# phylo42/IPK

Hardware: AMD Instinct MI355X
Metric: scored phylo-k-mers/sec (higher is better)
Workload: dtype f32

## Files before the change

### ipk_amd/csrc/ipkgpu.hip

```cpp
#include <cstring>
#include <hip/hip_runtime.h>
#include <rocprim/rocprim.hpp>

#include <algorithm>
#include <cmath>
#include <cstdarg>
#include <cstdio>
#include <cstring>
#include <new>
#include <string>
#include <type_traits>
#include <unordered_map>
#include <memory>
#include <vector>

#include "../../include/ipkgpu.h"
#include "dcla_device.hpp"
#include "kernels_score.hpp"
#include "kernels_quad.hpp"
#include "kernels_compact.hpp"
#include "kernels_keymajor.hpp"
#include "kernels_reduce_pipe.hpp"
#include "kernels_filter.hpp"
#include "kernels_dbfile.hpp"
#include "kernels_spill.hpp"
#include "spill_format.hpp"
#include <sys/stat.h>
#include <chrono>

using namespace ipkgpu;


namespace {

struct DevBuf {
    void* p = nullptr;
    size_t cap = 0;
    template <class T> T* as() const { return reinterpret_cast<T*>(p); }
};

struct EventPool {
    std::vector<hipEvent_t> free_ev;
    hipEvent_t get()
    {
        if (!free_ev.empty()) { hipEvent_t e = free_ev.back(); free_ev.pop_back(); return e; }
        hipEvent_t e = nullptr;
        return hipEventCreate(&e) == hipSuccess ? e : nullptr;
    }
    void put(hipEvent_t e) { if (free_ev.size() < 64) free_ev.push_back(e); else (void)hipEventDestroy(e); }
};
struct Stopwatch {
    hipStream_t stream;
    EventPool* pool;
    std::vector<hipEvent_t> ev;
    Stopwatch(hipStream_t s, EventPool* p) : stream(s), pool(p) {}
    ~Stopwatch() { for (hipEvent_t e : ev) pool->put(e); }
    int mark()
    {
        hipEvent_t e = pool->get();
        if (!e) return -1;
        (void)hipEventRecord(e, stream);
        ev.push_back(e);
        return (int)ev.size() - 1;
    }
    double ms(int a, int b) const
    {
        float t = 0;
        if (a < 0 || b < 0 || hipEventElapsedTime(&t, ev[a], ev[b]) != hipSuccess) return 0;
        return t;
    }
};

}

struct ipkgpu_comm;
struct ipkgpu_ctx;
static void ipkgpu_comm_release(ipkgpu_ctx* ctx);
struct ipkgpu_ctx {
    int device = 0;
    ipkgpu_comm* comm = nullptr;
    hipStream_t stream = nullptr;
    std::string err;
    int64_t workspace_bytes = 0;
    int64_t opt_variant = 0;
    int64_t opt_flags = 0;
    int64_t opt_kmc_pass = 0;
    int64_t opt_prefix_mats = 0;
    int64_t opt_wg_chunks2 = 0;
    int64_t opt_rounds = 0;
    int64_t opt_pool_limit = 0;
    int64_t opt_pool_chunks = 0;
    DevBuf table, best, ovfq, counts, offsets, goff, idx, branch, scan_sums, scan_boff, tmp_a, tmp_b, tmp_c;
    DevBuf pool, desc, gbcnt, gboff, gbcur, clist, gm, tile_next;
    DevBuf ptrs;
    DevBuf sp_bits, sp_pops, sp_rank, sp_c16;
    void* h_spill[2] = {nullptr, nullptr}; hipEvent_t ev_spill[2] = {nullptr, nullptr}; size_t h_spill_cap = 0;
    size_t held = 0, held_peak = 0;
    int64_t budget = 0;
    size_t refused_need = 0;
    DevBuf mask;
    bool mask_valid = false;
    uint64_t mask_words = 0;
    bool table_compressed = false;
    DevBuf rank, vaddr, ucnt, qpack, xstart, pcounts;
    DevBuf seq, pvals, pvaddr, mrank, cursnap;
    DevBuf cvals, coff, croom;
    bool comp_own_vals = false;
    std::vector<uint32_t> h_branch;
    uint32_t comp_nb = 0, comp_stride = 0, comp_tbl = 0;
    double pairs_per_window = 0;
    double acc_main_ms = 0, acc_reduce_ms = 0;
    double acc_count_ms = 0, acc_write_ms = 0, acc_km_ms = 0;
    const char* main_kernel = "";
    std::vector<std::pair<void*, size_t>> free_blocks;
    std::unordered_map<void*, size_t> live_blocks;
    size_t cached_bytes = 0, cache_limit = 0;
    void* small = nullptr;
    void* h_up = nullptr; size_t h_up_cap = 0; hipEvent_t up_done = nullptr; bool up_pending = false;
    unsigned long long emitted_host = 0; bool emitted_fetched = false;
    uint32_t* h_rb = nullptr;
    EventPool events;
    bool spec_skip_wait = false;
    uint64_t pool_want_min = 0;
    struct Pending {
        bool active = false;
        std::unique_ptr<Stopwatch> sw; int ev_a = -1, ev_b = -1, ev_c = -1, ev_d = -1;
        uint64_t cap = 0, max_chunks = 0, windows = 0; uint32_t gb = 0; bool pool_ovf_ok = false, use_quad = false;
    } pend;
    uint64_t last_entries = 0; uint32_t last_gb = 0;
    double t_write_total = 0, t_write_device = 0, t_write_file = 0;
    int num_cu = 256;
};

struct ipkgpu_result {
    ipkgpu_ctx* ctx = nullptr;
    std::vector<uint32_t> group_ids;
    std::vector<uint64_t> offsets;
    uint64_t emitted = 0;
    uint32_t* d_keys = nullptr;
    float* d_scores = nullptr;
    uint32_t* d_positions = nullptr;
    size_t cap = 0;
    std::vector<uint32_t> h_keys;
    std::vector<float> h_scores;
    std::vector<uint32_t> h_positions;
    bool h_keys_ok = false, h_scores_ok = false, h_positions_ok = false;
    double t_total = 0, t_prefix = 0, t_score = 0, t_compact = 0, t_main = 0, t_reduce = 0;
    int score_launches = 0;
};

struct ipkgpu_parts {
    ipkgpu_ctx* ctx = nullptr;
    uint32_t n_owners = 1;
    uint64_t slots = 0;
    uint32_t* d_counts = nullptr;
    uint2* d_entries = nullptr;
    uint32_t* d_positions = nullptr;
    std::vector<uint64_t> owner_off;
    uint64_t emitted = 0;
    uint32_t* pre_keys = nullptr; uint64_t* pre_key_off = nullptr; uint64_t pre_n_keys = 0; double t_keys = 0;
    uint32_t sigma = 0, k = 0;
    uint32_t lead = 0;
    uint64_t key_base = 0;
    double t_total = 0, t_prefix = 0, t_score = 0, t_compact = 0, t_main = 0, t_reduce = 0, t_count = 0, t_write = 0, t_km = 0;
    int score_launches = 0;
};

struct ipkgpu_db {
    ipkgpu_ctx* ctx = nullptr;
    uint64_t n_keys = 0, n_entries = 0;
    uint32_t* d_keys = nullptr;
    uint64_t* d_key_off = nullptr;
    uint2* d_entries = nullptr;
    uint32_t* d_positions = nullptr;
    std::vector<uint32_t> h_positions;
    bool h_pos_ok = false;
    std::vector<uint32_t> h_keys;
    std::vector<uint64_t> h_key_off;
    std::vector<uint32_t> h_entries;
    bool h_ok = false;
    double t_merge = 0;
    double* d_fv64 = nullptr;
    float* d_fv32 = nullptr;
    uint32_t* d_order = nullptr;
    std::vector<double> h_fv64;
    std::vector<float> h_fv32;
    std::vector<uint32_t> h_order;
    bool h_filter_ok = false;
    double t_filter = 0;
};

static std::string g_create_err;
constexpr size_t RB_BYTES = 4096, RB_OWNER_OFF = 8 , RB_OWNERS_MAX = 500;

template <class T = uint32_t> static T* small_at(const ipkgpu_ctx* ctx, uint32_t off) { return reinterpret_cast<T*>(static_cast<char*>(ctx->small) + off); }

static int fail(ipkgpu_ctx* ctx, int code, const char* fmt, ...)
{
    char buf[512];
    va_list ap;
    va_start(ap, fmt);
    vsnprintf(buf, sizeof buf, fmt, ap);
    va_end(ap);
    if (ctx) ctx->err = buf; else g_create_err = buf;
    return code;
}

#define HIP_TRY(ctx, expr)                                                                      \
    do {                                                                                        \
        hipError_t e_ = (expr);                                                                 \
// ... 49 lines not shown


static int upload_stage(ipkgpu_ctx* ctx, size_t bytes, void** out)
{
    if (ctx->up_pending) { HIP_TRY(ctx, hipEventSynchronize(ctx->up_done)); ctx->up_pending = false; }
    if (!ctx->up_done) HIP_TRY(ctx, hipEventCreateWithFlags(&ctx->up_done, hipEventDisableTiming));
    if (bytes > ctx->h_up_cap) {
        if (ctx->h_up) { (void)hipHostFree(ctx->h_up); ctx->h_up = nullptr; ctx->h_up_cap = 0; }
        const size_t cap = std::max<size_t>(bytes + bytes / 2, 1 << 16);
        HIP_TRY(ctx, hipHostMalloc(&ctx->h_up, cap, hipHostMallocDefault));
        ctx->h_up_cap = cap;
    }
    *out = ctx->h_up;
    return IPKGPU_OK;
}
static int upload_staged(ipkgpu_ctx* ctx)
{
    HIP_TRY(ctx, hipEventRecord(ctx->up_done, ctx->stream));
    ctx->up_pending = true;
    return IPKGPU_OK;
}

static hipError_t ctx_alloc(ipkgpu_ctx* ctx, void** out, size_t bytes)
{
    bytes = std::max<size_t>((bytes + 255) & ~(size_t)255, 256);
    size_t best = (size_t)-1;
    for (size_t i = 0; i < ctx->free_blocks.size(); ++i) {
        const size_t cap = ctx->free_blocks[i].second;
        if (cap >= bytes && cap <= bytes + bytes / 2 + (1 << 20) && (best == (size_t)-1 || cap < ctx->free_blocks[best].second)) best = i;
    }
    if (best != (size_t)-1) {
        *out = ctx->free_blocks[best].first;
        ctx->live_blocks[*out] = ctx->free_blocks[best].second;
        ctx->cached_bytes -= ctx->free_blocks[best].second;
        ctx->free_blocks.erase(ctx->free_blocks.begin() + best);
        return hipSuccess;
    }
    hipError_t e = dev_malloc(ctx, out, bytes);
    if (e != hipSuccess && !ctx->free_blocks.empty()) {
        drop_cache(ctx);
        (void)hipGetLastError();
        e = dev_malloc(ctx, out, bytes);
    }
    if (e == hipSuccess) ctx->live_blocks[*out] = bytes;
    return e;
}
static void ctx_release(ipkgpu_ctx* ctx, void* p)
{
    if (!p) return;
    auto it = ctx->live_blocks.find(p);
    if (it == ctx->live_blocks.end()) { (void)hipFree(p); return; }
    const size_t cap = it->second;
    ctx->live_blocks.erase(it);
    if (ctx->cached_bytes + cap <= ctx->cache_limit) { ctx->free_blocks.push_back({p, cap}); ctx->cached_bytes += cap; }
    else (void)dev_free(ctx, p, cap);
}

static constexpr uint64_t WAVE_PER_ITEM_SPAN = 1ull << 24;

static hipError_t ctx_alloc_atleast(ipkgpu_ctx* ctx, void** out, size_t min_bytes, size_t want_bytes, size_t* got)
{
    min_bytes = std::max<size_t>((min_bytes + 255) & ~(size_t)255, 256);
    want_bytes = std::max(want_bytes, min_bytes);
    size_t best = (size_t)-1;
    for (size_t i = 0; i < ctx->free_blocks.size(); ++i) {
        const size_t cap = ctx->free_blocks[i].second;
        if (cap >= min_bytes && cap <= want_bytes + want_bytes / 2 + (1 << 20) && (best == (size_t)-1 || cap < ctx->free_blocks[best].second)) best = i;
    }
    if (best != (size_t)-1) {
        *out = ctx->free_blocks[best].first;
        *got = ctx->free_blocks[best].second;
        ctx->live_blocks[*out] = *got;
        ctx->cached_bytes -= *got;
        ctx->free_blocks.erase(ctx->free_blocks.begin() + best);
        return hipSuccess;
    }
    const hipError_t e = ctx_alloc(ctx, out, want_bytes);
    if (e == hipSuccess) *got = ctx->live_blocks[*out];
    return e;
}

static std::vector<DevBuf*> all_workspaces(ipkgpu_ctx* ctx)
{
    return {&ctx->table, &ctx->best, &ctx->ovfq, &ctx->counts, &ctx->offsets, &ctx->goff, &ctx->idx,
            &ctx->branch, &ctx->scan_sums, &ctx->scan_boff, &ctx->tmp_a, &ctx->tmp_b, &ctx->tmp_c,
            &ctx->pool, &ctx->desc, &ctx->gbcnt, &ctx->gboff, &ctx->gbcur, &ctx->clist, &ctx->gm, &ctx->tile_next, &ctx->mask,
            &ctx->rank, &ctx->vaddr, &ctx->ucnt, &ctx->qpack, &ctx->xstart, &ctx->pcounts, &ctx->ptrs,
            &ctx->cvals, &ctx->coff, &ctx->croom, &ctx->seq, &ctx->pvals, &ctx->pvaddr, &ctx->mrank, &ctx->cursnap,
            &ctx->sp_bits, &ctx->sp_pops, &ctx->sp_rank, &ctx->sp_c16};
}

extern "C" {

uint32_t ipkgpu_bits_per_symbol(uint32_t sigma) { return sigma == 4 ? 2u : sigma == 20 ? 5u : 0u; }
uint32_t ipkgpu_max_k(uint32_t sigma) { return sigma == 4 ? 14u : sigma == 20 ? 6u : 0u; }
uint32_t ipkgpu_max_k_keyrange(uint32_t sigma) { return sigma == 4 ? 16u : ipkgpu_max_k(sigma); }
size_t ipkgpu_kmer_batch(uint32_t key, size_t n_ranges) { return n_ranges ? key % n_ranges : 0; }

float ipkgpu_log_threshold(float omega, uint32_t sigma, uint32_t k)
{
    return log10f(powf(omega / (float)sigma, (float)k));
}

const char* ipkgpu_last_error(const ipkgpu_ctx* ctx) { return ctx ? ctx->err.c_str() : g_create_err.c_str(); }

int ipkgpu_create(int device_id, ipkgpu_ctx** out)
{
    if (!out) return fail(nullptr, IPKGPU_ERR_INVALID, "ipkgpu_create: null out pointer");
    *out = nullptr;
    int n = 0;
    hipError_t e = hipGetDeviceCount(&n);
    if (e != hipSuccess || n <= 0)
        return fail(nullptr, IPKGPU_ERR_NODEVICE, "no HIP device available (%s); this engine has no CPU fallback",
                    e != hipSuccess ? hipGetErrorString(e) : "device count 0");
    if (device_id < 0 || device_id >= n)
        return fail(nullptr, IPKGPU_ERR_INVALID, "device %d out of range (0..%d)", device_id, n - 1);
    ipkgpu_ctx* ctx = new (std::nothrow) ipkgpu_ctx();
    if (!ctx) return fail(nullptr, IPKGPU_ERR_NOMEM, "out of host memory");
    ctx->device = device_id;
    if ((e = hipSetDevice(device_id)) != hipSuccess ||
        (e = hipStreamCreateWithFlags(&ctx->stream, hipStreamNonBlocking)) != hipSuccess) {
        delete ctx;
        return fail(nullptr, IPKGPU_ERR_HIP, "device setup failed: %s", hipGetErrorString(e));
    }
    hipDeviceProp_t prop;
    if (hipGetDeviceProperties(&prop, device_id) == hipSuccess) ctx->num_cu = prop.multiProcessorCount;
    size_t free_b = 0, total_b = 0;
    if (hipMemGetInfo(&free_b, &total_b) == hipSuccess) { ctx->workspace_bytes = (int64_t)(free_b / 2); ctx->cache_limit = free_b / 4; }
    else ctx->workspace_bytes = (int64_t)8 << 30;
    if ((e = hipMalloc(&ctx->small, SMALL_BYTES)) != hipSuccess) {
        (void)hipStreamDestroy(ctx->stream);
        delete ctx;
        return fail(nullptr, IPKGPU_ERR_NOMEM, "hipMalloc failed: %s", hipGetErrorString(e));
    }
    if ((e = hipHostMalloc((void**)&ctx->h_rb, RB_BYTES, hipHostMallocDefault)) != hipSuccess) {
        (void)hipFree(ctx->small);
        (void)hipStreamDestroy(ctx->stream);
        delete ctx;
        return fail(nullptr, IPKGPU_ERR_NOMEM, "hipHostMalloc failed: %s", hipGetErrorString(e));
    }
    memset(ctx->h_rb, 0, RB_BYTES);
    *out = ctx;
    return IPKGPU_OK;
}

void ipkgpu_destroy(ipkgpu_ctx* ctx)
{
    if (!ctx) return;
    (void)hipSetDevice(ctx->device);
    (void)hipStreamSynchronize(ctx->stream);
    for (DevBuf* b : all_workspaces(ctx)) if (b->p) (void)hipFree(b->p);
    for (auto& b : ctx->free_blocks) (void)hipFree(b.first);
    ipkgpu_comm_release(ctx);
    if (ctx->small) (void)hipFree(ctx->small);
    if (ctx->h_up) (void)hipHostFree(ctx->h_up);
    for (int i = 0; i < 2; ++i) { if (ctx->h_spill[i]) (void)hipHostFree(ctx->h_spill[i]); if (ctx->ev_spill[i]) (void)hipEventDestroy(ctx->ev_spill[i]); }
    ctx->pend.sw.reset();
    for (hipEvent_t e : ctx->events.free_ev) (void)hipEventDestroy(e);
    ctx->events.free_ev.clear();
    if (ctx->h_rb) (void)hipHostFree(ctx->h_rb);
    if (ctx->up_done) (void)hipEventDestroy(ctx->up_done);
    (void)hipStreamDestroy(ctx->stream);
    delete ctx;
}

int ipkgpu_set_option(ipkgpu_ctx* ctx, const char* name, int64_t value)
{
// ... 55 lines not shown
    if (SIGMA == 4) return K <= 10 ? IPK_QCAP : IPK_QCAP12;
    return IPK_AACAP;
}

template <int SIGMA, int K, bool POS = false>
int launch_score(ipkgpu_ctx* ctx, const ScoreParams& p)
{
    constexpr int CAP = fast_cap<SIGMA, K>();
    constexpr size_t lds = TileGeo<SIGMA, K, TW>::HEAD_BYTES + (size_t)NW * wave_scratch_entries<SIGMA, K, CAP>() * 8;
    static_assert(lds <= 160 * 1024, "fast-path LDS budget");
    auto kern = score_tiles_kernel<SIGMA, K, CAP, TW, NW, POS>;
    if (lds > 64 * 1024)
        HIP_TRY(ctx, hipFuncSetAttribute(reinterpret_cast<const void*>(kern), hipFuncAttributeMaxDynamicSharedMemorySize, (int)lds));
    const uint64_t blocks = (uint64_t)p.n_batch_mats * p.tiles_per_mat;
    if (blocks > 0x7fffffffull) return fail(ctx, IPKGPU_ERR_INVALID, "batch too large for one launch");
    hipLaunchKernelGGL(kern, dim3((uint32_t)blocks), dim3(NW * 64), lds, ctx->stream, p);
    HIP_TRY(ctx, hipGetLastError());
    return IPKGPU_OK;
}

template <int SIGMA, int K, bool POS = false>
int launch_overflow(ipkgpu_ctx* ctx, const ScoreParams& p)
{
    if constexpr (Geo<SIGMA, K, 1 << 30>::DIRECT || ipow(SIGMA, K - K / 2) <= (uint32_t)fast_cap<SIGMA, K>()) {
        (void)ctx; (void)p;
        return IPKGPU_OK;
    } else {
        constexpr size_t lds = TileGeo<SIGMA, K, 1>::HEAD_BYTES + (size_t)wave_scratch_entries<SIGMA, K, big_capf<SIGMA, K>()>() * 8;
        static_assert(lds <= 160 * 1024, "big-list LDS budget");
        auto kern = score_overflow_kernel<SIGMA, K, POS>;
        if (lds > 64 * 1024)
            HIP_TRY(ctx, hipFuncSetAttribute(reinterpret_cast<const void*>(kern), hipFuncAttributeMaxDynamicSharedMemorySize, (int)lds));
        const uint32_t per_cu = (uint32_t)std::max<size_t>(1, std::min<size_t>(32 / OVF_NW, (160 * 1024) / (lds + 64)));
        hipLaunchKernelGGL(kern, dim3(ctx->num_cu * per_cu), dim3(OVF_NW * 64), lds, ctx->stream, p);
        HIP_TRY(ctx, hipGetLastError());
        return IPKGPU_OK;
    }
}

template <int SIGMA, int K, bool POS>
int launch_both(ipkgpu_ctx* ctx, const ScoreParams& p)
{
    RC_TRY((launch_score<SIGMA, K, POS>(ctx, p)));
    return launch_overflow<SIGMA, K, POS>(ctx, p);
}


template <int SIGMA, int K> constexpr uint32_t stream_tbl()
{
    constexpr uint64_t T = ipow(SIGMA, K);
    if (Geo<SIGMA, K, 1 << 30>::DIRECT) return 0;
    if (SIGMA == 4 && K >= 13) return 0;
    if (SIGMA == 4) return T <= 16384 ? (uint32_t)T : (K <= 10 ? 16384u : 32768u);
    if (K <= 3) return (uint32_t)T;
    if (K <= 5) return 32000u;
    return 0;
}

template <int SIGMA, int K> constexpr int stream_nw() { return NW; }
template <int SIGMA, int K> constexpr int stream_tw() { return TW; }

template <int SIGMA, int K>
int launch_stream_pass1(ipkgpu_ctx* ctx, const StreamParams& sp, uint32_t n_wg)
{
    constexpr uint32_t TBL = stream_tbl<SIGMA, K>();
    if constexpr (TBL == 0) { (void)sp; (void)n_wg; return fail(ctx, IPKGPU_ERR_INVALID, "stream variant unsupported for this sigma/k"); }
    else {
        constexpr int CAP = fast_cap<SIGMA, K>();
        constexpr uint32_t T = ipow(SIGMA, K);
        constexpr uint32_t NB = (T + TBL - 1) / TBL;
        constexpr int SNW = stream_nw<SIGMA, K>(), STW = stream_tw<SIGMA, K>();
        constexpr size_t lds = TileGeo<SIGMA, K, STW>::HEAD_BYTES + (size_t)SNW * stream_wave_scratch<SIGMA, K, CAP>() * 8 + (size_t)SNW * 2 * NB * SUB * 4;
        static_assert(lds <= 160 * 1024, "stream pass-1 LDS budget");
        auto kern = score_stream_kernel<SIGMA, K, CAP, STW, SNW, TBL>;
        if (lds > 64 * 1024)
            HIP_TRY(ctx, hipFuncSetAttribute(reinterpret_cast<const void*>(kern), hipFuncAttributeMaxDynamicSharedMemorySize, (int)lds));
        hipLaunchKernelGGL(kern, dim3(n_wg), dim3(SNW * 64), lds, ctx->stream, sp);
        HIP_TRY(ctx, hipGetLastError());
        return IPKGPU_OK;
    }
}

template <int SIGMA, int K>
int launch_stream_overflow(ipkgpu_ctx* ctx, const StreamParams& sp)
{
    constexpr uint32_t TBL = stream_tbl<SIGMA, K>();
    if constexpr (TBL == 0 || ipow(SIGMA, K - K / 2) <= (uint32_t)fast_cap<SIGMA, K>()) {
        (void)ctx; (void)sp;
        return IPKGPU_OK;
    } else {
        constexpr uint32_t NB = (uint32_t)((ipow(SIGMA, K) + TBL - 1) / TBL);
        constexpr size_t lds = TileGeo<SIGMA, K, 1>::HEAD_BYTES + (size_t)wave_scratch_entries<SIGMA, K, big_capf<SIGMA, K>()>() * 8 +
                               (size_t)OVF_NW * 2 * NB * SUB * 4;
        static_assert(lds + 64 <= 160 * 1024, "big-list (stream) LDS budget");
        auto kern = score_overflow_stream_kernel<SIGMA, K, TBL>;
        if (lds > 64 * 1024)
            HIP_TRY(ctx, hipFuncSetAttribute(reinterpret_cast<const void*>(kern), hipFuncAttributeMaxDynamicSharedMemorySize, (int)lds));
        const uint32_t per_cu = (uint32_t)std::max<size_t>(1, std::min<size_t>(32 / OVF_NW, (160 * 1024) / (lds + 64)));
        hipLaunchKernelGGL(kern, dim3(ctx->num_cu * per_cu), dim3(OVF_NW * 64), lds, ctx->stream, sp);
        HIP_TRY(ctx, hipGetLastError());
        return IPKGPU_OK;
    }
}

#ifndef IPK_RPIPE_DEFAULT
#define IPK_RPIPE_DEFAULT 1
#endif
#ifndef IPK_RPIPE_D
#define IPK_RPIPE_D 2
#endif
template <int SIGMA, int K>
int launch_stream_pass2(ipkgpu_ctx* ctx, uint32_t n_gb, uint64_t T, uint32_t* table, bool compress)
{
    constexpr uint32_t TBL = stream_tbl<SIGMA, K>();
    if constexpr (TBL == 0) { (void)n_gb; (void)T; (void)table; (void)compress; return fail(ctx, IPKGPU_ERR_INVALID, "stream variant unsupported"); }
    else {
        constexpr uint32_t NB = (uint32_t)((ipow(SIGMA, K) + TBL - 1) / TBL);
        constexpr int NT = TBL <= 16384 ? 512 : 1024;
        const size_t lds = compress ? (size_t)comp_padded_slots<TBL, NT>() * 4 + (NT / 64 + 1) * 4 : (size_t)TBL * 4;
        auto launch = [&](auto kern) -> int {
            if (lds > 64 * 1024)
                HIP_TRY(ctx, hipFuncSetAttribute(reinterpret_cast<const void*>(kern), hipFuncAttributeMaxDynamicSharedMemorySize, (int)lds));
            hipLaunchKernelGGL(kern, dim3(n_gb), dim3(NT), lds, ctx->stream, ctx->pool.as<uint2>(),
                               ctx->gboff.as<uint64_t>(), ctx->clist.as<uint2>(), NB, T, table, ctx->mask.as<uint32_t>(), ctx->mask_words,
                               ctx->cvals.as<uint2>(), ctx->coff.as<uint64_t>(), ctx->rank.as<uint32_t>(), ctx->vaddr.as<uint64_t>(), ctx->ucnt.as<uint32_t>());
            HIP_TRY(ctx, hipGetLastError());
            return IPKGPU_OK;
        };
        if constexpr (TBL * 4 > 80 * 1024) {
            if (compress && ((IPK_RPIPE_DEFAULT != 0) != ((ctx->opt_flags & 2048) != 0))) {
                constexpr int PD = IPK_RPIPE_D;
                auto kern = reduce_buckets_pipe_kernel<TBL, NT, PD>;
                HIP_TRY(ctx, hipFuncSetAttribute(reinterpret_cast<const void*>(kern), hipFuncAttributeMaxDynamicSharedMemorySize, (int)lds));
                hipLaunchKernelGGL(kern, dim3(std::min<uint32_t>(n_gb, (uint32_t)ctx->num_cu)), dim3(NT), lds, ctx->stream, ctx->pool.as<uint2>(),
                                   ctx->gboff.as<uint64_t>(), ctx->clist.as<uint2>(), n_gb, NB, T, ctx->mask.as<uint32_t>(), ctx->mask_words,
                                   ctx->cvals.as<uint2>(), ctx->coff.as<uint64_t>(), ctx->rank.as<uint32_t>(), ctx->vaddr.as<uint64_t>(), ctx->ucnt.as<uint32_t>());
                HIP_TRY(ctx, hipGetLastError());
                return IPKGPU_OK;
            }
        }
        return compress ? launch(reduce_buckets_kernel<TBL, NT, true>) : launch(reduce_buckets_kernel<TBL, NT, false>);
    }
}

template <int SIGMA, int K> size_t stream_lds() {
    constexpr uint32_t TBL = stream_tbl<SIGMA, K>();
    if constexpr (TBL == 0) return 0;
    else {
        constexpr int CAP = fast_cap<SIGMA, K>();
        constexpr uint32_t NB = (uint32_t)((ipow(SIGMA, K) + TBL - 1) / TBL);
        return TileGeo<SIGMA, K, stream_tw<SIGMA, K>()>::HEAD_BYTES + (size_t)stream_nw<SIGMA, K>() * stream_wave_scratch<SIGMA, K, CAP>() * 8 +
               (size_t)stream_nw<SIGMA, K>() * 2 * NB * SUB * 4;
    }
}
template <int SIGMA, int K> uint32_t stream_nb() {
    constexpr uint32_t TBL = stream_tbl<SIGMA, K>();
    if constexpr (TBL == 0) return 0; else return (uint32_t)((ipow(SIGMA, K) + TBL - 1) / TBL);
}

template <int SIGMA, int K> constexpr bool quad_ok() { return QuadGeo<SIGMA, K>::OK && stream_tbl<SIGMA, K>() != 0; }
#ifndef IPK_QNW
#define IPK_QNW 4
#endif
#ifndef IPK_QTW
#define IPK_QTW 40
#endif
template <int SIGMA, int K> constexpr int quad_nw() { return K <= 10 ? IPK_QNW : IPK_QNW12; }
template <int SIGMA, int K> constexpr int quad_tw() { return K <= 10 ? IPK_QTW : IPK_QTW12; }
#ifndef IPK_QROWLANE12
#define IPK_QROWLANE12 1
#endif
#ifndef IPK_QROWLANE
#define IPK_QROWLANE 0
#endif
template <int SIGMA, int K> constexpr bool quad_rowlane() { return K <= 10 ? IPK_QROWLANE != 0 : IPK_QROWLANE12 != 0; }
#ifndef IPK_QONEWIN12
#define IPK_QONEWIN12 1
#endif
template <int SIGMA, int K> constexpr bool quad_onewin() { return K >= 11 && IPK_QONEWIN12 != 0 && quad_rowlane<SIGMA, K>(); }
template <int SIGMA, int K> size_t quad_lds()
{
    if constexpr (!quad_ok<SIGMA, K>()) return 0;
    else {
        constexpr int CAP = fast_cap<SIGMA, K>();
        constexpr uint32_t TBL = stream_tbl<SIGMA, K>();
        constexpr uint32_t NB = (uint32_t)((ipow(SIGMA, K) + TBL - 1) / TBL);
        return QuadTile<SIGMA, K, quad_tw<SIGMA, K>()>::HEAD_BYTES + (size_t)quad_nw<SIGMA, K>() * quad_wave_entries<SIGMA, K, CAP, quad_onewin<SIGMA, K>()>() * 8 +
               (size_t)quad_nw<SIGMA, K>() * NB * 8;
    }
}
template <int SIGMA, int K, bool COUNT_ONLY = false>
int launch_quad_pass1(ipkgpu_ctx* ctx, const StreamParams& sp, uint32_t n_wg)
{
    if constexpr (!quad_ok<SIGMA, K>()) { (void)sp; (void)n_wg; return fail(ctx, IPKGPU_ERR_INVALID, "quad kernel unsupported for this sigma/k"); }
    else {
        constexpr int CAP = fast_cap<SIGMA, K>();
        constexpr uint32_t TBL = stream_tbl<SIGMA, K>();
        constexpr int QNW = quad_nw<SIGMA, K>(), QTW = quad_tw<SIGMA, K>();
        const size_t lds = quad_lds<SIGMA, K>();
        auto kern = score_quad_kernel<SIGMA, K, CAP, QTW, QNW, TBL, COUNT_ONLY, quad_rowlane<SIGMA, K>(), quad_onewin<SIGMA, K>()>;
        if (lds > 64 * 1024)
            HIP_TRY(ctx, hipFuncSetAttribute(reinterpret_cast<const void*>(kern), hipFuncAttributeMaxDynamicSharedMemorySize, (int)lds));
        hipLaunchKernelGGL(kern, dim3(n_wg), dim3(QNW * 64), lds, ctx->stream, sp);
        HIP_TRY(ctx, hipGetLastError());
        return IPKGPU_OK;
    }
}

#ifndef IPK_XPNW
#define IPK_XPNW 11
#endif
#ifndef IPK_XPTW
#define IPK_XPTW 128
#endif
constexpr int XP_TW = IPK_XPTW;
template <int SIGMA, int K> constexpr int xp_nw() { return SIGMA == 20 ? IPK_XPNW : 11; }
template <int SIGMA, int K> constexpr uint32_t xp_tbl()
{
    if (SIGMA == 20 && K == 6) return 16000u;
    if (SIGMA == 4 && K >= 13) return 32768u;
    return stream_tbl<SIGMA, K>();
}
template <int SIGMA, int K, int KK = K> uint32_t xp_nb() {
    constexpr uint32_t TBL = xp_tbl<SIGMA, K>();
    if constexpr (TBL == 0) return 0; else return (uint32_t)((ipow(SIGMA, KK) + TBL - 1) / TBL);
}
template <int SIGMA, int K, int KK = K> size_t xp_lds() {
    constexpr uint32_t TBL = xp_tbl<SIGMA, K>();
    if constexpr (TBL == 0) return 0;
    else {
        constexpr int CAP = fast_cap<SIGMA, K>();
        constexpr uint32_t NB = (uint32_t)((ipow(SIGMA, KK) + TBL - 1) / TBL);
        return TileGeo<SIGMA, K, XP_TW>::HEAD_BYTES + (size_t)xp_nw<SIGMA, K>() * stream_wave_scratch<SIGMA, K, CAP>() * 8 + (size_t)NB * 4;
    }
}
template <int SIGMA, int K, bool WRITE, int KK = K, bool POS = false>
int launch_xp(ipkgpu_ctx* ctx, const XpParams& xp, uint32_t n_wg)
{
    constexpr uint32_t TBL = xp_tbl<SIGMA, K>();
    if constexpr (TBL == 0) { (void)xp; (void)n_wg; return fail(ctx, IPKGPU_ERR_INVALID, "exact-partition variant unsupported for this sigma/k"); }
    else {
        constexpr int CAP = fast_cap<SIGMA, K>();
        constexpr uint32_t NB = (uint32_t)((ipow(SIGMA, KK) + TBL - 1) / TBL);
        constexpr size_t lds = TileGeo<SIGMA, K, XP_TW>::HEAD_BYTES + (size_t)xp_nw<SIGMA, K>() * stream_wave_scratch<SIGMA, K, CAP>() * 8 + (size_t)NB * 4;
        static_assert(lds <= 160 * 1024, "exact-partition LDS budget");
        static_assert((TileGeo<SIGMA, K, XP_TW>::HEAD_BYTES + (size_t)xp_nw<SIGMA, K>() * stream_wave_scratch<SIGMA, K, CAP>() * 8) % 8 == 0, "cursor alignment");
        auto kern = score_xp_kernel<SIGMA, K, CAP, XP_TW, xp_nw<SIGMA, K>(), TBL, WRITE, KK, POS>;
        if (lds > 64 * 1024)
            HIP_TRY(ctx, hipFuncSetAttribute(reinterpret_cast<const void*>(kern), hipFuncAttributeMaxDynamicSharedMemorySize, (int)lds));
        hipLaunchKernelGGL(kern, dim3(n_wg), dim3(xp_nw<SIGMA, K>() * 64), lds, ctx->stream, xp);
        HIP_TRY(ctx, hipGetLastError());
        return IPKGPU_OK;
    }
}
template <int SIGMA, int K, bool WRITE, int KK = K, bool POS = false>
int launch_xp_overflow(ipkgpu_ctx* ctx, const XpParams& xp)
{
    constexpr uint32_t TBL = xp_tbl<SIGMA, K>();
    if constexpr (TBL == 0 || ipow(SIGMA, K - K / 2) <= (uint32_t)fast_cap<SIGMA, K>()) {
        (void)ctx; (void)xp;
        return IPKGPU_OK;
    } else {
// ... 9 lines not shown
    }
}
template <int SIGMA, int K, bool COMPRESS, int KK = K>
int launch_xp_reduce(ipkgpu_ctx* ctx, uint32_t n_gb, uint32_t S, uint64_t T, const uint64_t* off, uint32_t* table)
{
    constexpr uint32_t TBL = xp_tbl<SIGMA, K>();
    if constexpr (TBL == 0) { (void)n_gb; (void)S; (void)T; (void)off; (void)table; return fail(ctx, IPKGPU_ERR_INVALID, "exact-partition variant unsupported"); }
    else {
        constexpr uint32_t NB = (uint32_t)((ipow(SIGMA, KK) + TBL - 1) / TBL);
        static_assert(!COMPRESS || NB == 1 || TBL % 64 == 0, "a 64-slot block must not straddle two buckets");
        constexpr int NT = TBL <= 16384 ? 512 : 1024;
        constexpr size_t lds = COMPRESS ? (size_t)comp_padded_slots<TBL, NT>() * 4 + (NT / 64 + 1) * 4 : (size_t)TBL * 4;
        auto kern = reduce_ranges_kernel<TBL, NT, COMPRESS>;
        if (lds > 64 * 1024)
            HIP_TRY(ctx, hipFuncSetAttribute(reinterpret_cast<const void*>(kern), hipFuncAttributeMaxDynamicSharedMemorySize, (int)lds));
        hipLaunchKernelGGL(kern, dim3(n_gb), dim3(NT), lds, ctx->stream, ctx->pool.as<uint2>(), off, S, NB, T, table,
                           ctx->mask.as<uint32_t>(), ctx->mask_words, ctx->rank.as<uint32_t>(), ctx->vaddr.as<uint64_t>(), ctx->ucnt.as<uint32_t>());
        HIP_TRY(ctx, hipGetLastError());
        return IPKGPU_OK;
    }
}
template <int SIGMA, int K>
int launch_xp_reduce_pos(ipkgpu_ctx* ctx, uint32_t n_gb, uint32_t S, uint64_t T, const uint64_t* off, uint32_t nwin)
{
    constexpr uint32_t TBL = xp_tbl<SIGMA, K>();
    if constexpr (TBL == 0) { (void)n_gb; (void)S; (void)T; (void)off; (void)nwin; return fail(ctx, IPKGPU_ERR_INVALID, "exact-partition variant unsupported"); }
    else {
        constexpr uint32_t NB = (uint32_t)((ipow(SIGMA, K) + TBL - 1) / TBL);
        static_assert(NB == 1 || TBL % 64 == 0, "a 64-slot block must not straddle two buckets");
        constexpr int NT = pos_sub_slots<TBL>() <= 4096 ? 256 : 1024;
        constexpr size_t lds = (size_t)pos_sub_blocks<TBL>() * 64 * 8 + (pos_sub_blocks<TBL>() + 1) * 4;
        static_assert(lds <= 160 * 1024, "positions reduce LDS budget");
        auto kern = reduce_ranges_pos_kernel<TBL, NT>;
        if (lds > 64 * 1024)
            HIP_TRY(ctx, hipFuncSetAttribute(reinterpret_cast<const void*>(kern), hipFuncAttributeMaxDynamicSharedMemorySize, (int)lds));
        hipLaunchKernelGGL(kern, dim3(n_gb), dim3(NT), lds, ctx->stream, ctx->pool.as<uint2>(), ctx->seq.as<uint32_t>(), off, S, NB, T, nwin,
                           ctx->mask_words, ctx->pvals.as<uint32_t>(), ctx->pvaddr.as<uint64_t>());
        HIP_TRY(ctx, hipGetLastError());
        return IPKGPU_OK;
    }
}
template <int V> using int_c = std::integral_constant<int, V>;

template <int SIGMA, int K, int KMAX, class F> int with_k(ipkgpu_ctx* ctx, uint32_t k, F& f)
{
    if (k == (uint32_t)K) return f(int_c<SIGMA>{}, int_c<K>{});
    if constexpr (K < KMAX) return with_k<SIGMA, K + 1, KMAX>(ctx, k, f);
    else return fail(ctx, IPKGPU_ERR_INVALID, "unsupported sigma/k (%u/%u)", (uint32_t)SIGMA, k);
}
template <class F> int with_sigma_k(ipkgpu_ctx* ctx, uint32_t sigma, uint32_t k, F&& f)
{
    if (sigma == 4) return with_k<4, 2, 14>(ctx, k, f);
    if (sigma == 20) return with_k<20, 2, 6>(ctx, k, f);
    return fail(ctx, IPKGPU_ERR_INVALID, "unsupported sigma/k (%u/%u)", sigma, k);
}

bool keyrange_supported(uint32_t sigma, uint32_t k, uint32_t lead)
{
    return sigma == 4 && lead >= 1 && k > lead && k - lead >= 13 && k - lead <= 14 && k <= 16;
}
template <class F> int with_xp_shape(ipkgpu_ctx* ctx, uint32_t sigma, uint32_t k, uint32_t lead, F&& f)
{
    if (!lead) return with_sigma_k(ctx, sigma, k, [&](auto S_, auto K_) { return f(S_, K_, K_); });
    if (sigma == 4) {
        switch (k * 8 + lead) {
            case 14 * 8 + 1: return f(int_c<4>{}, int_c<14>{}, int_c<13>{});
            case 15 * 8 + 1: return f(int_c<4>{}, int_c<15>{}, int_c<14>{});
            case 15 * 8 + 2: return f(int_c<4>{}, int_c<15>{}, int_c<13>{});
            case 16 * 8 + 2: return f(int_c<4>{}, int_c<16>{}, int_c<14>{});
            case 16 * 8 + 3: return f(int_c<4>{}, int_c<16>{}, int_c<13>{});
        }
    }
    return fail(ctx, IPKGPU_ERR_INVALID, "unsupported key range");
}

struct Geometry {
    uint32_t fast_cap = 0;
    uint32_t stream_nb = 0, stream_tbl = 0;
    uint32_t stream_nw = NW, stream_tw = TW;
    size_t stream_lds = 0;
    bool quad = false;
    uint32_t quad_nw = NW, quad_tw = TW;
    size_t quad_lds = 0;
    uint32_t xp_nb = 0, xp_tbl = 0;
    size_t xp_lds = 0;
};

int fill_geometry(ipkgpu_ctx* ctx, uint32_t sigma, uint32_t k, uint32_t lead, Geometry& g)
{
    if (!lead)
        RC_TRY(with_sigma_k(ctx, sigma, k, [&](auto S_, auto K_) {
            g.fast_cap = fast_cap<S_, K_>();
            g.stream_nb = stream_nb<S_, K_>(); g.stream_tbl = stream_tbl<S_, K_>();
            g.stream_nw = stream_nw<S_, K_>(); g.stream_tw = stream_tw<S_, K_>(); g.stream_lds = stream_lds<S_, K_>();
            g.quad = quad_ok<S_, K_>();
            g.quad_nw = quad_nw<S_, K_>(); g.quad_tw = quad_tw<S_, K_>(); g.quad_lds = quad_lds<S_, K_>();
            return IPKGPU_OK;
        }));
    return with_xp_shape(ctx, sigma, k, lead, [&](auto S_, auto K_, auto KK_) {
        g.xp_nb = xp_nb<S_, K_, KK_>(); g.xp_tbl = xp_tbl<S_, K_>(); g.xp_lds = xp_lds<S_, K_, KK_>();
        return IPKGPU_OK;
    });
}

#ifndef IPK_KMC_RUNS_DEFAULT
#define IPK_KMC_RUNS_DEFAULT 1
#endif
#ifndef IPK_KMC_PASS
#define IPK_KMC_PASS 256
#endif
#define KM_LAUNCH(KERN, CAPV, ...)                                                                                        \
    do {                                                                                                                  \
        if (P == 1) hipLaunchKernelGGL((KERN<true, CAPV>), dim3((uint32_t)(per_xcd * 8)), dim3(256), 0, ctx->stream, __VA_ARGS__); \
        else hipLaunchKernelGGL((KERN<false, CAPV>), dim3((uint32_t)(per_xcd * 8)), dim3(256), 0, ctx->stream, __VA_ARGS__);     \
    } while (0)

CompTable comp_table(const ipkgpu_ctx* ctx)
{
    CompTable ct;
    ct.mask = ctx->mask.as<uint32_t>(); ct.rank = ctx->rank.as<uint32_t>(); ct.vaddr = ctx->vaddr.as<uint64_t>();
    ct.pool = ctx->comp_own_vals ? ctx->cvals.as<uint2>() : ctx->pool.as<uint2>();
    ct.off = ctx->comp_own_vals ? ctx->coff.as<uint64_t>() : ctx->gboff.as<uint64_t>(); ct.mask_words = ctx->mask_words;
    ct.NB = ctx->comp_nb; ct.stride = ctx->comp_stride; ct.TBL = ctx->comp_tbl;
    return ct;
}

}

namespace {

constexpr int IPKGPU_RETRY_SMALLER = 100;
constexpr int IPKGPU_RETRY_AGAIN = 101;
#ifndef IPK_OVF_POOL_RATIO
#define IPK_OVF_POOL_RATIO 500
#endif

enum class PassKind { tiles, stream, quad, xp };
struct Pass {
    PassKind kind = PassKind::tiles;
    bool positions = false;
    bool compress = false;
    bool seq = false;
    double slot_bytes() const { return positions ? 8.0 : kind == PassKind::xp && compress ? 0.3125 : 4.0; }
};

Pass choose_pass(int64_t variant, uint32_t sigma, uint32_t lead, bool positions, bool km_positions, const Geometry& g)
{
    Pass ps;
    ps.positions = positions;
    if (positions) return ps;
    if (km_positions) { ps.kind = PassKind::xp; ps.compress = true; ps.seq = true; return ps; }
    const int64_t v = variant;
    if (g.xp_nb != 0 && (v == 3 || v == 4 || (v == 0 && g.stream_nb == 0) || lead != 0)) {
        ps.kind = PassKind::xp;
        ps.compress = v != 3;
    } else if (g.stream_nb != 0 && g.stream_nb <= 2048 && (v == 0 || v == 2 || v == 5 || v == 6 || v == 7)) {
        ps.kind = v != 2 && g.quad ? PassKind::quad : PassKind::stream;
        ps.compress = v == 6 || (v == 0 && g.stream_tbl == 32768u && sigma == 4);
    }
    return ps;
}

struct Plan {
    uint32_t n_mats = 0, sites = 0, sigma = 0, k = 0;
    float eps = 0;
    std::vector<uint32_t> group_ids;
    std::vector<uint32_t> slot_of;
    uint32_t n_groups = 0, nwin = 0, tiles_per_mat = 0, chunks_per_group = 0;
    uint64_t table_size = 0, gpb = 1;
    uint32_t lead = 0, lead_c = 0;
    Geometry geo;
    Pass pass;
    const uint32_t* mat_rank = nullptr;
};

int make_plan(ipkgpu_ctx* ctx, const void* logp, uint32_t n_mats, uint32_t sites, uint32_t sigma,
              const uint32_t* mat_group, uint32_t k, float log_eps, Plan& pl, uint32_t lead = 0, uint32_t lead_c = 0,
              bool positions = false, bool km_positions = false)
{
    if (!logp || !mat_group) return fail(ctx, IPKGPU_ERR_INVALID, "null input pointer");
    if (sigma != 4 && sigma != 20) return fail(ctx, IPKGPU_ERR_INVALID, "unsupported alphabet size %u (4 or 20)", sigma);
    if (lead == 0 && (k < 2 || k > ipkgpu_max_k(sigma)))
        return fail(ctx, IPKGPU_ERR_INVALID, "k=%u out of range [2, %u] for sigma=%u", k, ipkgpu_max_k(sigma), sigma);
    if (lead != 0 && !keyrange_supported(sigma, k, lead))
        return fail(ctx, IPKGPU_ERR_INVALID, "no key-range pass of k=%u with %u leading symbols for sigma=%u", k, lead, sigma);
    pl.lead = lead; pl.lead_c = lead_c;
    if (n_mats == 0) return fail(ctx, IPKGPU_ERR_INVALID, "no matrices");
    if (sites < k) return fail(ctx, IPKGPU_ERR_INVALID, "alignment has %u sites, fewer than k=%u", sites, k);
    pl.n_mats = n_mats; pl.sites = sites; pl.sigma = sigma; pl.k = k; pl.eps = log_eps;
    RC_TRY(fill_geometry(ctx, sigma, k, lead, pl.geo));
    if (km_positions && (lead != 0 || pl.geo.xp_nb == 0))
        return fail(ctx, IPKGPU_ERR_INVALID, "no positioned database for sigma=%u k=%u: the call takes the exact partition, which needs more than 64 keys "
                                             "and no key-range pass", sigma, k);
    pl.pass = choose_pass(ctx->opt_variant, sigma, lead, positions, km_positions, pl.geo);
    pl.slot_of.resize(n_mats);
    std::unordered_map<uint32_t, uint32_t> index;
    index.reserve(n_mats);
    for (uint32_t i = 0; i < n_mats; ++i) {
        auto it = index.find(mat_group[i]);
        if (it == index.end()) {
            it = index.emplace(mat_group[i], (uint32_t)pl.group_ids.size()).first;
            pl.group_ids.push_back(mat_group[i]);
        }
        pl.slot_of[i] = it->second;
    }
    pl.n_groups = (uint32_t)pl.group_ids.size();
    pl.table_size = ipow(sigma, (int)(k - lead));
    pl.chunks_per_group = (uint32_t)((pl.table_size + CHUNK - 1) / CHUNK);
    pl.nwin = sites - k + 1;
    {
        const double ppw = ctx->pairs_per_window > 0 ? ctx->pairs_per_window : 256.0;
        const double pool_per_group = (double)n_mats / (double)pl.n_groups * (double)pl.nwin * ppw * (pl.pass.seq ? 16.0 : 8.0) * 1.25;
        const double per_group = (double)pl.table_size * pl.pass.slot_bytes() + pool_per_group;
        pl.gpb = std::max<uint64_t>(1, (uint64_t)((double)ctx->workspace_bytes / per_group));
    }
    pl.gpb = std::min<uint64_t>(pl.gpb, pl.n_groups);
    while (pl.gpb > 1 && pl.gpb * pl.chunks_per_group > 0x7fffffffull) pl.gpb /= 2;
    pl.tiles_per_mat = (pl.nwin + TW - 1) / TW;
// ... 81 lines not shown
        const size_t free_b = mem_free_bytes(ctx);
        const bool over_limit = ctx->opt_pool_limit > 0 && total * 8 > (uint64_t)ctx->opt_pool_limit;
        const uint64_t side = seq ? total * 8 + 512 : 0;
        const uint64_t side_have = seq ? ctx->seq.cap + ctx->pvals.cap : 0;
        if (over_limit || (total * 8 > ctx->pool.cap && total * 8 > free_b + ctx->pool.cap) ||
            (side > side_have && total * 8 + side > free_b + ctx->pool.cap + side_have)) {
            if (gb > 1) return IPKGPU_RETRY_SMALLER;
            return fail(ctx, IPKGPU_ERR_NOMEM, "the pair pool of ONE branch group (%llu pairs) does not fit device memory", (unsigned long long)total);
        }
    }
    RC_TRY(ensure(ctx, ctx->pool, std::max<uint64_t>(total, 1) * 8 + 256));
    {
        const uint64_t n_start = (uint64_t)gb * S * XNB;
        RC_TRY(ensure(ctx, ctx->xstart, n_start * 4));
        hipLaunchKernelGGL(xp_unit_starts_kernel, dim3((uint32_t)((n_start + 255) / 256)), dim3(256), 0, ctx->stream,
                           ctx->gboff.as<uint64_t>(), XNB, S, stride, n_start, ctx->xstart.as<uint32_t>(), small_at(ctx, SMALL_XP_TOO_BIG));
        HIP_TRY(ctx, hipGetLastError());
        xp.start = ctx->xstart.as<uint32_t>();
    }
    sp.pool = ctx->pool.as<uint2>();
    if (seq) {
        RC_TRY(ensure(ctx, ctx->seq, std::max<uint64_t>(total, 1) * 4 + 256));
        RC_TRY(ensure(ctx, ctx->pvals, std::max<uint64_t>(total, 1) * 4 + 256));
        xp.seq = ctx->seq.as<uint32_t>(); xp.mat_rank = pl.mat_rank;
    }
    const int ev_c = sw.mark();
    RC_TRY(xp_kernel(true));
    const int ev_d0 = sw.mark();
    RC_TRY(xp_overflow(true));
    const int ev_d = sw.mark();
    if (compress) {
        RC_TRY(ensure(ctx, ctx->rank, (size_t)gb * (ctx->mask_words / 2) * 4));
        RC_TRY(ensure(ctx, ctx->vaddr, (size_t)gb * (ctx->mask_words / 2) * 8));
        RC_TRY(ensure(ctx, ctx->ucnt, n_gb * 4));
    } else {
        RC_TRY(ensure(ctx, ctx->table, (size_t)gb * pl.table_size * 4));
    }
    uint32_t* const table = compress ? nullptr : ctx->table.as<uint32_t>();
    if (seq) {
        RC_TRY(ensure(ctx, ctx->pvaddr, (size_t)gb * (ctx->mask_words / 2) * 8));
        RC_TRY(with_sigma_k(ctx, pl.sigma, pl.k, [&](auto S_, auto K_) {
            return launch_xp_reduce_pos<S_, K_>(ctx, (uint32_t)n_gb, stride, pl.table_size, ctx->gboff.as<uint64_t>(), pl.nwin);
        }));
    }
    RC_TRY(with_xp_shape(ctx, pl.sigma, pl.k, pl.lead, [&](auto S_, auto K_, auto KK_) {
        const uint64_t* off = ctx->gboff.as<uint64_t>();
        return compress ? launch_xp_reduce<S_, K_, true, KK_>(ctx, (uint32_t)n_gb, stride, pl.table_size, off, table)
                        : launch_xp_reduce<S_, K_, false, KK_>(ctx, (uint32_t)n_gb, stride, pl.table_size, off, table);
    }));
    const int ev_e = sw.mark();
    uint32_t too_big = 0;
    HIP_TRY(ctx, hipMemcpyAsync(&too_big, small_at(ctx, SMALL_XP_TOO_BIG), 4, hipMemcpyDeviceToHost, ctx->stream));
    HIP_TRY(ctx, hipStreamSynchronize(ctx->stream));
    if (too_big) return fail(ctx, IPKGPU_ERR_INVALID, "a branch group scores 2^32 phylo-k-mers or more in one batch (exact-partition variant: 32-bit offsets inside a group)");
    ctx->mask_valid = true;
    ctx->table_compressed = compress;
    ctx->comp_nb = XNB; ctx->comp_stride = stride; ctx->comp_tbl = pl.geo.xp_tbl;
    ctx->acc_main_ms += sw.ms(ev_a, ev_a2) + sw.ms(ev_c, ev_d0);
    ctx->acc_count_ms += sw.ms(ev_a, ev_a2); ctx->acc_write_ms += sw.ms(ev_c, ev_d0);
    ctx->acc_reduce_ms += sw.ms(ev_d, ev_e);
    ctx->main_kernel = "score_xp_kernel";
    return IPKGPU_OK;
}

int stream_batch_check(ipkgpu_ctx* ctx)
{
    ipkgpu_ctx::Pending& pd = ctx->pend;
    if (!pd.active) return IPKGPU_OK;
    pd.active = false;
    std::unique_ptr<Stopwatch> sw(pd.sw.release());
    const uint32_t n_ovf = ctx->h_rb[SMALL_OVF_COUNT / 4], pool_exhausted = ctx->h_rb[SMALL_POOL_OVF / 4];
    if (pool_exhausted) {
        if (pd.cap >= pd.max_chunks) {
            ctx->pool_want_min = 0;
            if (pd.gb > 1) return IPKGPU_RETRY_SMALLER;
            return fail(ctx, IPKGPU_ERR_NOMEM, "the pair pool of ONE branch group is exhausted at the device-memory limit");
        }
        ctx->pool_want_min = pd.cap * 2;
        return IPKGPU_RETRY_AGAIN;
    }
    ctx->pool_want_min = 0;
    memcpy(&ctx->emitted_host, ctx->h_rb + SMALL_EMITTED / 4, 8);
    ctx->emitted_fetched = true;
    ctx->spec_skip_wait = !(n_ovf > 0 && (uint64_t)n_ovf * IPK_OVF_POOL_RATIO >= pd.windows && pd.pool_ovf_ok);
    if (sw) { ctx->acc_main_ms += sw->ms(pd.ev_a, pd.ev_b); ctx->acc_reduce_ms += sw->ms(pd.ev_c, pd.ev_d); }
    return IPKGPU_OK;
}

int arm_capped(ipkgpu_ctx* ctx, uint32_t sigma, uint32_t k, ScoreParams& p)
{
    const bool capped_lists = sigma == 4 && k >= 13;
    p.big_ovf = capped_lists ? small_at(ctx, SMALL_BIG_OVF) : nullptr;
    if (capped_lists) HIP_TRY(ctx, hipMemsetAsync(p.big_ovf, 0, 4, ctx->stream));
    return IPKGPU_OK;
}

int check_capped(ipkgpu_ctx* ctx, uint32_t k, const ScoreParams& p)
{
    if (!p.big_ovf) return IPKGPU_OK;
    uint32_t hit = 0;
    HIP_TRY(ctx, hipMemcpyAsync(&hit, p.big_ovf, 4, hipMemcpyDeviceToHost, ctx->stream));
    HIP_TRY(ctx, hipStreamSynchronize(ctx->stream));
    if (hit) return fail(ctx, IPKGPU_ERR_INVALID, "a window's half list exceeds %d entries: beyond the capacity of this engine at k = %u "
                                                  "(the lists of k >= 13 are capped; lower omega's reach or k)", BIG_CAP_ENTRIES, k);
    return IPKGPU_OK;
}

int score_batch_impl(ipkgpu_ctx* ctx, const Plan& pl, const float* logp_dev, uint32_t g0, uint32_t gb, bool defer)
{
    const uint32_t n_mats = pl.n_mats;
    uint32_t nb = 0;
    for (uint32_t i = 0; i < n_mats; ++i) nb += (pl.slot_of[i] >= g0 && pl.slot_of[i] < g0 + gb);
    const size_t gm_words = (size_t)gb + 1 + nb;
    void* stage = nullptr;
    RC_TRY(upload_stage(ctx, ((size_t)n_mats * 2 + gm_words) * 4, &stage));
    uint32_t* mat_list_h = reinterpret_cast<uint32_t*>(stage);
    uint32_t* mat_slot_h = mat_list_h + n_mats;
    uint32_t* gm = mat_slot_h + n_mats;
    nb = 0;
    for (uint32_t i = 0; i < n_mats; ++i) {
        mat_slot_h[i] = 0;
        if (pl.slot_of[i] >= g0 && pl.slot_of[i] < g0 + gb) { mat_list_h[nb++] = i; mat_slot_h[i] = pl.slot_of[i] - g0; }
    }
    for (uint32_t i = nb; i < n_mats; ++i) mat_list_h[i] = 0;
    for (size_t i = 0; i < gm_words; ++i) gm[i] = 0;
    for (uint32_t i = 0; i < n_mats; ++i)
        if (pl.slot_of[i] >= g0 && pl.slot_of[i] < g0 + gb) gm[pl.slot_of[i] - g0 + 1]++;
    for (uint32_t g = 0; g < gb; ++g) gm[g + 1] += gm[g];
    {
        std::vector<uint32_t> cur(gm, gm + gb);
        for (uint32_t i = 0; i < n_mats; ++i)
            if (pl.slot_of[i] >= g0 && pl.slot_of[i] < g0 + gb) gm[(size_t)gb + 1 + cur[pl.slot_of[i] - g0]++] = i;
    }
    RC_TRY(ensure(ctx, ctx->idx, (size_t)n_mats * 8));
    RC_TRY(ensure(ctx, ctx->ovfq, (size_t)nb * pl.nwin * 8));
    RC_TRY(ensure(ctx, ctx->gm, gm_words * 4));
    HIP_TRY(ctx, hipMemcpyAsync(ctx->idx.p, mat_list_h, (size_t)n_mats * 8, hipMemcpyHostToDevice, ctx->stream));
    HIP_TRY(ctx, hipMemcpyAsync(ctx->gm.p, gm, gm_words * 4, hipMemcpyHostToDevice, ctx->stream));
    RC_TRY(upload_staged(ctx));

    const Pass& ps = pl.pass;
    ScoreParams p;
    p.logp = logp_dev;
    p.best = ctx->best.as<float>();
    p.mat_list = ctx->idx.as<uint32_t>();
    p.mat_slot = ctx->idx.as<uint32_t>() + n_mats;
    p.n_batch_mats = nb; p.sites = pl.sites; p.nwin = pl.nwin; p.tiles_per_mat = pl.tiles_per_mat;
    p.eps = pl.eps;
    p.table = ctx->table.p;
    p.mat_rank = pl.mat_rank;
    p.table_size = pl.table_size;
    p.emitted = small_at<unsigned long long>(ctx, SMALL_EMITTED);
    p.ovf_queue = ctx->ovfq.as<unsigned long long>();
    p.ovf_count = small_at(ctx, SMALL_OVF_COUNT);
    p.flags = (uint32_t)(!ps.positions && ctx->opt_variant == 99 ? 1 : 0);
    p.mask = nullptr; p.mask_words = 0;
    RC_TRY(arm_capped(ctx, pl.sigma, pl.k, p));
    ctx->mask_valid = false;
    ctx->table_compressed = false;
    ctx->comp_own_vals = false;
    const bool use_stream = ps.kind == PassKind::stream || ps.kind == PassKind::quad;
    const bool use_quad = ps.kind == PassKind::quad;
    if (!use_stream) {
        HIP_TRY(ctx, hipMemsetAsync(p.emitted, 0, 8, ctx->stream));
        HIP_TRY(ctx, hipMemsetAsync(p.ovf_count, 0, 4, ctx->stream));
    }
    if (ps.kind == PassKind::tiles) {
        const size_t table_bytes = (size_t)gb * pl.table_size * (ps.positions ? 8 : 4);
        RC_TRY(ensure(ctx, ctx->table, table_bytes));
        p.table = ctx->table.p;
        HIP_TRY(ctx, hipMemsetAsync(ctx->table.p, 0, table_bytes, ctx->stream));
        Stopwatch sw(ctx->stream, &ctx->events);
        const int a = sw.mark();
        RC_TRY(with_sigma_k(ctx, pl.sigma, pl.k, [&](auto S_, auto K_) {
            if (ps.positions) return launch_both<S_, K_, true>(ctx, p);
            if constexpr (S_ == 4 && K_ > 12) return fail(ctx, IPKGPU_ERR_INVALID, "unsupported sigma/k (%u/%u)", pl.sigma, pl.k);
            else return launch_both<S_, K_, false>(ctx, p);
        }));
        const int b = sw.mark();
        HIP_TRY(ctx, hipStreamSynchronize(ctx->stream));
        ctx->acc_main_ms += sw.ms(a, b);
        ctx->main_kernel = "score_tiles_kernel";
        return check_capped(ctx, pl.k, p);
    }

    ctx->mask_words = 2 * ((pl.table_size + 63) / 64);
    RC_TRY(ensure(ctx, ctx->mask, (size_t)gb * ctx->mask_words * 4));
    p.mask = ctx->mask.as<uint32_t>(); p.mask_words = ctx->mask_words;
    if (ps.kind == PassKind::xp) {
        if (!ps.compress) {
            RC_TRY(ensure(ctx, ctx->table, (size_t)gb * pl.table_size * 4));
            p.table = ctx->table.p;
        }
        const int rc = score_batch_xp(ctx, pl, logp_dev, gb, p);
        return rc ? rc : check_capped(ctx, pl.k, p);
    }

    const bool pool_ovf_ok = gb < (1u << 22) && n_mats < (1u << 21) && pl.nwin < (1u << 21);
    bool s_compress = pool_ovf_ok && ps.compress;
    const uint32_t NBK = pl.geo.stream_nb, TBL = pl.geo.stream_tbl;
    const uint32_t SNW = use_quad ? pl.geo.quad_nw : pl.geo.stream_nw;
    const uint32_t STW = use_quad ? pl.geo.quad_tw : pl.geo.stream_tw;
    const uint32_t s_tiles_per_mat = (pl.nwin + STW - 1) / STW;
    auto pass1 = [&](const StreamParams& sp, uint32_t n_wg, bool count_only) {
        return with_sigma_k(ctx, pl.sigma, pl.k, [&](auto S_, auto K_) {
            if (!use_quad) return launch_stream_pass1<S_, K_>(ctx, sp, n_wg);
            return count_only ? launch_quad_pass1<S_, K_, true>(ctx, sp, n_wg) : launch_quad_pass1<S_, K_, false>(ctx, sp, n_wg);
        });
    };

    const uint64_t windows = (uint64_t)nb * pl.nwin;
    if (ctx->pairs_per_window <= 0) {
        const uint32_t n_s = std::min<uint32_t>(gb, std::max<uint32_t>(2, gb / 64));
        const uint32_t stride_g = gb / n_s;
        std::vector<uint32_t> sgm((size_t)n_s + 1, 0), slist;
        for (uint32_t j = 0; j < n_s; ++j) {
            const uint32_t g = j * stride_g;
            for (uint32_t m = gm[g]; m < gm[g + 1]; ++m) slist.push_back(gm[(size_t)gb + 1 + m]);
            sgm[j + 1] = (uint32_t)slist.size();
        }
        std::vector<uint32_t> both(sgm);
        both.insert(both.end(), slist.begin(), slist.end());
        RC_TRY(ensure(ctx, ctx->tmp_a, both.size() * 4));
        HIP_TRY(ctx, hipMemcpyAsync(ctx->tmp_a.p, both.data(), both.size() * 4, hipMemcpyHostToDevice, ctx->stream));
        HIP_TRY(ctx, hipMemsetAsync(p.emitted, 0, 8, ctx->stream));
        HIP_TRY(ctx, hipMemsetAsync(p.ovf_count, 0, 4, ctx->stream));
        StreamParams ss;
        ss.logp = logp_dev; ss.best = ctx->best.as<float>();
        ss.gm_off = ctx->tmp_a.as<uint32_t>(); ss.gm_list = ctx->tmp_a.as<uint32_t>() + n_s + 1;
        ss.sites = pl.sites; ss.nwin = pl.nwin; ss.tiles_per_mat = s_tiles_per_mat;
        ss.S = (uint32_t)std::max<uint64_t>(1, std::min<uint64_t>(s_tiles_per_mat, (uint64_t)ctx->num_cu * 4 / n_s));
        ss.eps = pl.eps;
        ss.pool = nullptr; ss.pool_cap = 0; ss.pool_next = nullptr; ss.desc = nullptr; ss.pool_ovf = nullptr; ss.pre_chunks = 0;
        ss.emitted = p.emitted; ss.ovf_queue = p.ovf_queue; ss.ovf_count = p.ovf_count; ss.mat_slot = p.mat_slot;
        ss.flags = 2u;
        RC_TRY(pass1(ss, n_s * ss.S, true));
        unsigned long long se = 0; uint32_t so = 0;
        HIP_TRY(ctx, hipMemcpyAsync(&se, p.emitted, 8, hipMemcpyDeviceToHost, ctx->stream));
        HIP_TRY(ctx, hipMemcpyAsync(&so, p.ovf_count, 4, hipMemcpyDeviceToHost, ctx->stream));
        HIP_TRY(ctx, hipStreamSynchronize(ctx->stream));
        const uint64_t s_windows = (uint64_t)slist.size() * pl.nwin;
        const double cap_pairs = 0.25 * (double)pl.geo.fast_cap * (double)pl.geo.fast_cap;
        if (s_windows) ctx->pairs_per_window = std::max(1.0, ((double)se + (double)so * cap_pairs) / (double)s_windows * 1.15);
    }
    const double ppw_est = ctx->pairs_per_window > 0 ? ctx->pairs_per_window : 256.0;
    if (!s_compress && pool_ovf_ok && ctx->opt_variant == 0 && pl.table_size >= (1u << 16) &&
        (double)windows * ppw_est < 0.5 * (double)gb * (double)pl.table_size)
        s_compress = true;
    if (!s_compress) {
        RC_TRY(ensure(ctx, ctx->table, (size_t)gb * pl.table_size * 4));
        p.table = ctx->table.p;
    }
    const size_t lds_bytes = use_quad ? pl.geo.quad_lds : pl.geo.stream_lds;
    const uint64_t wg_per_cu = std::max<uint64_t>(1, std::min<uint64_t>(32 / SNW, (160 * 1024) / std::max<size_t>(lds_bytes, 1)));
    const uint64_t slots = (uint64_t)ctx->num_cu * wg_per_cu;
    const uint32_t CH = chunk_pairs_rt(TBL);
    const uint64_t expected_chunks = (uint64_t)((double)windows * ppw_est / CH);
#ifndef IPK_WG_CHUNKS2
#define IPK_WG_CHUNKS2 2
#endif
    const uint64_t wg_chunks2 = ctx->opt_wg_chunks2 > 0 ? (uint64_t)ctx->opt_wg_chunks2 : (uint64_t)IPK_WG_CHUNKS2;
    const uint64_t max_wg = std::max<uint64_t>(slots, expected_chunks * 2 / wg_chunks2 / ((uint64_t)SNW * NBK * SUB));
#ifndef IPK_ROUNDS
#define IPK_ROUNDS 8
#endif
    const uint64_t rounds = std::max<uint64_t>(1, std::min<uint64_t>(ctx->opt_rounds > 0 ? (uint64_t)ctx->opt_rounds : (uint64_t)IPK_ROUNDS, max_wg / slots));
    uint64_t S64 = std::max<uint64_t>(1, (slots * rounds) / gb);
    uint32_t S = (uint32_t)std::max<uint64_t>(1, std::min<uint64_t>(S64, s_tiles_per_mat));
    const uint32_t n_wg = gb * S;
    const uint64_t n_waves = (uint64_t)n_wg * SNW;
    const uint64_t n_gb = (uint64_t)gb * NBK;

    const size_t free_b = mem_free_bytes(ctx);
    uint64_t max_chunks = std::min<uint64_t>(0xFFFFFFF0ull, (uint64_t)(free_b + ctx->pool.cap + ctx->desc.cap) * 9 / 10 / (CH * 8 + 8));
    if (ctx->opt_pool_limit > 0) max_chunks = std::min<uint64_t>(max_chunks, (uint64_t)ctx->opt_pool_limit / (CH * 8 + 8));
    const double ppw = ctx->pairs_per_window > 0 ? ctx->pairs_per_window : 256.0;
    const uint64_t ovf_waves = (uint64_t)ctx->num_cu * 4 * OVF_NW;
    const uint64_t slack = 2 * (n_waves + ovf_waves) * NBK * SUB + (n_waves + ovf_waves) * ALLOC_BATCH + 1024;
    uint64_t want = (uint64_t)((double)windows * ppw * 1.25 / CH) + slack;
    {
        const uint64_t have = std::min<uint64_t>(std::max<uint64_t>(ctx->pool.cap / (CH * 8), 1) - 1, ctx->desc.cap / 8);
        const uint64_t need = (uint64_t)((double)windows * ppw * 1.1 / CH) + (n_waves + ovf_waves) * (NBK * SUB + ALLOC_BATCH) + 1024;
        if (have >= need) want = have;
    }
    want = std::max<uint64_t>(want, ctx->pool_want_min);
    for (int attempt = 0; attempt < 6; ++attempt) {
        uint64_t cap = std::min<uint64_t>(want, max_chunks);
        const bool forced = attempt == 0 && ctx->opt_pool_chunks > 0 && ctx->pool_want_min == 0;
        if (forced) cap = (uint64_t)ctx->opt_pool_chunks;
        else if (cap < n_waves * NBK * SUB) {
            if (gb > 1) return IPKGPU_RETRY_SMALLER;
            return fail(ctx, IPKGPU_ERR_NOMEM, "the pair pool of ONE branch group does not fit device memory");
        }
        RC_TRY(ensure(ctx, ctx->pool, (cap + 1) * CH * 8));
        RC_TRY(ensure(ctx, ctx->desc, cap * 8));
        if (!forced) cap = std::min<uint64_t>(ctx->pool.cap / (CH * 8) - 1, ctx->desc.cap / 8);
        RC_TRY(ensure(ctx, ctx->gbcnt, 2 * n_gb * 4));
        uint32_t* const d_gbcur = ctx->gbcnt.as<uint32_t>() + n_gb;
        RC_TRY(ensure(ctx, ctx->gboff, (n_gb + 1) * 8));
        uint32_t* d_pool_next = small_at(ctx, SMALL_POOL_NEXT);
        uint32_t* d_pool_ovf = small_at(ctx, SMALL_POOL_OVF);
        const bool pre_ok = use_quad && n_waves * NBK + 1024 <= cap && !(ctx->opt_flags & 32);
        const uint32_t pre_chunks = pre_ok ? (uint32_t)(n_waves * NBK) : 0u;
        uint32_t* d_tile_next = nullptr;
        if (use_quad && !(ctx->opt_flags & 128) && ((uint64_t)nb * s_tiles_per_mat >= 4ull * gb * S || (ctx->opt_flags & 256))) {
            RC_TRY(ensure(ctx, ctx->tile_next, (size_t)gb * 4));
            d_tile_next = ctx->tile_next.as<uint32_t>();
        }
        hipLaunchKernelGGL(small_reset_kernel, dim3((std::max<uint32_t>(gb, SMALL_XP_TOO_BIG / 4) + 255) / 256), dim3(256), 0, ctx->stream,
                           reinterpret_cast<uint32_t*>(ctx->small), pre_chunks, d_tile_next, gb, S);
        HIP_TRY(ctx, hipGetLastError());
        HIP_TRY(ctx, hipMemsetAsync(ctx->desc.p, 0, cap * 8, ctx->stream));

        StreamParams sp;
        sp.logp = logp_dev; sp.best = ctx->best.as<float>();
        sp.gm_off = ctx->gm.as<uint32_t>(); sp.gm_list = ctx->gm.as<uint32_t>() + gb + 1;
        sp.sites = pl.sites; sp.nwin = pl.nwin; sp.tiles_per_mat = s_tiles_per_mat; sp.S = S;
        sp.eps = pl.eps;
        sp.pool = ctx->pool.as<uint2>(); sp.pool_cap = (uint32_t)cap; sp.pool_next = d_pool_next;
        sp.desc = ctx->desc.as<unsigned long long>(); sp.pool_ovf = d_pool_ovf;
        sp.emitted = p.emitted; sp.ovf_queue = p.ovf_queue; sp.ovf_count = p.ovf_count; sp.mat_slot = p.mat_slot;
        sp.flags = (uint32_t)(ctx->opt_flags);
        sp.pre_chunks = pre_chunks;
        sp.tile_next = d_tile_next;
        std::unique_ptr<Stopwatch> sw_own(new Stopwatch(ctx->stream, &ctx->events));
        Stopwatch& sw = *sw_own;
        const int ev_a = sw.mark();
        RC_TRY(pass1(sp, n_wg, false));
        const int ev_b = sw.mark();
        const bool spec = ctx->spec_skip_wait && !s_compress && !(ctx->opt_flags & 64);
        uint32_t n_ovf = 0;
        uint32_t h[2] = {0, 0};
        if (!spec) {
            HIP_TRY(ctx, hipMemcpyAsync(ctx->h_rb, ctx->small, SMALL_BYTES, hipMemcpyDeviceToHost, ctx->stream));
            HIP_TRY(ctx, hipStreamSynchronize(ctx->stream));
            n_ovf = ctx->h_rb[SMALL_OVF_COUNT / 4]; h[0] = ctx->h_rb[SMALL_POOL_NEXT / 4]; h[1] = ctx->h_rb[SMALL_POOL_OVF / 4];
        }
        const bool ovf_in_pool = n_ovf > 0 && ((uint64_t)n_ovf * IPK_OVF_POOL_RATIO >= windows || s_compress) && pool_ovf_ok;
        if (ovf_in_pool) {
            RC_TRY(ensure(ctx, ctx->tmp_a, (size_t)n_ovf * 8));
            RC_TRY(ensure(ctx, ctx->tmp_b, (size_t)n_ovf * 8));
            hipLaunchKernelGGL(ovf_group_keys_kernel, dim3((n_ovf + 255) / 256), dim3(256), 0, ctx->stream,
                               p.ovf_queue, n_ovf, p.mat_slot, ctx->tmp_a.as<unsigned long long>());
            HIP_TRY(ctx, hipGetLastError());
            size_t tmp_bytes = 0;
            HIP_TRY(ctx, rocprim::radix_sort_keys(nullptr, tmp_bytes, ctx->tmp_a.as<unsigned long long>(), ctx->tmp_b.as<unsigned long long>(),
                                                  (size_t)n_ovf, 0, 64, ctx->stream));
            RC_TRY(ensure(ctx, ctx->tmp_c, tmp_bytes));
            HIP_TRY(ctx, rocprim::radix_sort_keys(ctx->tmp_c.p, tmp_bytes, ctx->tmp_a.as<unsigned long long>(), ctx->tmp_b.as<unsigned long long>(),
                                                  (size_t)n_ovf, 0, 64, ctx->stream));
            StreamParams so = sp;
            so.ovf_queue = ctx->tmp_b.as<unsigned long long>();
            if (use_quad) so.emitted = small_at<unsigned long long>(ctx, SMALL_OVF_EMITTED);
            RC_TRY(with_sigma_k(ctx, pl.sigma, pl.k, [&](auto S_, auto K_) { return launch_stream_overflow<S_, K_>(ctx, so); }));
        }
        if (ovf_in_pool) {
            HIP_TRY(ctx, hipMemcpyAsync(ctx->h_rb, ctx->small, SMALL_BYTES, hipMemcpyDeviceToHost, ctx->stream));
            HIP_TRY(ctx, hipStreamSynchronize(ctx->stream));
            h[0] = ctx->h_rb[SMALL_POOL_NEXT / 4]; h[1] = ctx->h_rb[SMALL_POOL_OVF / 4];
        }
        if (h[1] != 0) {
            if (cap >= max_chunks) {
                if (gb > 1) return IPKGPU_RETRY_SMALLER;
                return fail(ctx, IPKGPU_ERR_NOMEM, "the pair pool of ONE branch group is exhausted at the device-memory limit");
            }
            want = std::max<uint64_t>(cap * 2, want);
            continue;
        }
        const uint32_t n_used = spec ? (uint32_t)cap : (uint32_t)std::min<uint64_t>(h[0], cap);
        const uint32_t* n_used_dev = spec ? d_pool_next : nullptr;
        HIP_TRY(ctx, hipMemsetAsync(ctx->gbcnt.p, 0, 2 * n_gb * 4, ctx->stream));
        RC_TRY(ensure(ctx, ctx->clist, ((uint64_t)n_used + 16) * 8));
        if (s_compress) {
            RC_TRY(ensure(ctx, ctx->croom, 2 * n_gb * 4));
            HIP_TRY(ctx, hipMemsetAsync(ctx->croom.p, 0, n_gb * 4, ctx->stream));
        }
        if (n_used) {
            hipLaunchKernelGGL(chunk_hist_kernel, dim3(std::min<uint32_t>((n_used + 255) / 256, 2048u)), dim3(256), 0, ctx->stream,
                               ctx->desc.as<unsigned long long>(), n_used, ctx->gbcnt.as<uint32_t>(),
                               use_quad ? p.emitted : (unsigned long long*)nullptr, s_compress ? ctx->croom.as<uint32_t>() : (uint32_t*)nullptr,
                               n_used_dev);
            HIP_TRY(ctx, hipGetLastError());
        }
        RC_TRY(scan_u32(ctx, ctx->gbcnt.as<uint32_t>(), n_gb, ctx->gboff.as<uint64_t>()));
        if (s_compress) {
            hipLaunchKernelGGL(comp_slice_room_kernel, dim3((uint32_t)((n_gb + 255) / 256)), dim3(256), 0, ctx->stream,
                               ctx->croom.as<uint32_t>(), (uint32_t)n_gb, NBK, pl.table_size, TBL, ctx->croom.as<uint32_t>() + n_gb);
            HIP_TRY(ctx, hipGetLastError());
            RC_TRY(ensure(ctx, ctx->coff, (n_gb + 1) * 8));
            RC_TRY(scan_u32(ctx, ctx->croom.as<uint32_t>() + n_gb, n_gb, ctx->coff.as<uint64_t>()));
            const uint64_t max_vals = std::min<uint64_t>((uint64_t)n_used * CH, (uint64_t)gb * pl.table_size);
            RC_TRY(ensure(ctx, ctx->cvals, (max_vals / 2 + n_gb + 1) * 8 + 256));
            RC_TRY(ensure(ctx, ctx->rank, (size_t)gb * (ctx->mask_words / 2) * 4));
            RC_TRY(ensure(ctx, ctx->vaddr, (size_t)gb * (ctx->mask_words / 2) * 8));
            RC_TRY(ensure(ctx, ctx->ucnt, n_gb * 4));
        }
        if (n_used) {
            const uint64_t n_grid = spec ? std::min<uint64_t>(n_used, expected_chunks * 2 + n_waves * NBK + 4096) : n_used;
            hipLaunchKernelGGL(chunk_scatter_kernel, dim3((uint32_t)std::min<uint64_t>((n_grid + 255) / 256, 1u << 16)), dim3(256), 0, ctx->stream,
                               ctx->desc.as<unsigned long long>(), n_used, ctx->gboff.as<uint64_t>(), d_gbcur,
                               ctx->clist.as<uint2>(), n_used_dev);
            HIP_TRY(ctx, hipGetLastError());
        }
        const int ev_c = sw.mark();
        RC_TRY(with_sigma_k(ctx, pl.sigma, pl.k, [&](auto S_, auto K_) {
            return launch_stream_pass2<S_, K_>(ctx, (uint32_t)n_gb, pl.table_size, ctx->table.as<uint32_t>(), s_compress);
        }));
        const int ev_d = sw.mark();
        if ((spec || n_ovf > 0) && !ovf_in_pool)
            RC_TRY(with_sigma_k(ctx, pl.sigma, pl.k, [&](auto S_, auto K_) { return launch_overflow<S_, K_, false>(ctx, p); }));
        if (s_compress) {
            ctx->table_compressed = true; ctx->comp_own_vals = true;
            ctx->comp_nb = NBK; ctx->comp_stride = 1; ctx->comp_tbl = TBL;
        }
        ctx->mask_valid = true;
        ctx->main_kernel = use_quad ? "score_quad_kernel" : "score_stream_kernel";
        HIP_TRY(ctx, hipMemcpyAsync(ctx->h_rb, ctx->small, SMALL_BYTES, hipMemcpyDeviceToHost, ctx->stream));
        ipkgpu_ctx::Pending& pd = ctx->pend;
        pd.sw.reset(sw_own.release());
        pd.ev_a = ev_a; pd.ev_b = ev_b; pd.ev_c = ev_c; pd.ev_d = ev_d;
        pd.cap = cap; pd.max_chunks = max_chunks; pd.windows = windows; pd.gb = gb; pd.pool_ovf_ok = pool_ovf_ok; pd.use_quad = use_quad;
        pd.active = true;
        if (defer) return IPKGPU_OK;
        HIP_TRY(ctx, hipStreamSynchronize(ctx->stream));
        const int rcf = stream_batch_check(ctx);
        if (rcf == IPKGPU_RETRY_AGAIN) { want = std::max<uint64_t>(want, ctx->pool_want_min); continue; }
        return rcf;
    }
    return fail(ctx, IPKGPU_ERR_NOMEM, "pair pool could not be sized");
}

int score_batch_finish(ipkgpu_ctx* ctx, const Plan& pl, uint32_t g0, uint32_t gb, uint64_t* emitted_acc)
{
    if (ctx->pend.active) RC_TRY(stream_batch_check(ctx));
    unsigned long long e = ctx->emitted_host;
    if (!ctx->emitted_fetched) {
        HIP_TRY(ctx, hipMemcpyAsync(ctx->h_rb, small_at(ctx, SMALL_EMITTED), 8, hipMemcpyDeviceToHost, ctx->stream));
        HIP_TRY(ctx, hipStreamSynchronize(ctx->stream));
        memcpy(&e, ctx->h_rb, 8);
    }
    *emitted_acc += e;
    if (pl.pass.positions) return IPKGPU_OK;
    uint64_t nb = 0;
    for (uint32_t i = 0; i < pl.n_mats; ++i) nb += (pl.slot_of[i] >= g0 && pl.slot_of[i] < g0 + gb);
    if (nb) ctx->pairs_per_window = (double)e / ((double)nb * pl.nwin);
    return IPKGPU_OK;
}

int score_batch(ipkgpu_ctx* ctx, const Plan& pl, const float* logp_dev, uint32_t g0, uint32_t gb, uint64_t* emitted_acc, bool defer = false)
{
    ctx->emitted_fetched = false;
    ctx->pend.active = false; ctx->pend.sw.reset();
    RC_TRY(score_batch_impl(ctx, pl, logp_dev, g0, gb, defer));
    if (ctx->pend.active) return IPKGPU_OK;
    return score_batch_finish(ctx, pl, g0, gb, emitted_acc);
}

#if defined(__HIP_DEVICE_COMPILE__)
#define IPK_GLOBAL_U32(p) ((ipkgpu::global_u32_ptr)(p))
#else
#define IPK_GLOBAL_U32(p) (p)
#endif
struct ScanU32In {
    const uint32_t* in; uint64_t n;
    __host__ __device__ uint64_t operator()(uint64_t i) const { return i < n ? (uint64_t)IPK_GLOBAL_U32(in)[i] : 0ull; }
};
struct ScanNonzeroIn {
    const uint32_t* in; uint64_t n;
    __host__ __device__ uint64_t operator()(uint64_t i) const { return i < n ? (uint64_t)(IPK_GLOBAL_U32(in)[i] != 0u) : 0ull; }
};
int scan_nonzero_u32(ipkgpu_ctx* ctx, const uint32_t* in, uint64_t n, uint64_t* out)
{
    if (n == 0) { HIP_TRY(ctx, hipMemsetAsync(out, 0, 8, ctx->stream)); return IPKGPU_OK; }
    auto it = rocprim::make_transform_iterator(rocprim::make_counting_iterator<uint64_t>(0), ScanNonzeroIn{in, n});
    size_t bytes = 0;
    HIP_TRY(ctx, rocprim::exclusive_scan(nullptr, bytes, it, out, (uint64_t)0, (size_t)(n + 1), rocprim::plus<uint64_t>(), ctx->stream));
    RC_TRY(ensure(ctx, ctx->scan_sums, bytes));
    HIP_TRY(ctx, rocprim::exclusive_scan(ctx->scan_sums.p, bytes, it, out, (uint64_t)0, (size_t)(n + 1), rocprim::plus<uint64_t>(), ctx->stream));
    return IPKGPU_OK;
}
struct ScanRowsIn {
    const uint32_t* const* rows; uint64_t slots, n;
    __host__ __device__ uint64_t operator()(uint64_t i) const
    {
#if defined(__HIP_DEVICE_COMPILE__)
        typedef const uint32_t* const __attribute__((address_space(1)))* rows_ptr;
        return i < n ? (uint64_t)IPK_GLOBAL_U32(((rows_ptr)rows)[i / slots])[i % slots] : 0ull;
#else
        return i < n ? (uint64_t)rows[i / slots][i % slots] : 0ull;
#endif
    }
};
int scan_rows_u32(ipkgpu_ctx* ctx, const uint32_t* const* rows, uint32_t S, uint64_t slots, uint64_t* out)
{
    const uint64_t n = (uint64_t)S * slots;
    if (n == 0) { HIP_TRY(ctx, hipMemsetAsync(out, 0, 8, ctx->stream)); return IPKGPU_OK; }
    auto it = rocprim::make_transform_iterator(rocprim::make_counting_iterator<uint64_t>(0), ScanRowsIn{rows, slots, n});
    size_t bytes = 0;
    HIP_TRY(ctx, rocprim::exclusive_scan(nullptr, bytes, it, out, (uint64_t)0, (size_t)(n + 1), rocprim::plus<uint64_t>(), ctx->stream));
    RC_TRY(ensure(ctx, ctx->scan_sums, bytes));
    HIP_TRY(ctx, rocprim::exclusive_scan(ctx->scan_sums.p, bytes, it, out, (uint64_t)0, (size_t)(n + 1), rocprim::plus<uint64_t>(), ctx->stream));
    return IPKGPU_OK;
}
int scan_u32(ipkgpu_ctx* ctx, const uint32_t* in, uint64_t n, uint64_t* out)
{
    if (n == 0) { HIP_TRY(ctx, hipMemsetAsync(out, 0, 8, ctx->stream)); return IPKGPU_OK; }
    auto it = rocprim::make_transform_iterator(rocprim::make_counting_iterator<uint64_t>(0), ScanU32In{in, n});
    size_t bytes = 0;
    HIP_TRY(ctx, rocprim::exclusive_scan(nullptr, bytes, it, out, (uint64_t)0, (size_t)(n + 1), rocprim::plus<uint64_t>(), ctx->stream));
    RC_TRY(ensure(ctx, ctx->scan_sums, bytes));
    HIP_TRY(ctx, rocprim::exclusive_scan(ctx->scan_sums.p, bytes, it, out, (uint64_t)0, (size_t)(n + 1), rocprim::plus<uint64_t>(), ctx->stream));
    return IPKGPU_OK;
}

int group_major(ipkgpu_ctx* ctx, const float* logp_dev, uint32_t n_mats, uint32_t sites, uint32_t sigma, const uint32_t* mat_group,
                uint32_t k, float log_eps, bool positions, ipkgpu_result** out)
{
    if (!ctx) return IPKGPU_ERR_INVALID;
    if (!out) return fail(ctx, IPKGPU_ERR_INVALID, "null out pointer");
    *out = nullptr;
    Plan pl;
    RC_TRY(make_plan(ctx, logp_dev, n_mats, sites, sigma, mat_group, k, log_eps, pl, 0, 0, positions));
    HIP_TRY(ctx, hipSetDevice(ctx->device));
    const uint32_t n_groups = pl.n_groups, cpg = pl.chunks_per_group;
    if (positions) {
        if ((uint64_t)n_mats * pl.nwin >= 0xFFFFFFFFull) return fail(ctx, IPKGPU_ERR_INVALID, "too many windows per group for the position code");
        std::vector<uint32_t> rank(n_mats), seen(n_groups, 0);
        for (uint32_t i = 0; i < n_mats; ++i) rank[i] = seen[pl.slot_of[i]]++;
        RC_TRY(ensure(ctx, ctx->branch, (size_t)n_mats * 4));
        HIP_TRY(ctx, hipMemcpy(ctx->branch.p, rank.data(), (size_t)n_mats * 4, hipMemcpyHostToDevice));
        pl.mat_rank = ctx->branch.as<uint32_t>();
    }

    ipkgpu_result* res = new (std::nothrow) ipkgpu_result();
    if (!res) return fail(ctx, IPKGPU_ERR_NOMEM, "out of host memory");
    res->ctx = ctx;
    res->group_ids = pl.group_ids;
    res->offsets.assign((size_t)n_groups + 1, 0);
    struct Guard { ipkgpu_result* r; ~Guard() { if (r) ipkgpu_result_free(r); } } guard{res};
    void** const arrays[3] = {(void**)&res->d_keys, (void**)&res->d_scores, (void**)&res->d_positions};
    const int n_arrays = positions ? 3 : 2;

    RC_TRY(ensure(ctx, ctx->counts, (size_t)(pl.gpb * cpg) * 4));
    RC_TRY(ensure(ctx, ctx->offsets, (size_t)(pl.gpb * cpg + 1) * 8));
    RC_TRY(ensure(ctx, ctx->goff, (size_t)(pl.gpb + 1) * 8));

    ctx->acc_main_ms = ctx->acc_reduce_ms = ctx->acc_count_ms = ctx->acc_write_ms = ctx->acc_km_ms = 0;
    Stopwatch sw(ctx->stream, &ctx->events);
    const int t_begin = sw.mark();
    RC_TRY(run_prefix(ctx, pl, logp_dev));
    const int t_pre = sw.mark();
    std::vector<std::pair<int, int>> ev_score, ev_compact;
    uint64_t total_entries = 0;
    uint32_t gpb_now = (uint32_t)pl.gpb, gb = 0;
    for (uint32_t g0 = 0; g0 < n_groups; g0 += gb) {
        gb = std::min<uint32_t>(gpb_now, n_groups - g0);
        const int s0 = sw.mark();
        const int rcb = score_batch(ctx, pl, logp_dev, g0, gb, &res->emitted);
        if (rcb == IPKGPU_RETRY_SMALLER) { gpb_now = std::max<uint32_t>(1, gb / 2); gb = 0; continue; }
        if (rcb) return rcb;
        const int s1 = sw.mark();
        ev_score.push_back({s0, s1});
        res->score_launches += 1;

        const uint32_t n_chunks = ctx->table_compressed ? gb * ctx->comp_nb : gb * cpg;
        const uint32_t per_group = ctx->table_compressed ? ctx->comp_nb : cpg;
        if (ctx->table_compressed) {
            RC_TRY(ensure(ctx, ctx->offsets, ((size_t)n_chunks + 1) * 8));
            RC_TRY(scan_u32(ctx, ctx->ucnt.as<uint32_t>(), n_chunks, ctx->offsets.as<uint64_t>()));
            if (total_entries)
                hipLaunchKernelGGL(add_base_kernel, dim3((n_chunks + 1 + 255) / 256), dim3(256), 0, ctx->stream,
                                   ctx->offsets.as<uint64_t>(), (uint64_t)n_chunks + 1, total_entries);
        } else {
            if (positions)
                hipLaunchKernelGGL(count_chunks64_kernel, dim3(n_chunks), dim3(256), 0, ctx->stream,
                                   ctx->table.as<unsigned long long>(), pl.table_size, cpg, ctx->counts.as<uint32_t>());
            else if (ctx->mask_valid)
                hipLaunchKernelGGL(count_chunks_mask_kernel, dim3(n_chunks), dim3(256), 0, ctx->stream,
                                   ctx->mask.as<uint32_t>(), ctx->mask_words, cpg, ctx->counts.as<uint32_t>());
            else
                hipLaunchKernelGGL(count_chunks_kernel, dim3(n_chunks), dim3(256), 0, ctx->stream,
                                   ctx->table.as<uint32_t>(), pl.table_size, cpg, ctx->counts.as<uint32_t>());
            hipLaunchKernelGGL(scan_counts_kernel, dim3(1), dim3(1024), 0, ctx->stream,
                               ctx->counts.as<uint32_t>(), (uint64_t)n_chunks, total_entries, ctx->offsets.as<uint64_t>());
        }
        hipLaunchKernelGGL(gather_offsets_kernel, dim3((gb + 1 + 255) / 256), dim3(256), 0, ctx->stream,
                           ctx->offsets.as<uint64_t>(), per_group, gb + 1, ctx->goff.as<uint64_t>());
        HIP_TRY(ctx, hipGetLastError());
        std::vector<uint64_t> goff((size_t)gb + 1);
        HIP_TRY(ctx, hipMemcpyAsync(goff.data(), ctx->goff.p, ((size_t)gb + 1) * 8, hipMemcpyDeviceToHost, ctx->stream));
        HIP_TRY(ctx, hipStreamSynchronize(ctx->stream));
        for (uint32_t g = 0; g <= gb; ++g) res->offsets[g0 + g] = goff[g];
        const uint64_t new_total = goff[gb];
        if (new_total > res->cap) {
            const size_t new_cap = (g0 + gb >= n_groups) ? (size_t)new_total : (size_t)std::max<uint64_t>(new_total, 2 * res->cap);
            void* grown[3] = {nullptr, nullptr, nullptr};
            for (int a = 0; a < n_arrays; ++a) {
                const hipError_t e = ctx_alloc(ctx, &grown[a], std::max<size_t>(new_cap, 1) * 4);
                if (e != hipSuccess) { for (int b = 0; b < a; ++b) ctx_release(ctx, grown[b]); HIP_TRY(ctx, e); }
            }
            if (total_entries) {
                for (int a = 0; a < n_arrays; ++a)
                    (void)hipMemcpyAsync(grown[a], *arrays[a], total_entries * 4, hipMemcpyDeviceToDevice, ctx->stream);
                (void)hipStreamSynchronize(ctx->stream);
            }
            for (int a = 0; a < n_arrays; ++a) { ctx_release(ctx, *arrays[a]); *arrays[a] = grown[a]; }
            res->cap = new_cap;
        }
        auto write = [&](auto S_) {
            if (ctx->table_compressed)
                hipLaunchKernelGGL(write_group_c_kernel<S_>, dim3(n_chunks), dim3(256), 0, ctx->stream, comp_table(ctx),
                                   pl.table_size, (int)k, ctx->offsets.as<uint64_t>(), res->d_keys, res->d_scores);
            else if (positions)
                hipLaunchKernelGGL(write_chunks_pos_kernel<S_>, dim3(n_chunks), dim3(256), 0, ctx->stream, ctx->table.as<unsigned long long>(),
                                   pl.table_size, cpg, (int)k, pl.nwin, ctx->offsets.as<uint64_t>(), res->d_keys, res->d_scores, res->d_positions);
            else
                hipLaunchKernelGGL(write_chunks_kernel<S_>, dim3(n_chunks), dim3(256), 0, ctx->stream, ctx->table.as<uint32_t>(),
                                   pl.table_size, cpg, (int)k, ctx->offsets.as<uint64_t>(), res->d_keys, res->d_scores);
        };
        if (sigma == 4) write(int_c<4>{}); else write(int_c<20>{});
        HIP_TRY(ctx, hipGetLastError());
        ev_compact.push_back({s1, sw.mark()});
        total_entries = new_total;
    }
    const int t_end = sw.mark();
    HIP_TRY(ctx, hipStreamSynchronize(ctx->stream));
    res->t_total = sw.ms(t_begin, t_end);
    res->t_prefix = sw.ms(t_begin, t_pre);
    for (auto& pr : ev_score) res->t_score += sw.ms(pr.first, pr.second);
    res->t_main = ctx->acc_main_ms; res->t_reduce = ctx->acc_reduce_ms;
// ... 175 lines not shown
        const uint64_t keys_bound = std::max<uint64_t>(1, std::min<uint64_t>(slots, n_total));
        HIP_TRY(ctx, ctx_alloc(ctx, (void**)&db->d_keys, keys_bound * 4));
        HIP_TRY(ctx, ctx_alloc(ctx, (void**)&db->d_key_off, (keys_bound + 1) * 8));
        const uint32_t nbk = (uint32_t)((slots + 1 + 255) / 256);
        if (sigma == 4)
            hipLaunchKernelGGL(merge_write_keys_kernel<4>, dim3(nbk), dim3(256), 0, ctx->stream, total_out, ctx->offsets.as<uint64_t>(),
                               ctx->tmp_b.as<uint64_t>(), slots, owner, P, (int)k, db->d_keys, db->d_key_off);
        else
            hipLaunchKernelGGL(merge_write_keys_kernel<20>, dim3(nbk), dim3(256), 0, ctx->stream, total_out, ctx->offsets.as<uint64_t>(),
                               ctx->tmp_b.as<uint64_t>(), slots, owner, P, (int)k, db->d_keys, db->d_key_off);
        HIP_TRY(ctx, hipGetLastError());
        HIP_TRY(ctx, hipStreamSynchronize(ctx->stream));
        const uint64_t n_keys = h_tot[1];
        db->n_keys = n_keys;
    }
    return IPKGPU_OK;
}

int keymajor_impl(ipkgpu_ctx* ctx, const float* logp_dev, uint32_t n_mats, uint32_t sites, uint32_t sigma, const uint32_t* mat_group,
                  uint32_t k, float log_eps, uint32_t n_owners, uint32_t lead, uint32_t lead_c, ipkgpu_parts** out, bool positions = false,
                  bool pos_owners = false)
{
    if (!ctx) return IPKGPU_ERR_INVALID;
    if (!out) return fail(ctx, IPKGPU_ERR_INVALID, "null out pointer");
    *out = nullptr;
    if (n_owners == 0) return fail(ctx, IPKGPU_ERR_INVALID, "n_owners must be >= 1");
    if (positions && !pos_owners && n_owners != 1) return fail(ctx, IPKGPU_ERR_INVALID, "a positioned database is built for one owner (n_owners = %u): the exchange does not carry positions", n_owners);
    if (positions && !pos_owners && n_mats == 0) return fail(ctx, IPKGPU_ERR_INVALID, "no matrices");
    const uint64_t key_base = lead ? (uint64_t)lead_c * ipow(sigma, (int)(k - lead)) : 0;
    if (n_mats == 0) {
        if (lead == 0 && ((sigma != 4 && sigma != 20) || k < 2 || k > ipkgpu_max_k(sigma))) return fail(ctx, IPKGPU_ERR_INVALID, "unsupported sigma/k");
        HIP_TRY(ctx, hipSetDevice(ctx->device));
        ipkgpu_parts* e = new (std::nothrow) ipkgpu_parts();
        if (!e) return fail(ctx, IPKGPU_ERR_NOMEM, "out of host memory");
        e->ctx = ctx; e->n_owners = n_owners; e->slots = (ipow(sigma, (int)(k - lead)) + n_owners - 1) / n_owners;
        e->lead = lead; e->key_base = key_base; e->sigma = sigma; e->k = k;
        e->owner_off.assign((size_t)n_owners + 1, 0);
        struct EGuard { ipkgpu_parts* r; ~EGuard() { if (r) ipkgpu_parts_free(r); } } eg{e};
        HIP_TRY(ctx, ctx_alloc(ctx, (void**)&e->d_counts, (size_t)n_owners * e->slots * 4));
        HIP_TRY(ctx, ctx_alloc(ctx, (void**)&e->d_entries, 8));
        if (positions) {
            Geometry geo;
            RC_TRY(fill_geometry(ctx, sigma, k, 0, geo));
            if (lead != 0 || geo.xp_nb == 0)
                return fail(ctx, IPKGPU_ERR_INVALID, "no positioned database for sigma=%u k=%u: the call takes the exact partition, which needs more than 64 keys "
                                                     "and no key-range pass", sigma, k);
            HIP_TRY(ctx, ctx_alloc(ctx, (void**)&e->d_positions, 4));
        }
        HIP_TRY(ctx, hipMemsetAsync(e->d_counts, 0, (size_t)n_owners * e->slots * 4, ctx->stream));
        HIP_TRY(ctx, hipStreamSynchronize(ctx->stream));
        eg.r = nullptr;
        *out = e;
        return IPKGPU_OK;
    }
    Plan pl;
    RC_TRY(make_plan(ctx, logp_dev, n_mats, sites, sigma, mat_group, k, log_eps, pl, lead, lead_c, false, positions));
    HIP_TRY(ctx, hipSetDevice(ctx->device));
    if (positions) {
        std::vector<uint32_t> rank(n_mats), seen(pl.n_groups, 0);
        for (uint32_t i = 0; i < n_mats; ++i) rank[i] = seen[pl.slot_of[i]]++;
        const uint32_t most = *std::max_element(seen.begin(), seen.end());
        if ((uint64_t)most * pl.nwin >= 0xFFFFFFFFull) return fail(ctx, IPKGPU_ERR_INVALID, "too many windows per group for the position code (%u matrices x %u windows)", most, pl.nwin);
        RC_TRY(ensure(ctx, ctx->mrank, (size_t)n_mats * 4));
        HIP_TRY(ctx, hipMemcpy(ctx->mrank.p, rank.data(), (size_t)n_mats * 4, hipMemcpyHostToDevice));
        pl.mat_rank = ctx->mrank.as<uint32_t>();
    }
    const uint64_t T = pl.table_size;
    const uint32_t P = n_owners;
    const uint64_t slots = (T + P - 1) / P;
    const uint32_t n_groups = pl.n_groups;

    ipkgpu_parts* parts = new (std::nothrow) ipkgpu_parts();
    if (!parts) return fail(ctx, IPKGPU_ERR_NOMEM, "out of host memory");
    parts->ctx = ctx; parts->n_owners = P; parts->slots = slots;
    parts->lead = lead; parts->key_base = key_base; parts->sigma = sigma; parts->k = k;
    parts->owner_off.assign((size_t)P + 1, 0);
    struct Guard { ipkgpu_parts* r; ~Guard() { if (r) ipkgpu_parts_free(r); } } guard{parts};

    RC_TRY(ensure(ctx, ctx->branch, (size_t)n_groups * 4));
    ctx->h_branch = pl.group_ids;
    HIP_TRY(ctx, hipMemcpyAsync(ctx->branch.p, ctx->h_branch.data(), (size_t)n_groups * 4, hipMemcpyHostToDevice, ctx->stream));

    ctx->acc_main_ms = ctx->acc_reduce_ms = ctx->acc_count_ms = ctx->acc_write_ms = ctx->acc_km_ms = 0;
    Stopwatch sw(ctx->stream, &ctx->events);
    const int t_begin = sw.mark();
    RC_TRY(run_prefix(ctx, pl, logp_dev));
    const int t_pre = sw.mark();
    std::vector<std::pair<int, int>> ev_score, ev_compact, ev_km;
    std::pair<int, int> ev_keys{-1, -1};

    struct Batch { uint32_t* counts = nullptr; uint2* entries = nullptr; uint2* pentries = nullptr; std::vector<uint64_t> owner_off; };
    std::vector<Batch> batches;
    auto free_batches = [&]() { for (auto& b : batches) { ctx_release(ctx, b.counts); ctx_release(ctx, b.entries); ctx_release(ctx, b.pentries); } batches.clear(); };
    struct BGuard { decltype(free_batches)& f; ~BGuard() { f(); } } bguard{free_batches};

    const uint64_t n_slots_all = (uint64_t)P * slots;
    uint32_t gpb_now = (uint32_t)pl.gpb, gb = 0;
    for (uint32_t g0 = 0; g0 < n_groups; g0 += gb) {
        gb = std::min<uint32_t>(gpb_now, n_groups - g0);
        const int s0 = sw.mark();
        const int rcb = score_batch(ctx, pl, logp_dev, g0, gb, &parts->emitted, true);
        if (rcb == IPKGPU_RETRY_SMALLER) { gpb_now = std::max<uint32_t>(1, gb / 2); gb = 0; continue; }
        if (rcb) return rcb;
        const int s1 = sw.mark();
        ev_score.push_back({s0, s1});
        parts->score_launches += 1;

        batches.emplace_back();
        Batch& b = batches.back();
        HIP_TRY(ctx, ctx_alloc(ctx, (void**)&b.counts, n_slots_all * 4));
        HIP_TRY(ctx, hipMemsetAsync(b.counts, 0, n_slots_all * 4, ctx->stream));
        const uint32_t kmc_pass = (uint32_t)std::min<int64_t>(256, std::max<int64_t>(4, ctx->opt_kmc_pass > 0 ? ctx->opt_kmc_pass : IPK_KMC_PASS));
        const bool fast_c = ctx->table_compressed && 64ull * (ctx->mask_words / 2) * 8 < (1ull << 32);
        uint32_t* qpack = nullptr;
        if (fast_c) {
            RC_TRY(ensure(ctx, ctx->qpack, n_slots_all * 4));
            if (gb <= kmc_pass) qpack = ctx->qpack.as<uint32_t>();
        }
        if (ctx->mask_valid && (T + 31) / 32 >= (uint64_t)ctx->num_cu * 1024)
            hipLaunchKernelGGL(km_count_mask_kernel, dim3((uint32_t)(((T + 31) / 32 + 255) / 256)), dim3(256), 0, ctx->stream,
                               ctx->mask.as<uint32_t>(), ctx->mask_words, T, gb, P, slots, b.counts, qpack);
        else if (ctx->mask_valid)
            hipLaunchKernelGGL(km_count_mask_key_kernel, dim3((uint32_t)((T + 255) / 256)), dim3(256), 0, ctx->stream,
                               ctx->mask.as<uint32_t>(), ctx->mask_words, T, gb, P, slots, b.counts, qpack);
        else
            hipLaunchKernelGGL(km_count_kernel, dim3((uint32_t)((T + 255) / 256)), dim3(256), 0, ctx->stream,
                               ctx->table.as<uint32_t>(), T, gb, P, slots, b.counts);
        HIP_TRY(ctx, hipGetLastError());
        RC_TRY(ensure(ctx, ctx->offsets, (n_slots_all + 1) * 8));
        RC_TRY(scan_u32(ctx, b.counts, n_slots_all, ctx->offsets.as<uint64_t>()));
        RC_TRY(ensure(ctx, ctx->goff, ((size_t)P + 1) * 8));
        hipLaunchKernelGGL(gather_offsets_kernel, dim3((P + 1 + 255) / 256), dim3(256), 0, ctx->stream,
                           ctx->offsets.as<uint64_t>(), (uint32_t)slots, P + 1, ctx->goff.as<uint64_t>());
        HIP_TRY(ctx, hipGetLastError());
        b.owner_off.resize((size_t)P + 1);
        const bool rb_ok = P <= RB_OWNERS_MAX;
        uint64_t* h_off = rb_ok ? reinterpret_cast<uint64_t*>(ctx->h_rb) + RB_OWNER_OFF : b.owner_off.data();
        HIP_TRY(ctx, hipMemcpyAsync(h_off, ctx->goff.p, ((size_t)P + 1) * 8, hipMemcpyDeviceToHost, ctx->stream));

        const bool pre_keys = P == 1 && g0 == 0 && gb == n_groups && rb_ok && !(ctx->opt_flags & 64) &&
                              (slots <= (1ull << 24) || ctx->last_entries * 8 >= slots * 12 * 4);
        uint32_t* k_keys = nullptr; uint64_t* k_off = nullptr;
        struct KGuard { ipkgpu_ctx* c; uint32_t*& a; uint64_t*& b; ~KGuard() { ctx_release(c, a); ctx_release(c, b); } } kguard{ctx, k_keys, k_off};
        int kt0 = -1, kt1 = -1;
        if (pre_keys) {
            kt0 = sw.mark();
            RC_TRY(ensure(ctx, ctx->tmp_b, (slots + 1) * 8));
            RC_TRY(scan_nonzero_u32(ctx, b.counts, slots, ctx->tmp_b.as<uint64_t>()));
            HIP_TRY(ctx, hipMemcpyAsync(h_off + P + 1, ctx->tmp_b.as<uint64_t>() + slots, 8, hipMemcpyDeviceToHost, ctx->stream));
            HIP_TRY(ctx, ctx_alloc(ctx, (void**)&k_keys, slots * 4));
            HIP_TRY(ctx, ctx_alloc(ctx, (void**)&k_off, (slots + 1) * 8));
            const uint32_t nbk = (uint32_t)((slots + 1 + 255) / 256);
            if (sigma == 4)
                hipLaunchKernelGGL(merge_write_keys_kernel<4>, dim3(nbk), dim3(256), 0, ctx->stream, b.counts, ctx->tmp_b.as<uint64_t>(),
                                   ctx->offsets.as<uint64_t>(), slots, (uint32_t)key_base, 1u, (int)k, k_keys, k_off);
            else
                hipLaunchKernelGGL(merge_write_keys_kernel<20>, dim3(nbk), dim3(256), 0, ctx->stream, b.counts, ctx->tmp_b.as<uint64_t>(),
                                   ctx->offsets.as<uint64_t>(), slots, 0u, 1u, (int)k, k_keys, k_off);
            HIP_TRY(ctx, hipGetLastError());
            kt1 = sw.mark();
        }

        uint2* w_dst = nullptr; bool w_posv = false;
        auto comp_table_w = [&]() { CompTable c = comp_table(ctx); if (w_posv) c.vaddr = ctx->pvaddr.as<uint64_t>(); return c; };
        auto launch_writer = [&](uint64_t cap_e) -> int {
            uint2* const dst_entries = w_dst ? w_dst : b.entries;
// ... 722 lines not shown
            HIP_TRY(ctx, hipEventSynchronize(ev[j & 1]));
            t_dev += since(tw);
            const auto tf = std::chrono::steady_clock::now();
            const uint64_t nb = rec_off[pieces[j].hi] - rec_off[pieces[j].lo];
            if (!out.put(h_stage[j & 1], nb)) return fail(ctx, IPKGPU_ERR_INVALID, "write failed");
            t_file += since(tf);
            total += nb;
        }
    }
    { const auto t0 = std::chrono::steady_clock::now(); const int rc = fclose(out.f); out.f = nullptr; if (rc != 0) return fail(ctx, IPKGPU_ERR_INVALID, "close failed"); t_file += since(t0); }
    ctx->t_write_total = since(t_begin); ctx->t_write_device = t_dev; ctx->t_write_file = t_file;
    if (bytes_written) *bytes_written = total;
    return IPKGPU_OK;
}

}

namespace {

constexpr size_t SPILL_STAGE = (size_t)64 << 20;

int spill_stage(ipkgpu_ctx* ctx, size_t want)
{
    want = std::min(std::max<size_t>(want, 1 << 16), SPILL_STAGE);
    for (int i = 0; i < 2; ++i)
        if (!ctx->ev_spill[i]) HIP_TRY(ctx, hipEventCreateWithFlags(&ctx->ev_spill[i], hipEventDisableTiming));
    if (ctx->h_spill_cap >= want) return IPKGPU_OK;
    for (int i = 0; i < 2; ++i) { if (ctx->h_spill[i]) (void)hipHostFree(ctx->h_spill[i]); ctx->h_spill[i] = nullptr; }
    ctx->h_spill_cap = 0;
    for (int i = 0; i < 2; ++i) HIP_TRY(ctx, hipHostMalloc(&ctx->h_spill[i], want, hipHostMallocDefault));
    ctx->h_spill_cap = want;
    return IPKGPU_OK;
}

struct SpillSeg { uint64_t at, bytes; const void* src; const void* dev; };

std::string spill_block_path(const char* dir, uint32_t piece, uint32_t owner)
{
    char name[64];
    snprintf(name, sizeof name, "/p%u_b%u.blk", piece, owner);
    return std::string(dir) + name;
}

struct SpillFile {
    std::string path; ipkspill::Head head; uint64_t key_base = 0, entry_base = 0;
};

int spill_check_files(ipkgpu_ctx* ctx, uint32_t sigma, uint32_t k, uint32_t owner, uint32_t n_owners, const char* const* paths, uint32_t n_blocks,
                      uint64_t slots, std::vector<SpillFile>& files)
{
    files.resize(n_blocks);
    uint64_t keys = 0, entries = 0;
    for (uint32_t s = 0; s < n_blocks; ++s) {
        if (!paths[s]) return fail(ctx, IPKGPU_ERR_INVALID, "null path of block %u", s);
        SpillFile& f = files[s];
        f.path = paths[s];
        FILE* fh = fopen(paths[s], "rb");
        if (!fh) return fail(ctx, IPKGPU_ERR_INVALID, "cannot open spill block %s", paths[s]);
        struct stat st;
        const bool stat_ok = fstat(fileno(fh), &st) == 0;
        memset(&f.head, 0, sizeof f.head);
        const size_t got = fread(&f.head, 1, sizeof f.head, fh);
        fclose(fh);
        if (!stat_ok) return fail(ctx, IPKGPU_ERR_INVALID, "cannot stat spill block %s", paths[s]);
        const char* what = got < sizeof f.head ? "shorter than a block's head"
                                               : ipkspill::check_head(f.head, (uint64_t)st.st_size, sigma, k, n_owners, owner, slots);
        if (what) return fail(ctx, IPKGPU_ERR_INVALID, "spill block %s: %s", paths[s], what);
        f.key_base = keys; f.entry_base = entries;
        keys += f.head.n_keys; entries += f.head.n_entries;
    }
    return IPKGPU_OK;
}

}

extern "C" {

int ipkgpu_get_option(const ipkgpu_ctx* ctx, const char* name, int64_t* value)
{
    if (!ctx || !name || !value) return IPKGPU_ERR_INVALID;
    if (!strcmp(name, "workspace_bytes")) { *value = ctx->workspace_bytes; return IPKGPU_OK; }
    if (!strcmp(name, "device_budget_bytes")) { *value = ctx->budget; return IPKGPU_OK; }
    if (!strcmp(name, "last_refused_bytes")) { *value = (int64_t)ctx->refused_need; return IPKGPU_OK; }
    return IPKGPU_ERR_INVALID;
}

int ipkgpu_mem_stats(ipkgpu_ctx* ctx, uint64_t* held, uint64_t* held_peak, int reset_peak)
{
    if (!ctx) return IPKGPU_ERR_INVALID;
    if (held) *held = ctx->held;
    if (held_peak) *held_peak = ctx->held_peak;
    if (reset_peak) ctx->held_peak = ctx->held;
    return IPKGPU_OK;
}

int ipkgpu_parts_spill(ipkgpu_ctx* ctx, ipkgpu_parts* parts, const char* dir, uint32_t piece, uint64_t* bytes_written)
{
    if (!ctx) return IPKGPU_ERR_INVALID;
    if (!parts || parts->ctx != ctx || !dir) return fail(ctx, IPKGPU_ERR_INVALID, "bad argument");
    if (parts->d_positions) return fail(ctx, IPKGPU_ERR_INVALID, "positioned parts are not spilled: the on-disk build keeps no positions (as the reference's, db_builder.cpp:469)");
    if (parts->lead != 0) return fail(ctx, IPKGPU_ERR_INVALID, "key-range parts are not spilled: a key-range pass already bounds the device");
    if (!parts->d_counts || !parts->d_entries) return fail(ctx, IPKGPU_ERR_INVALID, "these parts' arrays have moved into a database");
    HIP_TRY(ctx, hipSetDevice(ctx->device));
    const uint32_t B = parts->n_owners;
    const uint64_t slots = parts->slots, W = ipkspill::bit_words(slots), n_words = (uint64_t)B * W;
    if (W > 0xFFFFFFFFull || (n_words + 3) / 4 > 0x7FFFFFFFull) return fail(ctx, IPKGPU_ERR_INVALID, "too many key slots to spill");
    RC_TRY(ensure(ctx, ctx->sp_bits, n_words * 8));
    RC_TRY(ensure(ctx, ctx->sp_pops, n_words * 4));
    RC_TRY(ensure(ctx, ctx->sp_rank, (n_words + 1) * 8));
    RC_TRY(ensure(ctx, ctx->goff, ((size_t)B + 1) * 8));
    uint32_t* d_big = small_at(ctx, SMALL_REC_BIG);
    HIP_TRY(ctx, hipMemsetAsync(d_big, 0, 4, ctx->stream));
    const uint32_t grid = (uint32_t)((n_words + 3) / 4);
    hipLaunchKernelGGL(spill_bits_kernel, dim3(grid), dim3(256), 0, ctx->stream, parts->d_counts, slots, W, n_words,
                       ctx->sp_bits.as<unsigned long long>(), ctx->sp_pops.as<uint32_t>(), d_big);
    HIP_TRY(ctx, hipGetLastError());
    RC_TRY(scan_u32(ctx, ctx->sp_pops.as<uint32_t>(), n_words, ctx->sp_rank.as<uint64_t>()));
    hipLaunchKernelGGL(gather_offsets_kernel, dim3((B + 1 + 255) / 256), dim3(256), 0, ctx->stream, ctx->sp_rank.as<uint64_t>(), (uint32_t)W, B + 1,
                       ctx->goff.as<uint64_t>());
    HIP_TRY(ctx, hipGetLastError());
    std::vector<uint64_t> key_base((size_t)B + 1);
    uint32_t h_big = 0;
    HIP_TRY(ctx, hipMemcpyAsync(key_base.data(), ctx->goff.p, ((size_t)B + 1) * 8, hipMemcpyDeviceToHost, ctx->stream));
    HIP_TRY(ctx, hipMemcpyAsync(&h_big, d_big, 4, hipMemcpyDeviceToHost, ctx->stream));
    HIP_TRY(ctx, hipStreamSynchronize(ctx->stream));
    if (h_big) return fail(ctx, IPKGPU_ERR_INVALID, "a key with more than %u entries in one piece: a spill block's counts are 16-bit (pieces of at most %u groups)",
                           ipkspill::COUNT_MAX, ipkspill::COUNT_MAX);
    RC_TRY(ensure(ctx, ctx->sp_c16, key_base[B] * 2));
    hipLaunchKernelGGL(spill_pack_kernel, dim3(grid), dim3(256), 0, ctx->stream, parts->d_counts, slots, W, n_words, ctx->sp_rank.as<uint64_t>(),
                       ctx->sp_c16.as<uint16_t>());
    HIP_TRY(ctx, hipGetLastError());

    uint64_t largest = 0;
    for (uint32_t o = 0; o < B; ++o)
        largest = std::max(largest, ipkspill::file_bytes(slots, key_base[o + 1] - key_base[o], parts->owner_off[o + 1] - parts->owner_off[o]));
    RC_TRY(spill_stage(ctx, largest));
    const uint64_t cap = ctx->h_spill_cap;
    struct Chunk { uint32_t owner = 0; uint64_t bytes = 0; bool first = false, last = false, pending = false; } chunk[2];
    FILE* fh = nullptr;
    std::string tmp_path, final_path;
    uint64_t total = 0;
    auto abandon = [&]() { if (fh) { fclose(fh); fh = nullptr; } if (!tmp_path.empty()) (void)remove(tmp_path.c_str()); (void)hipStreamSynchronize(ctx->stream); };
    auto write_chunk = [&](int b) -> int {
        Chunk& c = chunk[b];
        if (!c.pending) return IPKGPU_OK;
        c.pending = false;
        HIP_TRY(ctx, hipEventSynchronize(ctx->ev_spill[b]));
        if (c.first) {
            final_path = spill_block_path(dir, piece, c.owner);
            tmp_path = final_path + ".tmp";
            fh = fopen(tmp_path.c_str(), "wb");
            if (!fh) { const std::string p = tmp_path; tmp_path.clear(); return fail(ctx, IPKGPU_ERR_INVALID, "cannot create %s", p.c_str()); }
            setvbuf(fh, nullptr, _IONBF, 0);
        }
        if (fwrite(ctx->h_spill[b], 1, c.bytes, fh) != c.bytes) return fail(ctx, IPKGPU_ERR_INVALID, "write failed: %s", tmp_path.c_str());
        total += c.bytes;
        if (c.last) {
            const int rc = fclose(fh);
            fh = nullptr;
            if (rc != 0) return fail(ctx, IPKGPU_ERR_INVALID, "close failed: %s", tmp_path.c_str());
            if (rename(tmp_path.c_str(), final_path.c_str()) != 0) return fail(ctx, IPKGPU_ERR_INVALID, "cannot rename %s", tmp_path.c_str());
            tmp_path.clear();
        }
        return IPKGPU_OK;
    };
    uint64_t n_chunks = 0;
// ... 130 lines not shown
```

### ipk_amd/csrc/kernels_quad.hpp

```cpp
#pragma once
#include "kernels_score.hpp"

namespace ipkgpu {

struct QuadNode { int J, H, TH, OFF; uint32_t F, CMUL; };
struct QuadStep { int H, A, B; };

template <int SIGMA, int K>
struct QuadGeo {
    using D = HalvesDD<SIGMA, K>;
    static constexpr int HL = D::HL, HR = D::HR, LA = D::LA, LB = D::LB, RA = D::RA, RB = D::RB;
    static constexpr bool OK = SIGMA == 4 && D::OK && LA >= 2 && LA <= 3 && LB >= 2 && LB <= 3 && RA >= 2 && RA <= 3 && RB >= 2 && RB <= 3;
    static constexpr uint32_t FLA = D::FLA, FLB = D::FLB, FRA = D::FRA, FRB = D::FRB;
    static constexpr uint32_t mulR = ipow(SIGMA, K - K / 2);
    static constexpr uint32_t CW = FLA + FLB + FRA + FRB;
    static constexpr int th_n(int h) { return h == 2 ? 3 : 5; }
    static constexpr int TH0 = 2, TH1 = TH0 + th_n(LA), TH2 = TH1 + th_n(LB), TH3 = TH2 + th_n(RA);
    static constexpr int TH_F = TH3 + th_n(RB);
    static constexpr int PADW = 1;
    static constexpr QuadNode node(int n)
    {
        return n == 0 ? QuadNode{0, LA, TH0, 0, FLA, 1u}
             : n == 1 ? QuadNode{LA, LB, TH1, (int)FLA, FLB, mulR}
             : n == 2 ? QuadNode{HL, RA, TH2, (int)(FLA + FLB), FRA, 1u}
// ... 362 lines not shown
            const float eps_l = eps - (bs[K] - bs[Q::HL]);
            const float eps_r = eps - (bs[Q::HL] - bs[0]);
            o[0] = eps_l; o[1] = eps_r;
            quad_node_thresholds<0, Q::LA>(bs, eps_l - (bs[Q::HL] - bs[Q::LA]), o + Q::node(0).TH);
            quad_node_thresholds<Q::LA, Q::LB>(bs, eps_l - (bs[Q::LA] - bs[0]), o + Q::node(1).TH);
            quad_node_thresholds<Q::HL, Q::RA>(bs, eps_r - (bs[K] - bs[Q::HL + Q::RA]), o + Q::node(2).TH);
            quad_node_thresholds<Q::HL + Q::RA, Q::RB>(bs, eps_r - (bs[Q::HL + Q::RA] - bs[Q::HL]), o + Q::node(3).TH);
        }
        __syncthreads();

        const uint32_t npair = (nw + WPW - 1) / WPW;
        const float* thw = thr + __umul24(wave * WPW + half, (uint32_t)Q::TH_F);
        for (uint32_t pr = wave; pr < npair; pr += NW, thw += WPW * NW * Q::TH_F) {
            const uint32_t wq = pr * WPW;
            const uint32_t wl = wq + half;
            const bool wvalid = wl < nw;
            uint32_t counts[3] = {0, 0, 0};
            wave_lds_sync();
            auto run_step = [&](auto S) {
                constexpr int s = decltype(S)::value;
                if constexpr (s < NST) {
                    const bool valid = wvalid && st_on[s];
                    const uint64_t vmask = ballot64(valid);
                    const uint32_t base = wl * 4 + st_j4[s];
                    constexpr int H = ONEWIN ? Q::step1_h(s) : Q::step(s < Q::NSTEPS ? s : 0).H;
                    quad_step<H>(cols, base, valid, vmask, thw + st_th[s], child + st_off[s], l16, slot, lt16, st_code[s], st_cmul[s], counts[s]);
                }
            };
            run_step(std::integral_constant<int, 0>{});
            run_step(std::integral_constant<int, 1>{});
            run_step(std::integral_constant<int, 2>{});
            wave_lds_sync();
            const uint32_t nwp = min(WPW, nw - wq);

#pragma unroll 1
            for (uint32_t gw = 0; gw < nwp; ++gw) {
                const uint32_t w = wq + gw;
                constexpr int so0 = ONEWIN ? Q::step1_of(0) : Q::step_of(0), so1 = ONEWIN ? Q::step1_of(1) : Q::step_of(1);
                constexpr int so2 = ONEWIN ? Q::step1_of(2) : Q::step_of(2), so3 = ONEWIN ? Q::step1_of(3) : Q::step_of(3);
                constexpr int sl0 = ONEWIN ? Q::slot1_of(0) : Q::slot_of(0), sl1 = ONEWIN ? Q::slot1_of(1) : Q::slot_of(1);
                constexpr int sl2 = ONEWIN ? Q::slot1_of(2) : Q::slot_of(2), sl3 = ONEWIN ? Q::slot1_of(3) : Q::slot_of(3);
                const uint32_t wbase = ONEWIN ? 0u : gw * 32u;
                const uint32_t nla = (uint32_t)__builtin_amdgcn_readlane((int)counts[so0], (int)(wbase + sl0 * 16));
                const uint32_t nlb = (uint32_t)__builtin_amdgcn_readlane((int)counts[so1], (int)(wbase + sl1 * 16));
                const uint32_t nra = (uint32_t)__builtin_amdgcn_readlane((int)counts[so2], (int)(wbase + sl2 * 16));
                const uint32_t nrb = (uint32_t)__builtin_amdgcn_readlane((int)counts[so3], (int)(wbase + sl3 * 16));
                if (nla * nlb * nra * nrb == 0) continue;
                const uint2* cw = child + gw * Q::CW;
                const uint2 *la = cw + Q::node(0).OFF, *lb = cw + Q::node(1).OFF, *ra = cw + Q::node(2).OFF, *rb = cw + Q::node(3).OFF;
                const float eps_l = thr[w * Q::TH_F], eps_r = thr[w * Q::TH_F + 1];
                const uint32_t tl = nla * nlb, tr = nra * nrb;
                uint32_t nL, nR;
                constexpr bool SLICE = ROWLANE;
                constexpr uint32_t SAFE_L = CAPL / Q::FLB, SAFE_R = CAPR / Q::FRB;
                static_assert(SAFE_L >= 1 && SAFE_R >= 1, "a slice of one row of the first child must fit the list");
                const bool one_step = tl <= 64 && tr <= 64;
                uint32_t sla = nla, sra = nra, ia = 0, ir = 0;
                bool keep_l = false;
                for (;;) {
                wave_lds_sync();
                if (one_step) {
                    const float rnl = __builtin_amdgcn_rcpf((float)nlb), rnr = __builtin_amdgcn_rcpf((float)nrb);
                    const uint32_t il = div_small(lane_h, rnl), jl = (uint32_t)(__mul24((int)il, -(int)nlb) + (int)lane);
                    const uint32_t ir = div_small(lane_h, rnr), jr = (uint32_t)(__mul24((int)ir, -(int)nrb) + (int)lane);
                    const uint2 a0 = la[il], b0 = lb[jl], a1 = ra[ir], b1 = rb[jr];
                    const float s0 = __uint_as_float(a0.y) + __uint_as_float(b0.y);
                    const float s1 = __uint_as_float(a1.y) + __uint_as_float(b1.y);
                    const bool v0 = lane < tl, v1 = lane < tr, c0 = s0 > eps_l, c1 = s1 > eps_r;
                    const bool p0 = v0 && c0, p1 = v1 && c1;
                    const uint64_t h0 = ballot64(v0) & ballot64(c0), h1 = ballot64(v1) & ballot64(c1);
                    if (p0) lp[mbcnt(h0)] = make_uint2(a0.x * (Q::FLB * mulR) + b0.x, __float_as_uint(s0));
                    if (p1) rp[mbcnt(h1)] = make_uint2(a1.x * Q::FRB + b1.x, __float_as_uint(s1));
                    nL = (uint32_t)__popcll(h0); nR = (uint32_t)__popcll(h1);
                } else {
                    if (!keep_l)
                        nL = (uint32_t)__builtin_amdgcn_readfirstlane((int)join_to_list(la + ia, min(sla, nla - ia), lb, nlb, eps_l, Q::FLB * mulR, lp, CAPL));
                    if constexpr (SLICE) {
                        if (nL == LIST_OVERFLOW) { sla = SAFE_L; continue; }
                    }
                    nR = nL == LIST_OVERFLOW || nL == 0 ? nL : (uint32_t)__builtin_amdgcn_readfirstlane((int)join_to_list(ra + ir, min(sra, nra - ir), rb, nrb, eps_r, Q::FRB, rp, CAPR));
                    if constexpr (SLICE) {
                        if (nR == LIST_OVERFLOW) { sra = SAFE_R; keep_l = true; continue; }
                    } else if (nL == LIST_OVERFLOW || nR == LIST_OVERFLOW) {
                        if (lane == 0) {
                            const uint32_t qi = atomicAdd(p.ovf_count, 1u);
                            p.ovf_queue[qi] = ((unsigned long long)mat << 32) | (unsigned long long)(t0 + w);
                        }
                        __builtin_amdgcn_wave_barrier();
                        break;
                    }
                }
                if (nL != 0 && nR != 0) {
                wave_lds_sync();
                if (p.flags & 4u) emitted += nL + nR;
                else
                if constexpr (ROWLANE) {
                    constexpr uint32_t CB = 64;
                    static_assert(CB <= CH, "row-per-lane join: a run must fit a chunk");
                    for (uint32_t ib = 0; ib < nL; ib += 64) {
                        const uint2 a = lp[ib + lane];
                        const bool rv = ib + lane < nL;
                        const float ay = rv ? __uint_as_float(a.y) : -__builtin_inff();
                        const uint32_t bk = a.x / TBL;
                        for (uint32_t jb = 0; jb < nR; jb += CB) {
                            const uint32_t nc = min(CB, nR - jb);
                            const uint2* rj = rp + jb;
                            uint32_t cnt = 0;
                            if constexpr (count_only) {
                                for (uint32_t j = 0; j < nc; ++j) emitted += (uint32_t)__popcll(ballot64(ay + __uint_as_float(rj[j].y) > eps));
                            } else {
                                auto count8 = [&](auto NC, uint32_t j0, uint32_t& n, float e) {
                                    constexpr uint32_t N = decltype(NC)::value;
                                    float by[N];
#pragma unroll
                                    for (uint32_t u = 0; u < N; ++u) by[u] = __uint_as_float(rj[j0 + u].y);
#pragma unroll
                                    for (uint32_t u = 0; u < N; ++u) {
                                        const float sj = ay + by[u];
                                        asm("v_cmp_lt_f32_e32 vcc, %2, %1\n\tv_addc_co_u32_e32 %0, vcc, 0, %0, vcc" : "+v"(n) : "v"(sj), "s"(e) : "vcc");
                                    }
                                };
                                uint32_t j0 = 0;
                                for (; j0 + 8 <= nc; j0 += 8) count8(std::integral_constant<uint32_t, 8>{}, j0, cnt, eps);
                                if (j0 + 4 <= nc) { count8(std::integral_constant<uint32_t, 4>{}, j0, cnt, eps); j0 += 4; }
                                for (; j0 < nc; ++j0) count8(std::integral_constant<uint32_t, 1>{}, j0, cnt, eps);
                            }
                            if constexpr (!count_only) {
                                const bool has = cnt != 0;
                                if (ballot64(has) == 0) continue;
                                if (p.flags & 16u) { emitted += cnt; continue; }
                                unsigned long long got;
                                asm volatile("" : "=v"(got));
                                if (has) got = atomicAdd(&app.st[bk], (unsigned long long)cnt);
                                uint32_t pre = (uint32_t)got, id = (uint32_t)(got >> 32);
                                for (;;) {
                                    uint64_t X = ballot64(has && pre <= CH && pre + cnt > CH);
                                    if (X == 0) break;
                                    do {
                                        const int ls = __ffsll((long long)X) - 1;
                                        const uint32_t bb = (uint32_t)__builtin_amdgcn_readlane((int)bk, ls);
                                        const uint32_t xv = (uint32_t)__builtin_amdgcn_readlane((int)pre, ls);
                                        const uint32_t xid = (uint32_t)__builtin_amdgcn_readlane((int)id, ls);
                                        const uint32_t nid = app.roll_at(bb, xv);
                                        const bool sel = has && bk == bb && id == xid && pre >= xv;
                                        id = sel ? nid : id;
                                        pre = sel ? pre - xv : pre;
                                        X &= X - 1ull;
                                    } while (X);
                                }
                                unsigned long long run = reinterpret_cast<unsigned long long>(p.pool) + (((unsigned long long)id * CH + pre) << 3);
                                if (p.flags & 2u) continue;
                                auto emit8 = [&](auto NC, uint32_t j0) {
                                    constexpr uint32_t N = decltype(NC)::value;
                                    uint2 b[N];
#pragma unroll
                                    for (uint32_t u = 0; u < N; ++u) b[u] = rj[j0 + u];
#pragma unroll
                                    for (uint32_t u = 0; u < N; ++u)
                                        store_pair_if_gt(run, a.x + b[u].x, ay + __uint_as_float(b[u].y), eps);
                                };
                                uint32_t j0 = 0;
                                for (; j0 + 8 <= nc; j0 += 8) emit8(std::integral_constant<uint32_t, 8>{}, j0);
                                if (j0 + 4 <= nc) { emit8(std::integral_constant<uint32_t, 4>{}, j0); j0 += 4; }
                                for (; j0 < nc; ++j0) emit8(std::integral_constant<uint32_t, 1>{}, j0);
                            }
                        }
                    }
                } else
                for (uint32_t jb = 0; jb < nR; jb += 64) {
                    const uint32_t nRb = min(64u, nR - jb);
// ... 110 lines not shown
```

### ipk_amd/csrc/kernels_score.hpp

```cpp
#pragma once
#include <type_traits>
#include "dcla_device.hpp"

namespace ipkgpu {


template <int SIGMA, int M>
__global__ __launch_bounds__(256) void prefix_max_kernel(const float* __restrict__ logp, uint32_t n_mats, uint32_t sites,
                                                         float* __restrict__ best)
{
    constexpr int CH = 2048 / M;
    constexpr int ROW = CH + 4;
    static_assert(M == 1 || M == 2 || M == 4 || M == 8, "matrices per workgroup");
    __shared__ __align__(16) float cmbuf[2][M][ROW];
    const uint32_t mat0 = blockIdx.x * M;
    const uint32_t mv = min((uint32_t)M, n_mats - mat0);
    const bool chain = threadIdx.x < mv;
    const uint32_t my = mat0 + (chain ? threadIdx.x : 0u);
    float* b = best + (size_t)my * (sites + 1);
    if (chain) b[0] = 0.0f;
    float carry = 0.0f;
    auto maxima = [&](uint32_t c0, float (*cmw)[ROW], uint32_t t0, uint32_t nt) {
        const uint32_t n = min((uint32_t)CH, sites - c0);
        for (uint32_t mm = 0; mm < mv; ++mm) {
// ... 238 lines not shown
        const uint32_t inv_seq = POS ? 0xFFFFFFFFu - (p.mat_rank[mat] * p.nwin + start) : 0u;
        const uint2 *L = scratch, *R = scratch + Geo<SIGMA, K / 2, CAPF>::CAPH;
        if (wave == 0) {
            WinCtx c{cols, best, 0};
            uint32_t nL = 0, nR = 0;
            const bool fits = build_halves<SIGMA, K, CAPF>(c, p.eps, scratch, L, nL, R, nR);
            if (!fits) { nL = 0; nR = 0; if (lane == 0 && p.big_ovf) atomicOr(p.big_ovf, 1u); }
            if (lane == 0) { sh_n[0] = nL; sh_n[1] = nR; }
        }
        __syncthreads();
        const uint32_t nL = sh_n[0], nR = sh_n[1];
        if (nL == 0 || nR == 0) continue;
        uint32_t cnt = 0;
        constexpr uint32_t OVF_ROWS = 4;
        const bool no_put = (p.flags & 1u) != 0 || IPK_OVF_NOPUT;
        for (uint32_t jb = 0; jb < nR; jb += 64) {
            const uint32_t j = jb + lane;
            const bool valid = j < nR;
            uint2 b = make_uint2(0, 0);
            if (valid) b = R[j];
            const float by = __uint_as_float(b.y);
            for (uint32_t i0 = wave; i0 < nL; i0 += OVF_NW * OVF_ROWS) {
                uint2 a[OVF_ROWS];
#pragma unroll
                for (uint32_t u = 0; u < OVF_ROWS; ++u) a[u] = L[min(i0 + u * OVF_NW, nL - 1)];
#pragma unroll
                for (uint32_t u = 0; u < OVF_ROWS; ++u) {
                    const float s = __uint_as_float(a[u].y) + by;
                    const bool pass = valid && (i0 + u * OVF_NW < nL) && (s > p.eps);
                    if (pass && !no_put) {
                        const uint32_t idx = a[u].x * mulR + b.x;
                        if constexpr (POS) PutScorePos{tab64, inv_seq}(idx, __float_as_uint(s));
                        else {
#if IPK_OVF_UNCOND_OR
                            atomicMax(tab + idx, enc_score_bits(__float_as_uint(s)));
                            if (p.mask) atomicOr(p.mask + (size_t)p.mat_slot[mat] * p.mask_words + (idx >> 5), 1u << (idx & 31u));
#elif IPK_OVF_PEEK
                            const uint32_t enc = enc_score_bits(__float_as_uint(s));
                            if (__builtin_nontemporal_load(tab + idx) < enc) {
                                const uint32_t old = atomicMax(tab + idx, enc);
                                if (old == 0u && p.mask)
                                    atomicOr(p.mask + (size_t)p.mat_slot[mat] * p.mask_words + (idx >> 5), 1u << (idx & 31u));
                            }
#else
                            const uint32_t old = atomicMax(tab + idx, enc_score_bits(__float_as_uint(s)));
                            if (old == 0u && p.mask)
                                atomicOr(p.mask + (size_t)p.mat_slot[mat] * p.mask_words + (idx >> 5), 1u << (idx & 31u));
#endif
                        }
                    }
                    cnt += (uint32_t)__popcll(__ballot(pass));
                }
            }
        }
        emitted += cnt;
    }
    if (lane == 0 && emitted) atomicAdd(p.emitted, emitted);
}

#ifndef IPK_CH512_TBL
#define IPK_CH512_TBL 0u
#endif
template <uint32_t TBL> constexpr uint32_t chunk_pairs() { return (TBL == 16384 || TBL == IPK_CH512_TBL) ? 512u : 256u; }
inline uint32_t chunk_pairs_rt(uint32_t tbl) { return (tbl == 16384 || tbl == IPK_CH512_TBL) ? 512u : 256u; }
constexpr uint32_t CHUNK_NONE = 0xFFFFFFFFu;
constexpr uint32_t ALLOC_BATCH = 32;
constexpr uint32_t SUB = 1;

struct StreamParams {
    const float* logp;
    const float* best;
    const uint32_t* gm_off;
    const uint32_t* gm_list;
    uint32_t sites, nwin, tiles_per_mat, S;
    float eps;
    uint2* pool;
    uint32_t pool_cap;
    uint32_t* pool_next;
    unsigned long long* desc;
    uint32_t* pool_ovf;
    unsigned long long* emitted;
    unsigned long long* ovf_queue;
    uint32_t* ovf_count;
    const uint32_t* mat_slot;
    uint32_t flags;
    uint32_t pre_chunks;
    uint32_t* tile_next = nullptr;
    uint32_t* big_ovf = nullptr;
};

__device__ __constant__ uint32_t RCP16[65] = {
    0, 65536, 32768, 21846, 16384, 13108, 10923, 9363, 8192, 7282, 6554, 5958, 5462, 5042, 4682, 4370, 4096,
    3856, 3641, 3450, 3277, 3121, 2979, 2850, 2731, 2622, 2521, 2428, 2341, 2260, 2185, 2115, 2048,
    1986, 1928, 1873, 1821, 1772, 1725, 1681, 1639, 1599, 1561, 1525, 1490, 1457, 1425, 1395, 1366,
    1338, 1311, 1286, 1261, 1237, 1214, 1192, 1171, 1150, 1130, 1111, 1093, 1075, 1058, 1041, 1024};

template <int SIGMA, int K>
struct HalvesDD {
    static constexpr int HL = K / 2, HR = K - K / 2;
    static constexpr int LA = HL / 2, LB = HL - LA, RA = HR / 2, RB = HR - RA;
    static constexpr bool OK = ipow(SIGMA, HL) > 64 && ipow(SIGMA, LB) <= 64 && ipow(SIGMA, RB) <= 64;
    static constexpr uint32_t FLA = ipow(SIGMA, LA), FLB = ipow(SIGMA, LB), FRA = ipow(SIGMA, RA), FRB = ipow(SIGMA, RB);
};
template <int SIGMA, int K, int CAP>
constexpr uint32_t stream_wave_scratch()
{
    using D = HalvesDD<SIGMA, K>;
    if constexpr (D::OK)
        return Geo<SIGMA, D::HL, CAP>::CAPH + Geo<SIGMA, D::HR, CAP>::CAPH + D::FLA + D::FLB + D::FRA + D::FRB;
    else
        return wave_scratch_entries<SIGMA, K, CAP>();
}

template <int SIGMA, int K, int CAP>
__device__ __forceinline__ bool build_halves_dd(const WinCtx& c, float eps, uint2* scratch,
                                                const uint2*& Lp, uint32_t& nL, const uint2*& Rp, uint32_t& nR)
{
    using D = HalvesDD<SIGMA, K>;
    constexpr int HL = D::HL, HR = D::HR, LA = D::LA, LB = D::LB, RA = D::RA, RB = D::RB;
    using GL = Geo<SIGMA, HL, CAP>;
    using GR = Geo<SIGMA, HR, CAP>;
    const uint32_t lane = lane_id();
    const float* bs = c.best + c.w;
    const float eps_l = eps - (bs[K] - bs[HL]);
    const float eps_r = eps - (bs[HL] - bs[0]);
    const float eps_la = eps_l - (bs[HL] - bs[LA]);
    const float eps_lb = eps_l - (bs[LA] - bs[0]);
    const float eps_ra = eps_r - (bs[K] - bs[HL + RA]);
    const float eps_rb = eps_r - (bs[HL + RA] - bs[HL]);
    uint2* lp = scratch;
    uint2* rp = lp + GL::CAPH;
    uint2* la = rp + GR::CAPH;
    uint2* lb = la + D::FLA;
    uint2* ra = lb + D::FLB;
    uint2* rb = ra + D::FRA;
    Lp = lp; Rp = rp; nL = 0; nR = 0;

    float sla = 0.f, slb = 0.f, sra = 0.f, srb = 0.f;
    bool pla = false, plb = false, pra = false, prb = false;
    if (lane < D::FLA) pla = Direct<SIGMA, 0, LA>::eval(c, eps_la, lane, sla);
    if (lane < D::FLB) plb = Direct<SIGMA, LA, LB>::eval(c, eps_lb, lane, slb);
    if (lane < D::FRA) pra = Direct<SIGMA, HL, RA>::eval(c, eps_ra, lane, sra);
    if (lane < D::FRB) prb = Direct<SIGMA, HL + RA, RB>::eval(c, eps_rb, lane, srb);
    const uint64_t mla = __ballot(pla), mlb = __ballot(plb), mra = __ballot(pra), mrb = __ballot(prb);
    if (mla == 0 || mlb == 0 || mra == 0 || mrb == 0) return true;
    if (pla) la[mbcnt(mla)] = make_uint2(lane, __float_as_uint(sla));
    if (plb) lb[mbcnt(mlb)] = make_uint2(lane, __float_as_uint(slb));
    if (pra) ra[mbcnt(mra)] = make_uint2(lane, __float_as_uint(sra));
    if (prb) rb[mbcnt(mrb)] = make_uint2(lane, __float_as_uint(srb));
    const uint32_t nla = (uint32_t)__popcll(mla), nlb = (uint32_t)__popcll(mlb);
    const uint32_t nra = (uint32_t)__popcll(mra), nrb = (uint32_t)__popcll(mrb);
    wave_lds_sync();
    const uint32_t tl = nla * nlb, tr = nra * nrb;
    uint32_t cl, cr;
    if (tl <= 64 && tr <= 64) {
        const uint32_t il = (lane * RCP16[nlb]) >> 16, jl = lane - il * nlb;
        const uint32_t ir = (lane * RCP16[nrb]) >> 16, jr = lane - ir * nrb;
        uint2 a0 = make_uint2(0, 0), b0 = a0, a1 = a0, b1 = a0;
        if (lane < tl) { a0 = la[il]; b0 = lb[jl]; }
        if (lane < tr) { a1 = ra[ir]; b1 = rb[jr]; }
        const float s0 = __uint_as_float(a0.y) + __uint_as_float(b0.y);
        const float s1 = __uint_as_float(a1.y) + __uint_as_float(b1.y);
        const bool p0 = (lane < tl) && (s0 > eps_l);
        const bool p1 = (lane < tr) && (s1 > eps_r);
        const uint64_t m0 = __ballot(p0), m1 = __ballot(p1);
        if (p0) lp[mbcnt(m0)] = make_uint2(a0.x * D::FLB + b0.x, __float_as_uint(s0));
        if (p1) rp[mbcnt(m1)] = make_uint2(a1.x * D::FRB + b1.x, __float_as_uint(s1));
        cl = (uint32_t)__popcll(m0); cr = (uint32_t)__popcll(m1);
    } else {
        cl = join_to_list(la, nla, lb, nlb, eps_l, D::FLB, lp, GL::CAPH);
        if (cl == LIST_OVERFLOW) return false;
        if (cl == 0) return true;
        cr = join_to_list(ra, nra, rb, nrb, eps_r, D::FRB, rp, GR::CAPH);
        if (cr == LIST_OVERFLOW) return false;
    }
    nL = cl; nR = cr;
    wave_lds_sync();
    return true;
}

template <uint32_t TBL, uint32_t NB>
struct Appender {
    static constexpr uint32_t CH = chunk_pairs<TBL>();
    const StreamParams& p;
    uint32_t* cbase;
    uint32_t* cfill;
    uint32_t g;
    uint32_t chunk_next = 0, chunk_end = 0;

    __device__ __forceinline__ uint32_t roll(uint32_t bb)
    {
        const uint32_t lane = lane_id();
        if (chunk_next == chunk_end) {
            uint32_t base = 0;
            if (lane == 0) base = atomicAdd(p.pool_next, ALLOC_BATCH);
            chunk_next = (uint32_t)__builtin_amdgcn_readfirstlane((int)base);
            chunk_end = chunk_next + ALLOC_BATCH;
        }
        uint32_t nid = chunk_next++;
        if (nid >= p.pool_cap) { if (lane == 0) atomicOr(p.pool_ovf, 1u); nid = CHUNK_NONE; }
        wave_lds_sync();
        const uint32_t old_id = cbase[bb];
        wave_lds_sync();
        if (lane == 0) {
            if (old_id != CHUNK_NONE) p.desc[old_id] = ((unsigned long long)(g * NB + bb / SUB) << 32) | (unsigned long long)CH;
            cbase[bb] = nid;
            cfill[bb] = cfill[bb] - CH;
        }
        wave_lds_sync();
        return nid;
    }

    __device__ __forceinline__ void append2(bool pass0, uint32_t idx0, uint32_t sb0, bool pass1, uint32_t idx1, uint32_t sb1)
    {
        const uint32_t sub = lane_id() & (SUB - 1);
        const uint32_t bk0 = pass0 ? (idx0 / TBL) * SUB + sub : 0u, bk1 = pass1 ? (idx1 / TBL) * SUB + sub : 0u;
        uint32_t slot0 = 0, slot1 = 0, cb0 = CHUNK_NONE, cb1 = CHUNK_NONE;
        if (pass0) slot0 = atomicAdd(&cfill[bk0], 1u);
        if (pass1) slot1 = atomicAdd(&cfill[bk1], 1u);
        if (pass0) cb0 = cbase[bk0];
        if (pass1) cb1 = cbase[bk1];
        const bool st = !(p.flags & 1u);
        if (pass0 && slot0 < CH && cb0 != CHUNK_NONE && st) p.pool[(size_t)cb0 * CH + slot0] = make_uint2(idx0, sb0);
        if (pass1 && slot1 < CH && cb1 != CHUNK_NONE && st) p.pool[(size_t)cb1 * CH + slot1] = make_uint2(idx1, sb1);
        const bool o0 = pass0 && slot0 >= CH, o1 = pass1 && slot1 >= CH;
        uint64_t ovf0 = __ballot(o0), ovf1 = __ballot(o1);
        while (ovf0 | ovf1) {
            uint32_t bb;
            if (ovf0) bb = (uint32_t)__builtin_amdgcn_readlane((int)bk0, (int)(__ffsll((long long)ovf0) - 1));
            else      bb = (uint32_t)__builtin_amdgcn_readlane((int)bk1, (int)(__ffsll((long long)ovf1) - 1));
            const bool h0 = o0 && bk0 == bb, h1 = o1 && bk1 == bb;
            const uint64_t m0 = __ballot(h0), m1 = __ballot(h1);
            const uint32_t nid = roll(bb);
            if (h0 && nid != CHUNK_NONE && st) p.pool[(size_t)nid * CH + (slot0 - CH)] = make_uint2(idx0, sb0);
            if (h1 && nid != CHUNK_NONE && st) p.pool[(size_t)nid * CH + (slot1 - CH)] = make_uint2(idx1, sb1);
            ovf0 &= ~m0; ovf1 &= ~m1;
        }
    }
};

template <int SIGMA, int K, int CAP, int TW, int NW, uint32_t TBL>
__global__ __launch_bounds__(NW * 64) __attribute__((amdgpu_num_sgpr(80))) void score_stream_kernel(StreamParams p)
{
    extern __shared__ __align__(16) unsigned char smem[];
    constexpr uint32_t CH = chunk_pairs<TBL>();
    using TG = TileGeo<SIGMA, K, TW>;
    constexpr uint32_t T = ipow(SIGMA, K);
    constexpr uint32_t NB = (T + TBL - 1) / TBL;
    constexpr uint32_t WS = stream_wave_scratch<SIGMA, K, CAP>();
    float* cols = reinterpret_cast<float*>(smem);
    float* best = cols + TG::COLS_F;
    uint2* scratch_all = reinterpret_cast<uint2*>(smem + TG::HEAD_BYTES);
    uint32_t* state_all = reinterpret_cast<uint32_t*>(scratch_all + (size_t)NW * WS);

    const uint32_t lane = lane_id(), wave = threadIdx.x >> 6;
    const uint32_t g = blockIdx.x / p.S, seg = blockIdx.x - g * p.S;
    const uint32_t m0 = p.gm_off[g], nm = p.gm_off[g + 1] - m0;
    const uint32_t total_tiles = nm * p.tiles_per_mat;
    const uint32_t t_lo = (uint32_t)(((uint64_t)total_tiles * seg) / p.S);
    const uint32_t t_hi = (uint32_t)(((uint64_t)total_tiles * (seg + 1)) / p.S);

    uint2* scratch = scratch_all + (size_t)wave * WS;
    uint32_t* cbase = state_all + (size_t)wave * 2 * NB * SUB;
    uint32_t* cfill = cbase + NB * SUB;
    for (uint32_t b = lane; b < NB * SUB; b += 64) { cbase[b] = CHUNK_NONE; cfill[b] = CH; }
    Appender<TBL, NB> app{p, cbase, cfill, g};
    unsigned long long emitted = 0;
    constexpr uint32_t mulR = ipow(SIGMA, K - K / 2);

    for (uint32_t t = t_lo; t < t_hi; ++t) {
        const uint32_t q = t / p.tiles_per_mat, tile = t - q * p.tiles_per_mat;
        const uint32_t mat = p.gm_list[m0 + q];
        const uint32_t t0 = tile * TW;
        const uint32_t nw = min((uint32_t)TW, p.nwin - t0);
        const uint32_t ncol = nw + K - 1;
        __syncthreads();
        {
            const float4* src = reinterpret_cast<const float4*>(p.logp + ((size_t)mat * p.sites + t0) * SIGMA);
            float4* dst = reinterpret_cast<float4*>(cols);
            const uint32_t n4 = ncol * (SIGMA / 4);
            for (uint32_t i = threadIdx.x; i < n4; i += NW * 64) dst[i] = src[i];
            const float* bsrc = p.best + (size_t)mat * (p.sites + 1) + t0;
            for (uint32_t i = threadIdx.x; i <= ncol; i += NW * 64) best[i] = bsrc[i];
        }
        __syncthreads();
        for (uint32_t w = wave; w < nw; w += NW) {
            WinCtx c{cols, best, w};
            const uint2 *L, *R;
            uint32_t nL, nR;
            static_assert(!Geo<SIGMA, K, CAP>::DIRECT, "stream variant needs k with sigma^k > 64");
            bool ok;
            if constexpr (HalvesDD<SIGMA, K>::OK) ok = build_halves_dd<SIGMA, K, CAP>(c, p.eps, scratch, L, nL, R, nR);
            else ok = build_halves<SIGMA, K, CAP>(c, p.eps, scratch, L, nL, R, nR);
            if (!ok) {
                if (lane == 0) {
                    const uint32_t qi = atomicAdd(p.ovf_count, 1u);
                    p.ovf_queue[qi] = ((unsigned long long)mat << 32) | (unsigned long long)(t0 + w);
                }
                continue;
            }
            if (nL == 0 || nR == 0) continue;
            if (p.flags & 4u) { emitted += nL + nR; continue; }
            uint32_t cnt = 0;
            if (nR < 64) {
                const uint32_t total = nL * nR;
                const uint32_t M = RCP16[nR];
                const uint32_t q64 = (64u * M) >> 16, r64 = 64u - q64 * nR;
                uint32_t bi = 0, bj = 0;
                for (uint32_t base = 0; base < total; base += 128) {
                    uint32_t bi1 = bi + q64, bj1 = bj + r64;
                    if (bj1 >= nR) { bj1 -= nR; ++bi1; }
                    const uint32_t ta = bj + lane, tb = bj1 + lane;
                    const uint32_t qa = (ta * M) >> 16, qb = (tb * M) >> 16;
                    const bool va = base + lane < total, vb = base + 64 + lane < total;
                    uint2 a0 = make_uint2(0, 0), b0 = a0, a1 = a0, b1 = a0;
                    if (va) { a0 = L[bi + qa]; b0 = R[ta - qa * nR]; }
                    if (vb) { a1 = L[bi1 + qb]; b1 = R[tb - qb * nR]; }
                    const float s0 = __uint_as_float(a0.y) + __uint_as_float(b0.y);
                    const float s1 = __uint_as_float(a1.y) + __uint_as_float(b1.y);
                    const bool p0 = va && (s0 > p.eps), p1 = vb && (s1 > p.eps);
                    cnt += (uint32_t)__popcll(__ballot(p0)) + (uint32_t)__popcll(__ballot(p1));
                    if (!(p.flags & 2u))
                        app.append2(p0, a0.x * mulR + b0.x, __float_as_uint(s0), p1, a1.x * mulR + b1.x, __float_as_uint(s1));
                    bi = bi1 + q64; bj = bj1 + r64;
                    if (bj >= nR) { bj -= nR; ++bi; }
                }
            } else {
                for (uint32_t i = 0; i < nL; ++i) {
                    const uint2 a = L[i];
                    for (uint32_t jb = 0; jb < nR; jb += 128) {
                        const uint32_t ja = jb + lane, jc = jb + 64 + lane;
                        const bool va = ja < nR, vb = jc < nR;
                        uint2 b0 = make_uint2(0, 0), b1 = b0;
                        if (va) b0 = R[ja];
                        if (vb) b1 = R[jc];
                        const float s0 = __uint_as_float(a.y) + __uint_as_float(b0.y);
                        const float s1 = __uint_as_float(a.y) + __uint_as_float(b1.y);
                        const bool p0 = va && (s0 > p.eps), p1 = vb && (s1 > p.eps);
                        cnt += (uint32_t)__popcll(__ballot(p0)) + (uint32_t)__popcll(__ballot(p1));
                        if (!(p.flags & 2u))
                            app.append2(p0, a.x * mulR + b0.x, __float_as_uint(s0), p1, a.x * mulR + b1.x, __float_as_uint(s1));
                    }
                }
            }
            emitted += cnt;
        }
    }
    wave_lds_sync();
    for (uint32_t b = lane; b < NB * SUB; b += 64) {
        const uint32_t id = cbase[b];
        if (id != CHUNK_NONE) p.desc[id] = ((unsigned long long)(g * NB + b / SUB) << 32) | (unsigned long long)min(cfill[b], CH);
    }
    if (lane == 0 && emitted) atomicAdd(p.emitted, emitted);
}

template <int SIGMA, int K, uint32_t TBL>
__global__ __launch_bounds__(OVF_NW * 64) void score_overflow_stream_kernel(StreamParams p)
{
    extern __shared__ __align__(16) unsigned char smem[];
    constexpr uint32_t CH = chunk_pairs<TBL>();
    constexpr int CAPF = big_capf<SIGMA, K>();
    constexpr uint32_t T = ipow(SIGMA, K);
    constexpr uint32_t NB = (T + TBL - 1) / TBL;
    using TG = TileGeo<SIGMA, K, 1>;
    __shared__ uint32_t sh_n[2];
    float* cols = reinterpret_cast<float*>(smem);
    float* best = cols + TG::COLS_F;
    uint2* scratch = reinterpret_cast<uint2*>(smem + TG::HEAD_BYTES);
    uint32_t* state_all = reinterpret_cast<uint32_t*>(scratch + wave_scratch_entries<SIGMA, K, CAPF>());
    const uint32_t n = *p.ovf_count;
    const uint32_t lane = lane_id(), wave = threadIdx.x >> 6;
    uint32_t* cbase = state_all + (size_t)wave * 2 * NB * SUB;
    uint32_t* cfill = cbase + NB * SUB;
    for (uint32_t b = lane; b < NB * SUB; b += 64) { cbase[b] = CHUNK_NONE; cfill[b] = CH; }
    Appender<TBL, NB> app{p, cbase, cfill, 0u};
    bool have_group = false;
    unsigned long long emitted = 0;
    constexpr uint32_t mulR = ipow(SIGMA, K - K / 2);
    auto close_chunks = [&]() {
        wave_lds_sync();
        for (uint32_t b = lane; b < NB * SUB; b += 64) {
            const uint32_t id = cbase[b];
            if (id != CHUNK_NONE) p.desc[id] = ((unsigned long long)(app.g * NB + b / SUB) << 32) | (unsigned long long)min(cfill[b], CH);
            cbase[b] = CHUNK_NONE; cfill[b] = CH;
        }
        wave_lds_sync();
    };
    const uint32_t per = (n + gridDim.x - 1) / gridDim.x;
    const uint32_t q_lo = min(n, blockIdx.x * per), q_hi = min(n, q_lo + per);
    for (uint32_t q = q_lo; q < q_hi; ++q) {
        const unsigned long long e = p.ovf_queue[q];
        const uint32_t g = (uint32_t)(e >> 42), mat = (uint32_t)(e >> 21) & 0x1FFFFFu, start = (uint32_t)e & 0x1FFFFFu;
        if (have_group && g != app.g) close_chunks();
        app.g = g; have_group = true;
        __syncthreads();
        const float* src = p.logp + ((size_t)mat * p.sites + start) * SIGMA;
        for (uint32_t i = threadIdx.x; i < K * SIGMA; i += OVF_NW * 64) cols[i] = src[i];
        const float* bsrc = p.best + (size_t)mat * (p.sites + 1) + start;
        for (uint32_t i = threadIdx.x; i <= K; i += OVF_NW * 64) best[i] = bsrc[i];
        __syncthreads();
        const uint2 *L = scratch, *R = scratch + Geo<SIGMA, K / 2, CAPF>::CAPH;
        if (wave == 0) {
            WinCtx c{cols, best, 0};
            uint32_t nL = 0, nR = 0;
            const bool fits = build_halves<SIGMA, K, CAPF>(c, p.eps, scratch, L, nL, R, nR);
            if (!fits) { nL = 0; nR = 0; if (lane == 0 && p.big_ovf) atomicOr(p.big_ovf, 1u); }
            if (lane == 0) { sh_n[0] = nL; sh_n[1] = nR; }
        }
        __syncthreads();
        const uint32_t nL = sh_n[0], nR = sh_n[1];
        if (nL == 0 || nR == 0) continue;
        uint32_t cnt = 0;
        for (uint32_t i = wave; i < nL; i += OVF_NW) {
            const uint2 a = L[i];
            for (uint32_t jb = 0; jb < nR; jb += 128) {
                const uint32_t ja = jb + lane, jc = jb + 64 + lane;
                const bool va = ja < nR, vb = jc < nR;
                uint2 b0 = make_uint2(0, 0), b1 = b0;
                if (va) b0 = R[ja];
                if (vb) b1 = R[jc];
                const float s0 = __uint_as_float(a.y) + __uint_as_float(b0.y);
                const float s1 = __uint_as_float(a.y) + __uint_as_float(b1.y);
                const bool p0 = va && (s0 > p.eps), p1 = vb && (s1 > p.eps);
                cnt += (uint32_t)__popcll(__ballot(p0)) + (uint32_t)__popcll(__ballot(p1));
                app.append2(p0, a.x * mulR + b0.x, __float_as_uint(s0), p1, a.x * mulR + b1.x, __float_as_uint(s1));
            }
        }
        emitted += cnt;
    }
    if (have_group) close_chunks();
    if (lane == 0 && emitted) atomicAdd(p.emitted, emitted);
}

__global__ __launch_bounds__(256) void ovf_group_keys_kernel(const unsigned long long* __restrict__ queue, uint32_t n,
                                                             const uint32_t* __restrict__ mat_slot,
                                                             unsigned long long* __restrict__ out)
{
    const uint32_t i = blockIdx.x * 256 + threadIdx.x;
    if (i >= n) return;
    const unsigned long long e = queue[i];
    const uint32_t mat = (uint32_t)(e >> 32), start = (uint32_t)e;
    out[i] = ((unsigned long long)mat_slot[mat] << 42) | ((unsigned long long)mat << 21) | (unsigned long long)start;
}

__global__ __launch_bounds__(256) void chunk_hist_kernel(const unsigned long long* __restrict__ desc, uint32_t n,
                                                         uint32_t* __restrict__ cnt, unsigned long long* __restrict__ pairs,
                                                         uint32_t* __restrict__ gb_pairs ,
                                                         const uint32_t* __restrict__ n_dev = nullptr)
{
    __shared__ unsigned long long wsum[4];
    unsigned long long c = 0;
    if (n_dev) n = min(n, *n_dev);
    for (uint32_t i = blockIdx.x * 256 + threadIdx.x; i < n; i += gridDim.x * 256) {
        const unsigned long long d = desc[i];
        if ((uint32_t)d != 0u) {
            atomicAdd(&cnt[(uint32_t)(d >> 32)], 1u);
            if (gb_pairs) atomicAdd(&gb_pairs[(uint32_t)(d >> 32)], (uint32_t)d);
        }
        c += (uint32_t)d;
    }
    if (pairs) {
        for (int o = 32; o > 0; o >>= 1) c += __shfl_down(c, o, 64);
        if (lane_id() == 0) wsum[threadIdx.x >> 6] = c;
        __syncthreads();
        if (threadIdx.x == 0) {
            const unsigned long long t = wsum[0] + wsum[1] + wsum[2] + wsum[3];
            if (t) atomicAdd(pairs, t);
        }
    }
}
__global__ __launch_bounds__(256) void chunk_scatter_kernel(const unsigned long long* __restrict__ desc, uint32_t n,
                                                            const uint64_t* __restrict__ off, uint32_t* __restrict__ cur,
                                                            uint2* __restrict__ list, const uint32_t* __restrict__ n_dev = nullptr)
{
    if (n_dev) n = min(n, *n_dev);
    for (uint32_t i = blockIdx.x * 256 + threadIdx.x; i < n; i += gridDim.x * 256) {
        const unsigned long long d = desc[i];
        if ((uint32_t)d == 0u) continue;
        const uint32_t gb = (uint32_t)(d >> 32);
        list[off[gb] + atomicAdd(&cur[gb], 1u)] = make_uint2(i, (uint32_t)d);
    }
}

constexpr uint32_t SMALL_EMITTED = 0;
constexpr uint32_t SMALL_OVF_COUNT = 16;
constexpr uint32_t SMALL_POOL_NEXT = 32;
constexpr uint32_t SMALL_POOL_OVF = 36;
constexpr uint32_t SMALL_BIG_OVF = 44;
constexpr uint32_t SMALL_OVF_EMITTED = 48;
constexpr uint32_t SMALL_XP_TOO_BIG = 56;
constexpr uint32_t SMALL_REC_BIG = 60;
constexpr uint32_t SMALL_BYTES = 64;

__global__ void small_reset_kernel(uint32_t* __restrict__ small, uint32_t pre_chunks, uint32_t* __restrict__ tile_next, uint32_t n_groups,
                                   uint32_t first_tile)
{
    const uint32_t i = blockIdx.x * blockDim.x + threadIdx.x;
    if (i < SMALL_XP_TOO_BIG / 4) small[i] = i == SMALL_POOL_NEXT / 4 ? pre_chunks : 0u;
    if (tile_next && i < n_groups) tile_next[i] = first_tile;
}

__device__ __forceinline__ void store_slice_mask(const uint32_t* tab, uint32_t nslots, uint32_t* mask_words, uint32_t nthreads)
{
    const uint32_t lane = lane_id(), wave = threadIdx.x >> 6, nwv = nthreads >> 6;
    const uint32_t nblk = (nslots + 63) / 64;
    const uint32_t bpw = (nblk + nwv - 1) / nwv;
    const uint32_t b_lo = min(nblk, wave * bpw), b_hi = min(nblk, b_lo + bpw);
    for (uint32_t b0 = b_lo; b0 < b_hi; b0 += 64) {
        const uint32_t nb = min(64u, b_hi - b0);
        uint64_t mine = 0;
#pragma unroll 4
        for (uint32_t j = 0; j < nb; ++j) {
            const uint32_t c = (b0 + j) * 64;
            const uint32_t v = (c + lane < nslots) ? tab[c + lane] : 0u;
            const uint64_t m = __ballot(v != 0u);
            if (lane == j) mine = m;
        }
        if (lane < nb) *reinterpret_cast<uint2*>(mask_words + 2 * (b0 + lane)) = make_uint2((uint32_t)mine, (uint32_t)(mine >> 32));
    }
}

__global__ __launch_bounds__(256) void comp_slice_room_kernel(const uint32_t* __restrict__ gb_pairs, uint32_t n_gb, uint32_t NB, uint64_t T,
                                                              uint32_t TBL, uint32_t* __restrict__ room)
{
    const uint32_t i = blockIdx.x * 256 + threadIdx.x;
    if (i >= n_gb) return;
    const uint32_t b = i % NB;
    const uint32_t nslots = (uint32_t)min((uint64_t)TBL, T - (uint64_t)b * TBL);
    room[i] = (min(gb_pairs[i], nslots) + 1u) / 2u;
}

#ifndef IPK_RB_ABL
#define IPK_RB_ABL 0
#endif
#ifndef IPK_COMPACT
#define IPK_COMPACT 0
#endif
template <uint32_t LANE>
__device__ __forceinline__ void writelane_imm(uint32_t& v, uint32_t s)
{
    asm("s_nop 1\n\tv_writelane_b32 %0, %1, %2" : "+v"(v) : "s"(s), "n"(LANE));
}
template <uint32_t LANE>
__device__ __forceinline__ void writelane64_imm(uint32_t& vlo, uint32_t& vhi, uint64_t s)
{
    asm("s_nop 1\n\tv_writelane_b32 %0, %2, %4\n\tv_writelane_b32 %1, %3, %4"
        : "+v"(vlo), "+v"(vhi) : "s"((uint32_t)s), "s"((uint32_t)(s >> 32)), "n"(LANE));
}
template <uint32_t N, class F, uint32_t... I>
__device__ __forceinline__ void static_for_impl(F&& f, std::integer_sequence<uint32_t, I...>) { (f(std::integral_constant<uint32_t, I>{}), ...); }
template <uint32_t N, class F>
__device__ __forceinline__ void static_for(F&& f) { static_for_impl<N>(f, std::make_integer_sequence<uint32_t, N>{}); }

template <uint32_t TBL, int NT> constexpr uint32_t comp_bpw() { return ((TBL + 63) / 64 + NT / 64 - 1) / (NT / 64); }
template <uint32_t TBL, int NT> constexpr uint32_t comp_padded_slots() { return comp_bpw<TBL, NT>() * (NT / 64) * 64; }
template <uint32_t TBL, int NT, bool ZERO = false, bool REREAD = false>
__device__ __forceinline__ void compress_slice(uint32_t* tab, uint32_t nslots, uint32_t* vals, uint32_t* mrow, uint32_t* rrow,
                                               uint64_t* arow, uint32_t* ucnt_gb)
{
    constexpr uint32_t NWV = NT / 64, BPW = comp_bpw<TBL, NT>(), PAD = comp_padded_slots<TBL, NT>();
    static_assert(BPW <= 64, "one lane per block of the wave");
    uint32_t* wtot = tab + PAD;
    const uint32_t lane = lane_id(), wave = (uint32_t)__builtin_amdgcn_readfirstlane((int)(threadIdx.x >> 6));
    const uint32_t nblk = (nslots + 63) / 64;
    uint32_t* wb = tab + wave * (BPW * 64) + lane;
    uint32_t vr[REREAD ? 1 : BPW];
    uint32_t mine = 0;
    if constexpr (REREAD) {
#pragma unroll
        for (uint32_t j = 0; j < BPW; ++j) mine += (uint32_t)__popcll(__ballot(wb[j * 64] != 0u));
    } else {
#pragma unroll
        for (uint32_t j = 0; j < BPW; ++j) vr[j] = wb[j * 64];
#pragma unroll
        for (uint32_t j = 0; j < BPW; ++j) mine += (uint32_t)__popcll(__ballot(vr[j] != 0u));
    }
    if (lane == 0) wtot[wave] = mine;
    __syncthreads();
    uint32_t base = 0, all = 0;
#pragma unroll
    for (uint32_t w = 0; w < NWV; ++w) { const uint32_t t = wtot[w]; if (w < wave) base += t; all += t; }
    base = (uint32_t)__builtin_amdgcn_readfirstlane((int)base);
// ... 709 lines not shown
```

Measured before the change: 131.8 billion.

## Replace sorted overflow queue with per-group pooled big-list kernel launched unconditionally

Overflow windows are now queued into per-group slots with a per-group counter, so no radix sort or host readback is needed. A new pooled big-list kernel is always launched right after pass 1, with gb*ovf_parts blocks that share per-bucket chunk state in LDS through CAS. This removes the host synchronisation and the fallback overflow launch, and lets speculation skip waiting unconditionally. The cost is an always-on extra launch, workgroup-level atomics, and extra pool slack reserved for open chunks.

```diff
diff --git a/ipk_amd/csrc/ipkgpu.hip b/ipk_amd/csrc/ipkgpu.hip
--- a/ipk_amd/csrc/ipkgpu.hip
+++ b/ipk_amd/csrc/ipkgpu.hip
@@ -90,7 +90,7 @@
     int64_t opt_rounds = 0;
     int64_t opt_pool_limit = 0;
     int64_t opt_pool_chunks = 0;
-    DevBuf table, best, ovfq, counts, offsets, goff, idx, branch, scan_sums, scan_boff, tmp_a, tmp_b, tmp_c;
+    DevBuf table, best, ovfq, ovfg, counts, offsets, goff, idx, branch, scan_sums, scan_boff, tmp_a, tmp_b, tmp_c;
     DevBuf pool, desc, gbcnt, gboff, gbcur, clist, gm, tile_next;
     DevBuf ptrs;
     DevBuf sp_bits, sp_pops, sp_rank, sp_c16;
@@ -121,11 +121,12 @@
     uint32_t* h_rb = nullptr;
     EventPool events;
     bool spec_skip_wait = false;
+    uint64_t biglist_windows = 0;
     uint64_t pool_want_min = 0;
     struct Pending {
         bool active = false;
         std::unique_ptr<Stopwatch> sw; int ev_a = -1, ev_b = -1, ev_c = -1, ev_d = -1;
-        uint64_t cap = 0, max_chunks = 0, windows = 0; uint32_t gb = 0; bool pool_ovf_ok = false, use_quad = false;
+        uint64_t cap = 0, max_chunks = 0; uint32_t gb = 0;
     } pend;
     uint64_t last_entries = 0; uint32_t last_gb = 0;
     double t_write_total = 0, t_write_device = 0, t_write_file = 0;
@@ -341,7 +342,7 @@
 
 static std::vector<DevBuf*> all_workspaces(ipkgpu_ctx* ctx)
 {
-    return {&ctx->table, &ctx->best, &ctx->ovfq, &ctx->counts, &ctx->offsets, &ctx->goff, &ctx->idx,
+    return {&ctx->table, &ctx->best, &ctx->ovfq, &ctx->ovfg, &ctx->counts, &ctx->offsets, &ctx->goff, &ctx->idx,
             &ctx->branch, &ctx->scan_sums, &ctx->scan_boff, &ctx->tmp_a, &ctx->tmp_b, &ctx->tmp_c,
             &ctx->pool, &ctx->desc, &ctx->gbcnt, &ctx->gboff, &ctx->gbcur, &ctx->clist, &ctx->gm, &ctx->tile_next, &ctx->mask,
             &ctx->rank, &ctx->vaddr, &ctx->ucnt, &ctx->qpack, &ctx->xstart, &ctx->pcounts, &ctx->ptrs,
@@ -563,22 +564,20 @@
 }
 
 template <int SIGMA, int K>
-int launch_stream_overflow(ipkgpu_ctx* ctx, const StreamParams& sp)
+int launch_biglist_pool(ipkgpu_ctx* ctx, const StreamParams& sp, uint32_t gb)
 {
     constexpr uint32_t TBL = stream_tbl<SIGMA, K>();
     if constexpr (TBL == 0 || ipow(SIGMA, K - K / 2) <= (uint32_t)fast_cap<SIGMA, K>()) {
-        (void)ctx; (void)sp;
+        (void)ctx; (void)sp; (void)gb;
         return IPKGPU_OK;
     } else {
         constexpr uint32_t NB = (uint32_t)((ipow(SIGMA, K) + TBL - 1) / TBL);
-        constexpr size_t lds = TileGeo<SIGMA, K, 1>::HEAD_BYTES + (size_t)wave_scratch_entries<SIGMA, K, big_capf<SIGMA, K>()>() * 8 +
-                               (size_t)OVF_NW * 2 * NB * SUB * 4;
-        static_assert(lds + 64 <= 160 * 1024, "big-list (stream) LDS budget");
-        auto kern = score_overflow_stream_kernel<SIGMA, K, TBL>;
+        constexpr size_t lds = TileGeo<SIGMA, K, 1>::HEAD_BYTES + (size_t)wave_scratch_entries<SIGMA, K, big_capf<SIGMA, K>()>() * 8 + (size_t)NB * 8;
+        static_assert(lds + 64 <= 160 * 1024, "big-list (pooled) LDS budget");
+        auto kern = score_biglist_pool_kernel<SIGMA, K, TBL>;
         if (lds > 64 * 1024)
             HIP_TRY(ctx, hipFuncSetAttribute(reinterpret_cast<const void*>(kern), hipFuncAttributeMaxDynamicSharedMemorySize, (int)lds));
-        const uint32_t per_cu = (uint32_t)std::max<size_t>(1, std::min<size_t>(32 / OVF_NW, (160 * 1024) / (lds + 64)));
-        hipLaunchKernelGGL(kern, dim3(ctx->num_cu * per_cu), dim3(OVF_NW * 64), lds, ctx->stream, sp);
+        hipLaunchKernelGGL(kern, dim3(gb * sp.ovf_parts), dim3(OVF_NW * 64), lds, ctx->stream, sp);
         HIP_TRY(ctx, hipGetLastError());
         return IPKGPU_OK;
     }
@@ -659,6 +658,12 @@
 #define IPK_QONEWIN12 1
 #endif
 template <int SIGMA, int K> constexpr bool quad_onewin() { return K >= 11 && IPK_QONEWIN12 != 0 && quad_rowlane<SIGMA, K>(); }
+template <int SIGMA, int K> constexpr bool stream_biglist(bool use_quad)
+{
+    if (stream_tbl<SIGMA, K>() == 0 || ipow(SIGMA, K - K / 2) <= (uint32_t)fast_cap<SIGMA, K>()) return false;
+    if constexpr (quad_ok<SIGMA, K>()) { if (use_quad && quad_rowlane<SIGMA, K>()) return false; }
+    return true;
+}
 template <int SIGMA, int K> size_t quad_lds()
 {
     if constexpr (!quad_ok<SIGMA, K>()) return 0;
@@ -834,6 +839,7 @@
     bool quad = false;
     uint32_t quad_nw = NW, quad_tw = TW;
     size_t quad_lds = 0;
+    bool stream_biglist = false, quad_biglist = false;
     uint32_t xp_nb = 0, xp_tbl = 0;
     size_t xp_lds = 0;
 };
@@ -847,6 +853,7 @@
             g.stream_nw = stream_nw<S_, K_>(); g.stream_tw = stream_tw<S_, K_>(); g.stream_lds = stream_lds<S_, K_>();
             g.quad = quad_ok<S_, K_>();
             g.quad_nw = quad_nw<S_, K_>(); g.quad_tw = quad_tw<S_, K_>(); g.quad_lds = quad_lds<S_, K_>();
+            g.stream_biglist = stream_biglist<S_, K_>(false); g.quad_biglist = stream_biglist<S_, K_>(true);
             return IPKGPU_OK;
         }));
     return with_xp_shape(ctx, sigma, k, lead, [&](auto S_, auto K_, auto KK_) {
@@ -883,9 +890,6 @@
 
 constexpr int IPKGPU_RETRY_SMALLER = 100;
 constexpr int IPKGPU_RETRY_AGAIN = 101;
-#ifndef IPK_OVF_POOL_RATIO
-#define IPK_OVF_POOL_RATIO 500
-#endif
 
 enum class PassKind { tiles, stream, quad, xp };
 struct Pass {
@@ -1133,7 +1137,8 @@
     ctx->pool_want_min = 0;
     memcpy(&ctx->emitted_host, ctx->h_rb + SMALL_EMITTED / 4, 8);
     ctx->emitted_fetched = true;
-    ctx->spec_skip_wait = !(n_ovf > 0 && (uint64_t)n_ovf * IPK_OVF_POOL_RATIO >= pd.windows && pd.pool_ovf_ok);
+    ctx->biglist_windows += n_ovf;
+    ctx->spec_skip_wait = true;
     if (sw) { ctx->acc_main_ms += sw->ms(pd.ev_a, pd.ev_b); ctx->acc_reduce_ms += sw->ms(pd.ev_c, pd.ev_d); }
     return IPKGPU_OK;
 }
@@ -1247,8 +1252,10 @@
         return rc ? rc : check_capped(ctx, pl.k, p);
     }
 
-    const bool pool_ovf_ok = gb < (1u << 22) && n_mats < (1u << 21) && pl.nwin < (1u << 21);
-    bool s_compress = pool_ovf_ok && ps.compress;
+    bool s_compress = ps.compress;
+    RC_TRY(ensure(ctx, ctx->ovfg, (size_t)gb * 4));
+    const bool biglist = use_quad ? pl.geo.quad_biglist : pl.geo.stream_biglist;
+    const uint32_t ovf_parts = biglist ? (uint32_t)std::max<uint64_t>(1, (uint64_t)ctx->num_cu * 4 / gb) : 0u;
     const uint32_t NBK = pl.geo.stream_nb, TBL = pl.geo.stream_tbl;
     const uint32_t SNW = use_quad ? pl.geo.quad_nw : pl.geo.stream_nw;
     const uint32_t STW = use_quad ? pl.geo.quad_tw : pl.geo.stream_tw;
@@ -1276,6 +1283,7 @@
         HIP_TRY(ctx, hipMemcpyAsync(ctx->tmp_a.p, both.data(), both.size() * 4, hipMemcpyHostToDevice, ctx->stream));
         HIP_TRY(ctx, hipMemsetAsync(p.emitted, 0, 8, ctx->stream));
         HIP_TRY(ctx, hipMemsetAsync(p.ovf_count, 0, 4, ctx->stream));
+        HIP_TRY(ctx, hipMemsetAsync(ctx->ovfg.p, 0, (size_t)n_s * 4, ctx->stream));
         StreamParams ss;
         ss.logp = logp_dev; ss.best = ctx->best.as<float>();
         ss.gm_off = ctx->tmp_a.as<uint32_t>(); ss.gm_list = ctx->tmp_a.as<uint32_t>() + n_s + 1;
@@ -1284,6 +1292,7 @@
         ss.eps = pl.eps;
         ss.pool = nullptr; ss.pool_cap = 0; ss.pool_next = nullptr; ss.desc = nullptr; ss.pool_ovf = nullptr; ss.pre_chunks = 0;
         ss.emitted = p.emitted; ss.ovf_queue = p.ovf_queue; ss.ovf_count = p.ovf_count; ss.mat_slot = p.mat_slot;
+        ss.ovf_gcount = ctx->ovfg.as<uint32_t>();
         ss.flags = 2u;
         RC_TRY(pass1(ss, n_s * ss.S, true));
         unsigned long long se = 0; uint32_t so = 0;
@@ -1295,7 +1304,7 @@
         if (s_windows) ctx->pairs_per_window = std::max(1.0, ((double)se + (double)so * cap_pairs) / (double)s_windows * 1.15);
     }
     const double ppw_est = ctx->pairs_per_window > 0 ? ctx->pairs_per_window : 256.0;
-    if (!s_compress && pool_ovf_ok && ctx->opt_variant == 0 && pl.table_size >= (1u << 16) &&
+    if (!s_compress && ctx->opt_variant == 0 && pl.table_size >= (1u << 16) &&
         (double)windows * ppw_est < 0.5 * (double)gb * (double)pl.table_size)
         s_compress = true;
     if (!s_compress) {
@@ -1326,12 +1335,12 @@
     uint64_t max_chunks = std::min<uint64_t>(0xFFFFFFF0ull, (uint64_t)(free_b + ctx->pool.cap + ctx->desc.cap) * 9 / 10 / (CH * 8 + 8));
     if (ctx->opt_pool_limit > 0) max_chunks = std::min<uint64_t>(max_chunks, (uint64_t)ctx->opt_pool_limit / (CH * 8 + 8));
     const double ppw = ctx->pairs_per_window > 0 ? ctx->pairs_per_window : 256.0;
-    const uint64_t ovf_waves = (uint64_t)ctx->num_cu * 4 * OVF_NW;
-    const uint64_t slack = 2 * (n_waves + ovf_waves) * NBK * SUB + (n_waves + ovf_waves) * ALLOC_BATCH + 1024;
+    const uint64_t ovf_open = (uint64_t)gb * ovf_parts * (NBK + (uint64_t)OVF_NW * BIG_ALLOC_BATCH);
+    const uint64_t slack = 2 * n_waves * NBK * SUB + n_waves * ALLOC_BATCH + ovf_open + 1024;
     uint64_t want = (uint64_t)((double)windows * ppw * 1.25 / CH) + slack;
     {
         const uint64_t have = std::min<uint64_t>(std::max<uint64_t>(ctx->pool.cap / (CH * 8), 1) - 1, ctx->desc.cap / 8);
-        const uint64_t need = (uint64_t)((double)windows * ppw * 1.1 / CH) + (n_waves + ovf_waves) * (NBK * SUB + ALLOC_BATCH) + 1024;
+        const uint64_t need = (uint64_t)((double)windows * ppw * 1.1 / CH) + n_waves * (NBK * SUB + ALLOC_BATCH) + ovf_open + 1024;
         if (have >= need) want = have;
     }
     want = std::max<uint64_t>(want, ctx->pool_want_min);
@@ -1359,7 +1368,7 @@
             d_tile_next = ctx->tile_next.as<uint32_t>();
         }
         hipLaunchKernelGGL(small_reset_kernel, dim3((std::max<uint32_t>(gb, SMALL_XP_TOO_BIG / 4) + 255) / 256), dim3(256), 0, ctx->stream,
-                           reinterpret_cast<uint32_t*>(ctx->small), pre_chunks, d_tile_next, gb, S);
+                           reinterpret_cast<uint32_t*>(ctx->small), pre_chunks, d_tile_next, gb, S, ctx->ovfg.as<uint32_t>());
         HIP_TRY(ctx, hipGetLastError());
         HIP_TRY(ctx, hipMemsetAsync(ctx->desc.p, 0, cap * 8, ctx->stream));
 
@@ -1371,6 +1380,7 @@
         sp.pool = ctx->pool.as<uint2>(); sp.pool_cap = (uint32_t)cap; sp.pool_next = d_pool_next;
         sp.desc = ctx->desc.as<unsigned long long>(); sp.pool_ovf = d_pool_ovf;
         sp.emitted = p.emitted; sp.ovf_queue = p.ovf_queue; sp.ovf_count = p.ovf_count; sp.mat_slot = p.mat_slot;
+        sp.ovf_gcount = ctx->ovfg.as<uint32_t>(); sp.ovf_parts = ovf_parts; sp.big_ovf = p.big_ovf;
         sp.flags = (uint32_t)(ctx->opt_flags);
         sp.pre_chunks = pre_chunks;
         sp.tile_next = d_tile_next;
@@ -1379,33 +1389,14 @@
         const int ev_a = sw.mark();
         RC_TRY(pass1(sp, n_wg, false));
         const int ev_b = sw.mark();
+        if (ovf_parts) {
+            StreamParams so = sp;
+            if (use_quad) so.emitted = small_at<unsigned long long>(ctx, SMALL_OVF_EMITTED);
+            RC_TRY(with_sigma_k(ctx, pl.sigma, pl.k, [&](auto S_, auto K_) { return launch_biglist_pool<S_, K_>(ctx, so, gb); }));
+        }
         const bool spec = ctx->spec_skip_wait && !s_compress && !(ctx->opt_flags & 64);
-        uint32_t n_ovf = 0;
         uint32_t h[2] = {0, 0};
         if (!spec) {
-            HIP_TRY(ctx, hipMemcpyAsync(ctx->h_rb, ctx->small, SMALL_BYTES, hipMemcpyDeviceToHost, ctx->stream));
-            HIP_TRY(ctx, hipStreamSynchronize(ctx->stream));
-            n_ovf = ctx->h_rb[SMALL_OVF_COUNT / 4]; h[0] = ctx->h_rb[SMALL_POOL_NEXT / 4]; h[1] = ctx->h_rb[SMALL_POOL_OVF / 4];
-        }
-        const bool ovf_in_pool = n_ovf > 0 && ((uint64_t)n_ovf * IPK_OVF_POOL_RATIO >= windows || s_compress) && pool_ovf_ok;
-        if (ovf_in_pool) {
-            RC_TRY(ensure(ctx, ctx->tmp_a, (size_t)n_ovf * 8));
-            RC_TRY(ensure(ctx, ctx->tmp_b, (size_t)n_ovf * 8));
-            hipLaunchKernelGGL(ovf_group_keys_kernel, dim3((n_ovf + 255) / 256), dim3(256), 0, ctx->stream,
-                               p.ovf_queue, n_ovf, p.mat_slot, ctx->tmp_a.as<unsigned long long>());
-            HIP_TRY(ctx, hipGetLastError());
-            size_t tmp_bytes = 0;
-            HIP_TRY(ctx, rocprim::radix_sort_keys(nullptr, tmp_bytes, ctx->tmp_a.as<unsigned long long>(), ctx->tmp_b.as<unsigned long long>(),
-                                                  (size_t)n_ovf, 0, 64, ctx->stream));
-            RC_TRY(ensure(ctx, ctx->tmp_c, tmp_bytes));
-            HIP_TRY(ctx, rocprim::radix_sort_keys(ctx->tmp_c.p, tmp_bytes, ctx->tmp_a.as<unsigned long long>(), ctx->tmp_b.as<unsigned long long>(),
-                                                  (size_t)n_ovf, 0, 64, ctx->stream));
-            StreamParams so = sp;
-            so.ovf_queue = ctx->tmp_b.as<unsigned long long>();
-            if (use_quad) so.emitted = small_at<unsigned long long>(ctx, SMALL_OVF_EMITTED);
-            RC_TRY(with_sigma_k(ctx, pl.sigma, pl.k, [&](auto S_, auto K_) { return launch_stream_overflow<S_, K_>(ctx, so); }));
-        }
-        if (ovf_in_pool) {
             HIP_TRY(ctx, hipMemcpyAsync(ctx->h_rb, ctx->small, SMALL_BYTES, hipMemcpyDeviceToHost, ctx->stream));
             HIP_TRY(ctx, hipStreamSynchronize(ctx->stream));
             h[0] = ctx->h_rb[SMALL_POOL_NEXT / 4]; h[1] = ctx->h_rb[SMALL_POOL_OVF / 4];
@@ -1458,8 +1449,6 @@
             return launch_stream_pass2<S_, K_>(ctx, (uint32_t)n_gb, pl.table_size, ctx->table.as<uint32_t>(), s_compress);
         }));
         const int ev_d = sw.mark();
-        if ((spec || n_ovf > 0) && !ovf_in_pool)
-            RC_TRY(with_sigma_k(ctx, pl.sigma, pl.k, [&](auto S_, auto K_) { return launch_overflow<S_, K_, false>(ctx, p); }));
         if (s_compress) {
             ctx->table_compressed = true; ctx->comp_own_vals = true;
             ctx->comp_nb = NBK; ctx->comp_stride = 1; ctx->comp_tbl = TBL;
@@ -1470,7 +1459,7 @@
         ipkgpu_ctx::Pending& pd = ctx->pend;
         pd.sw.reset(sw_own.release());
         pd.ev_a = ev_a; pd.ev_b = ev_b; pd.ev_c = ev_c; pd.ev_d = ev_d;
-        pd.cap = cap; pd.max_chunks = max_chunks; pd.windows = windows; pd.gb = gb; pd.pool_ovf_ok = pool_ovf_ok; pd.use_quad = use_quad;
+        pd.cap = cap; pd.max_chunks = max_chunks; pd.gb = gb;
         pd.active = true;
         if (defer) return IPKGPU_OK;
         HIP_TRY(ctx, hipStreamSynchronize(ctx->stream));
@@ -1597,6 +1586,7 @@
     RC_TRY(ensure(ctx, ctx->goff, (size_t)(pl.gpb + 1) * 8));
 
     ctx->acc_main_ms = ctx->acc_reduce_ms = ctx->acc_count_ms = ctx->acc_write_ms = ctx->acc_km_ms = 0;
+    ctx->biglist_windows = 0;
     Stopwatch sw(ctx->stream, &ctx->events);
     const int t_begin = sw.mark();
     RC_TRY(run_prefix(ctx, pl, logp_dev));
@@ -1938,6 +1928,7 @@
     HIP_TRY(ctx, hipMemcpyAsync(ctx->branch.p, ctx->h_branch.data(), (size_t)n_groups * 4, hipMemcpyHostToDevice, ctx->stream));
 
     ctx->acc_main_ms = ctx->acc_reduce_ms = ctx->acc_count_ms = ctx->acc_write_ms = ctx->acc_km_ms = 0;
+    ctx->biglist_windows = 0;
     Stopwatch sw(ctx->stream, &ctx->events);
     const int t_begin = sw.mark();
     RC_TRY(run_prefix(ctx, pl, logp_dev));
@@ -2826,6 +2817,7 @@
     if (!strcmp(name, "workspace_bytes")) { *value = ctx->workspace_bytes; return IPKGPU_OK; }
     if (!strcmp(name, "device_budget_bytes")) { *value = ctx->budget; return IPKGPU_OK; }
     if (!strcmp(name, "last_refused_bytes")) { *value = (int64_t)ctx->refused_need; return IPKGPU_OK; }
+    if (!strcmp(name, "last_biglist_windows")) { *value = (int64_t)ctx->biglist_windows; return IPKGPU_OK; }
     return IPKGPU_ERR_INVALID;
 }
 
diff --git a/ipk_amd/csrc/kernels_quad.hpp b/ipk_amd/csrc/kernels_quad.hpp
--- a/ipk_amd/csrc/kernels_quad.hpp
+++ b/ipk_amd/csrc/kernels_quad.hpp
@@ -468,10 +468,7 @@
                     if constexpr (SLICE) {
                         if (nR == LIST_OVERFLOW) { sra = SAFE_R; keep_l = true; continue; }
                     } else if (nL == LIST_OVERFLOW || nR == LIST_OVERFLOW) {
-                        if (lane == 0) {
-                            const uint32_t qi = atomicAdd(p.ovf_count, 1u);
-                            p.ovf_queue[qi] = ((unsigned long long)mat << 32) | (unsigned long long)(t0 + w);
-                        }
+                        if (lane == 0) queue_big_window(p, g, m0, mat, t0 + w);
                         __builtin_amdgcn_wave_barrier();
                         break;
                     }
diff --git a/ipk_amd/csrc/kernels_score.hpp b/ipk_amd/csrc/kernels_score.hpp
--- a/ipk_amd/csrc/kernels_score.hpp
+++ b/ipk_amd/csrc/kernels_score.hpp
@@ -344,6 +344,8 @@
     unsigned long long* emitted;
     unsigned long long* ovf_queue;
     uint32_t* ovf_count;
+    uint32_t* ovf_gcount = nullptr;
+    uint32_t ovf_parts = 0;
     const uint32_t* mat_slot;
     uint32_t flags;
     uint32_t pre_chunks;
@@ -441,6 +443,13 @@
     return true;
 }
 
+__device__ __forceinline__ void queue_big_window(const StreamParams& p, uint32_t g, uint32_t m0, uint32_t mat, uint32_t start)
+{
+    const uint32_t qi = atomicAdd(&p.ovf_gcount[g], 1u);
+    p.ovf_queue[(size_t)m0 * p.nwin + qi] = ((unsigned long long)mat << 32) | (unsigned long long)start;
+    atomicAdd(p.ovf_count, 1u);
+}
+
 template <uint32_t TBL, uint32_t NB>
 struct Appender {
     static constexpr uint32_t CH = chunk_pairs<TBL>();
@@ -555,10 +564,7 @@
             if constexpr (HalvesDD<SIGMA, K>::OK) ok = build_halves_dd<SIGMA, K, CAP>(c, p.eps, scratch, L, nL, R, nR);
             else ok = build_halves<SIGMA, K, CAP>(c, p.eps, scratch, L, nL, R, nR);
             if (!ok) {
-                if (lane == 0) {
-                    const uint32_t qi = atomicAdd(p.ovf_count, 1u);
-                    p.ovf_queue[qi] = ((unsigned long long)mat << 32) | (unsigned long long)(t0 + w);
-                }
+                if (lane == 0) queue_big_window(p, g, m0, mat, t0 + w);
                 continue;
             }
             if (nL == 0 || nR == 0) continue;
@@ -616,45 +622,39 @@
     if (lane == 0 && emitted) atomicAdd(p.emitted, emitted);
 }
 
+constexpr uint32_t BIG_ALLOC_BATCH = 8;
+
 template <int SIGMA, int K, uint32_t TBL>
-__global__ __launch_bounds__(OVF_NW * 64) void score_overflow_stream_kernel(StreamParams p)
+__global__ __launch_bounds__(OVF_NW * 64) void score_biglist_pool_kernel(StreamParams p)
 {
     extern __shared__ __align__(16) unsigned char smem[];
     constexpr uint32_t CH = chunk_pairs<TBL>();
     constexpr int CAPF = big_capf<SIGMA, K>();
     constexpr uint32_t T = ipow(SIGMA, K);
     constexpr uint32_t NB = (T + TBL - 1) / TBL;
+    constexpr uint32_t mulR = ipow(SIGMA, K - K / 2);
+    static_assert(TBL % mulR == 0, "a row of the final join must stay inside one bucket");
+    static_assert(CH >= 64, "a step's run must fit a chunk");
+    constexpr uint32_t ROWS_PER_BUCKET = TBL / mulR;
     using TG = TileGeo<SIGMA, K, 1>;
     __shared__ uint32_t sh_n[2];
     float* cols = reinterpret_cast<float*>(smem);
     float* best = cols + TG::COLS_F;
     uint2* scratch = reinterpret_cast<uint2*>(smem + TG::HEAD_BYTES);
-    uint32_t* state_all = reinterpret_cast<uint32_t*>(scratch + wave_scratch_entries<SIGMA, K, CAPF>());
-    const uint32_t n = *p.ovf_count;
+    unsigned long long* st = reinterpret_cast<unsigned long long*>(scratch + wave_scratch_entries<SIGMA, K, CAPF>());
+    const uint32_t g = blockIdx.x / p.ovf_parts, part = blockIdx.x - g * p.ovf_parts;
+    const uint32_t m0 = p.gm_off[g];
+    const uint32_t n = min(p.ovf_gcount[g], (p.gm_off[g + 1] - m0) * p.nwin);
+    if (part >= n) return;
+    const unsigned long long* queue = p.ovf_queue + (size_t)m0 * p.nwin;
     const uint32_t lane = lane_id(), wave = threadIdx.x >> 6;
-    uint32_t* cbase = state_all + (size_t)wave * 2 * NB * SUB;
-    uint32_t* cfill = cbase + NB * SUB;
-    for (uint32_t b = lane; b < NB * SUB; b += 64) { cbase[b] = CHUNK_NONE; cfill[b] = CH; }
-    Appender<TBL, NB> app{p, cbase, cfill, 0u};
-    bool have_group = false;
+    for (uint32_t b = threadIdx.x; b < NB; b += OVF_NW * 64) st[b] = ((unsigned long long)CHUNK_NONE << 32) | (unsigned long long)CH;
+    uint32_t chunk_next = 0, chunk_end = 0;
     unsigned long long emitted = 0;
-    constexpr uint32_t mulR = ipow(SIGMA, K - K / 2);
-    auto close_chunks = [&]() {
-        wave_lds_sync();
-        for (uint32_t b = lane; b < NB * SUB; b += 64) {
-            const uint32_t id = cbase[b];
-            if (id != CHUNK_NONE) p.desc[id] = ((unsigned long long)(app.g * NB + b / SUB) << 32) | (unsigned long long)min(cfill[b], CH);
-            cbase[b] = CHUNK_NONE; cfill[b] = CH;
-        }
-        wave_lds_sync();
-    };
-    const uint32_t per = (n + gridDim.x - 1) / gridDim.x;
-    const uint32_t q_lo = min(n, blockIdx.x * per), q_hi = min(n, q_lo + per);
-    for (uint32_t q = q_lo; q < q_hi; ++q) {
-        const unsigned long long e = p.ovf_queue[q];
-        const uint32_t g = (uint32_t)(e >> 42), mat = (uint32_t)(e >> 21) & 0x1FFFFFu, start = (uint32_t)e & 0x1FFFFFu;
-        if (have_group && g != app.g) close_chunks();
-        app.g = g; have_group = true;
+    const bool st_pool = !(p.flags & 1u);
+    for (uint32_t q = part; q < n; q += p.ovf_parts) {
+        const unsigned long long e = queue[q];
+        const uint32_t mat = (uint32_t)(e >> 32), start = (uint32_t)e;
         __syncthreads();
         const float* src = p.logp + ((size_t)mat * p.sites + start) * SIGMA;
         for (uint32_t i = threadIdx.x; i < K * SIGMA; i += OVF_NW * 64) cols[i] = src[i];
@@ -673,36 +673,67 @@
         const uint32_t nL = sh_n[0], nR = sh_n[1];
         if (nL == 0 || nR == 0) continue;
         uint32_t cnt = 0;
-        for (uint32_t i = wave; i < nL; i += OVF_NW) {
-            const uint2 a = L[i];
-            for (uint32_t jb = 0; jb < nR; jb += 128) {
-                const uint32_t ja = jb + lane, jc = jb + 64 + lane;
-                const bool va = ja < nR, vb = jc < nR;
-                uint2 b0 = make_uint2(0, 0), b1 = b0;
-                if (va) b0 = R[ja];
-                if (vb) b1 = R[jc];
-                const float s0 = __uint_as_float(a.y) + __uint_as_float(b0.y);
-                const float s1 = __uint_as_float(a.y) + __uint_as_float(b1.y);
-                const bool p0 = va && (s0 > p.eps), p1 = vb && (s1 > p.eps);
-                cnt += (uint32_t)__popcll(__ballot(p0)) + (uint32_t)__popcll(__ballot(p1));
-                app.append2(p0, a.x * mulR + b0.x, __float_as_uint(s0), p1, a.x * mulR + b1.x, __float_as_uint(s1));
+        constexpr uint32_t OVF_ROWS = 4;
+        for (uint32_t jb = 0; jb < nR; jb += 64) {
+            const uint32_t j = jb + lane;
+            const bool valid = j < nR;
+            uint2 b = make_uint2(0, 0);
+            if (valid) b = R[j];
+            const float by = __uint_as_float(b.y);
+            for (uint32_t i0 = wave; i0 < nL; i0 += OVF_NW * OVF_ROWS) {
+                uint2 a[OVF_ROWS];
+#pragma unroll
+                for (uint32_t u = 0; u < OVF_ROWS; ++u) a[u] = L[min(i0 + u * OVF_NW, nL - 1)];
+#pragma unroll
+                for (uint32_t u = 0; u < OVF_ROWS; ++u) {
+                    const float s = __uint_as_float(a[u].y) + by;
+                    const bool pass = valid && (i0 + u * OVF_NW < nL) && (s > p.eps);
+                    const uint64_t pm = __ballot(pass);
+                    if (pm == 0) continue;
+                    const uint32_t c = (uint32_t)__popcll(pm);
+                    cnt += c;
+                    const uint32_t ax = (uint32_t)__builtin_amdgcn_readfirstlane((int)a[u].x);
+                    const uint32_t bk = ax / ROWS_PER_BUCKET;
+                    uint32_t rid = 0, roff = 0;
+                    if (lane == 0) {
+                        unsigned long long old = __hip_atomic_load(&st[bk], __ATOMIC_RELAXED, __HIP_MEMORY_SCOPE_WORKGROUP);
+                        for (;;) {
+                            const uint32_t fill = (uint32_t)old, id = (uint32_t)(old >> 32);
+                            const bool fit = fill + c <= CH;
+                            if (!fit && chunk_next == chunk_end) {
+                                chunk_next = atomicAdd(p.pool_next, BIG_ALLOC_BATCH);
+                                chunk_end = chunk_next + BIG_ALLOC_BATCH;
+                            }
+                            const uint32_t nid = min(chunk_next, p.pool_cap);
+                            const unsigned long long want = fit ? old + c : (((unsigned long long)nid << 32) | (unsigned long long)c);
+                            const unsigned long long got = atomicCAS(&st[bk], old, want);
+                            if (got == old) {
+                                rid = fit ? id : nid; roff = fit ? fill : 0u;
+                                if (!fit) {
+                                    if (chunk_next >= p.pool_cap) atomicOr(p.pool_ovf, 1u);
+                                    ++chunk_next;
+                                    if (id < p.pool_cap) p.desc[id] = ((unsigned long long)(g * NB + bk) << 32) | (unsigned long long)fill;
+                                }
+                                break;
+                            }
+                            old = got;
+                        }
+                    }
+                    rid = (uint32_t)__builtin_amdgcn_readfirstlane((int)rid);
+                    roff = (uint32_t)__builtin_amdgcn_readfirstlane((int)roff);
+                    if (pass && st_pool) p.pool[(size_t)rid * CH + roff + mbcnt(pm)] = make_uint2(ax * mulR + b.x, __float_as_uint(s));
+                }
             }
         }
         emitted += cnt;
     }
-    if (have_group) close_chunks();
+    __syncthreads();
+    for (uint32_t b = threadIdx.x; b < NB; b += OVF_NW * 64) {
+        const unsigned long long s = st[b];
+        const uint32_t id = (uint32_t)(s >> 32);
+        if (id < p.pool_cap) p.desc[id] = ((unsigned long long)(g * NB + b) << 32) | (unsigned long long)(uint32_t)s;
+    }
     if (lane == 0 && emitted) atomicAdd(p.emitted, emitted);
-}
-
-__global__ __launch_bounds__(256) void ovf_group_keys_kernel(const unsigned long long* __restrict__ queue, uint32_t n,
-                                                             const uint32_t* __restrict__ mat_slot,
-                                                             unsigned long long* __restrict__ out)
-{
-    const uint32_t i = blockIdx.x * 256 + threadIdx.x;
-    if (i >= n) return;
-    const unsigned long long e = queue[i];
-    const uint32_t mat = (uint32_t)(e >> 32), start = (uint32_t)e;
-    out[i] = ((unsigned long long)mat_slot[mat] << 42) | ((unsigned long long)mat << 21) | (unsigned long long)start;
 }
 
 __global__ __launch_bounds__(256) void chunk_hist_kernel(const unsigned long long* __restrict__ desc, uint32_t n,
@@ -755,11 +786,12 @@
 constexpr uint32_t SMALL_BYTES = 64;
 
 __global__ void small_reset_kernel(uint32_t* __restrict__ small, uint32_t pre_chunks, uint32_t* __restrict__ tile_next, uint32_t n_groups,
-                                   uint32_t first_tile)
+                                   uint32_t first_tile, uint32_t* __restrict__ ovf_gcount)
 {
     const uint32_t i = blockIdx.x * blockDim.x + threadIdx.x;
     if (i < SMALL_XP_TOO_BIG / 4) small[i] = i == SMALL_POOL_NEXT / 4 ? pre_chunks : 0u;
     if (tile_next && i < n_groups) tile_next[i] = first_tile;
+    if (i < n_groups) ovf_gcount[i] = 0u;
 }
 
 __device__ __forceinline__ void store_slice_mask(const uint32_t* tab, uint32_t nslots, uint32_t* mask_words, uint32_t nthreads)
```

Measured after the change: 129.2 billion. 2.0% lower.
